# csmile-1006/ARP

Measured on NVIDIA B200. Metric: reward-labeled frames/sec, higher is better.
Workload: dtype fp16

## Files before the change

### arp_b200/build.py

```python
from __future__ import annotations

import hashlib
import os
import shutil
import subprocess
import sys
from pathlib import Path

PKG = Path(__file__).resolve().parent
CSRC = PKG / "csrc"
LIBDIR = PKG / "_lib"
LIB = LIBDIR / "libarp_b200.so"
STAMP = LIBDIR / "libarp_b200.stamp"

NVCC_FLAGS = [
    "-gencode", "arch=compute_100a,code=sm_100a",
    "-O3", "-std=c++17", "-lineinfo",
    "-shared", "-Xcompiler", "-fPIC",
    "-Xcompiler", "-fvisibility=hidden",
    "--expt-relaxed-constexpr",
    "-cudart", "static", "-Xcompiler", "-pthread",
]


if os.environ.get("ARP_OP_BF16", "0") not in ("", "0"):
    NVCC_FLAGS.append("-DARP_OP_FP16=0")


def _nvcc() -> str:
    for cand in (os.environ.get("NVCC"), shutil.which("nvcc"), "/usr/local/cuda/bin/nvcc"):
        if cand and Path(cand).exists():
            return cand
    raise RuntimeError("nvcc not found; arp_b200 has no prebuilt or CPU fallback")


def _sources_digest() -> str:
    h = hashlib.sha256()
    for p in sorted(list(CSRC.glob("*.cu")) + list(CSRC.glob("*.cuh")) + [PKG.parent / "include" / "arp_b200.h"]):
        h.update(p.name.encode())
        h.update(p.read_bytes())
    h.update(" ".join(NVCC_FLAGS).encode())
    return h.hexdigest()


def _file_digest(path: Path) -> str:
    return hashlib.sha256(path.read_bytes()).hexdigest()


def build_variant(out: Path, defines: list[str]) -> Path:
    out = Path(out)
    out.parent.mkdir(parents=True, exist_ok=True)
    flags = [f for f in NVCC_FLAGS if not f.startswith("-DARP_OP_")]
    res = subprocess.run([_nvcc(), *flags, *[f"-D{d}" for d in defines], "-o", str(out), str(CSRC / "capi.cu")],
                         capture_output=True, text=True)
    if res.returncode != 0:
        raise RuntimeError(f"nvcc failed:\n{res.stdout}\n{res.stderr}")
    return out


def build(force: bool = False, verbose: bool = False) -> Path:
    LIBDIR.mkdir(exist_ok=True)
    digest = _sources_digest()
    if not force and LIB.exists() and STAMP.exists() and STAMP.read_text().split() == [digest, _file_digest(LIB)]:
        return LIB
    cmd = [_nvcc(), *NVCC_FLAGS, "-o", str(LIB), str(CSRC / "capi.cu")]
    if verbose:
        cmd.insert(1, "-Xptxas")
        cmd.insert(2, "-v")
        print(" ".join(cmd), file=sys.stderr)
    res = subprocess.run(cmd, capture_output=True, text=True)
    if res.returncode != 0:
        raise RuntimeError(f"nvcc failed:\n{res.stdout}\n{res.stderr}")
    if verbose:
        print(res.stderr, file=sys.stderr)
    STAMP.write_text(f"{digest} {_file_digest(LIB)}")
    return LIB


JITTER_LIB = LIBDIR / "libarp_b200_jitter.so"


def build_jitter() -> Path:
    LIBDIR.mkdir(exist_ok=True)
    stamp = LIBDIR / "libarp_b200_jitter.stamp"
    digest = _sources_digest()
    if JITTER_LIB.exists() and stamp.exists() and stamp.read_text().split() == [digest, _file_digest(JITTER_LIB)]:
        return JITTER_LIB
    build_variant(JITTER_LIB, ["ARP_ATTN_JITTER"])
    stamp.write_text(f"{digest} {_file_digest(JITTER_LIB)}")
    return JITTER_LIB


if __name__ == "__main__":
    print(build(force="--force" in sys.argv, verbose="-v" in sys.argv))
```

### arp_b200/capi.py

```python
from __future__ import annotations

import ctypes as C
import os
from pathlib import Path

import numpy as np
import torch

_PKG = Path(__file__).resolve().parent
_LIB_PATH = Path(os.environ.get("ARP_B200_LIB") or _PKG / "_lib" / "libarp_b200.so")

ARP_OK = 0
ARP_ERR_INVALID, ARP_ERR_CUDA, ARP_ERR_STATE, ARP_ERR_NO_DEVICE, ARP_ERR_UNKNOWN_KEY = -1, -2, -3, -4, -5
PRE_PIL_BICUBIC, PRE_BILINEAR = 0, 1
HEAD_CLIP, HEAD_ADAPTER, HEAD_ADAPTER_ENSEMBLE, HEAD_CLIP_GOAL, HEAD_ADAPTER_GOAL = 0, 1, 2, 3, 4
REDUCE_FIRST, REDUCE_MEAN = 0, 1
DT_F32, DT_BF16, DT_F16 = 0, 1, 2
ACT_NONE, ACT_QUICKGELU, ACT_RELU = 0, 1, 2
PREC_BF16, PREC_F32, PREC_F32RESID = 0, 1, 2
PREC_16BIT = PREC_BF16
PRECISIONS = {"16bit": PREC_16BIT, "bf16": PREC_16BIT, "fp16": PREC_16BIT, "fp32resid": PREC_F32RESID, "fp32": PREC_F32}
(ARP_INFLATE_OK, ARP_INFLATE_TRUNCATED, ARP_INFLATE_BAD_HEADER, ARP_INFLATE_BAD_BLOCK, ARP_INFLATE_BAD_CODE,
 ARP_INFLATE_DISTANCE_TOO_FAR, ARP_INFLATE_TOO_LONG, ARP_INFLATE_TOO_SHORT, ARP_INFLATE_BAD_ADLER) = range(9)
MAX_TEXT = 16
MAX_TEXT_GROUPS = 16
MAX_TEXT_TOTAL = 64

EXPORTS = (
    "arp_create", "arp_destroy", "arp_last_error", "arp_abi_version", "arp_set_weight", "arp_missing_weights",
    "arp_set_text", "arp_label", "arp_label_host", "arp_compute_reward", "arp_encode_image", "arp_decode_only",
    "arp_scan_only", "arp_gemm_bf16", "arp_layernorm_bf16", "arp_attention", "arp_launch_count",
    "arp_profile_begin", "arp_profile_end", "arp_online_reward", "arp_preprocess_rtgs",
    "arp_quantile_f32", "arp_encode_taps_chw", "arp_operand_dtype", "arp_ln_gemm", "arp_resid_gemm_stats", "arp_label_file", "arp_wants_weight",
    "arp_set_text_groups", "arp_text_groups", "arp_embedding_dim", "arp_embed_host", "arp_embed_file",
    "arp_label_embeddings", "arp_tower_dim", "arp_embed_tower_host", "arp_embed_tower_file", "arp_label_tower",
    "arp_label_zfile", "arp_embed_zfile", "arp_embed_tower_zfile", "arp_inflate_rows",
)
PROFILE_CLASSES = ("gemm", "attention", "layernorm", "decode", "head", "scan", "other")


class ArpProfileStats(C.Structure):
    _fields_ = [("launches", C.c_int64), ("total_ms", C.c_double), ("flops", C.c_double), ("bytes", C.c_double)]


class ArpConfig(C.Structure):
    _fields_ = [(n, C.c_int32) for n in (
        "struct_size", "device", "patch", "width", "layers", "heads", "embed_dim", "in_h", "in_w", "use_crop",
        "preprocess", "head", "reduce", "max_batch", "precision")]


class ArpError(RuntimeError):
    def __init__(self, code: int, msg: str):
        super().__init__(f"arp_b200 error {code}: {msg}")
        self.code = code


_lib = None


def precision_enum(name: str) -> int:
    if name not in PRECISIONS:
        raise ValueError(f"precision must be one of {sorted(PRECISIONS)}, got {name!r}")
    return PRECISIONS[name]


def lib_path() -> Path:
    return _LIB_PATH


def load_library() -> C.CDLL:
    global _lib
    if _lib is not None:
        return _lib
    if not _LIB_PATH.exists():
        raise FileNotFoundError(
            f"{_LIB_PATH} not built — run `python -m arp_b200.build` (or __graft_entry__.build()). "
            "arp_b200 has no CPU or PyTorch fallback.")
    lib = C.CDLL(os.fspath(_LIB_PATH))
    vp, i32, i64, f32 = C.c_void_p, C.c_int32, C.c_int64, C.c_float
    lib.arp_create.argtypes = [C.POINTER(ArpConfig), C.POINTER(vp)]
    lib.arp_destroy.argtypes = [vp]
    lib.arp_destroy.restype = None
    lib.arp_last_error.argtypes = [vp]
    lib.arp_last_error.restype = C.c_char_p
    lib.arp_abi_version.argtypes = []
    lib.arp_operand_dtype.argtypes = []
    lib.arp_set_weight.argtypes = [vp, C.c_char_p, vp, i32, C.POINTER(i64), i32, vp]
    lib.arp_missing_weights.argtypes = [vp, C.c_char_p, i64]
    lib.arp_set_text.argtypes = [vp, vp, i32, i32, f32, vp]
    lib.arp_set_text_groups.argtypes = [vp, vp, i32, i32, vp, i32, f32, vp]
    lib.arp_text_groups.argtypes = [vp]
    lib.arp_label.argtypes = [vp, vp, i64, i64, vp, i32, i32, vp, vp, vp, vp, vp]
    lib.arp_label_host.argtypes = [vp, vp, i64, i64, vp, i32, i32, vp, vp, vp, vp]
    lib.arp_label_file.argtypes = [vp, i32, i64, i64, i64, vp, i32, i32, vp, vp, vp, vp]
    lib.arp_wants_weight.argtypes = [vp, C.c_char_p]
    lib.arp_embedding_dim.argtypes = [vp]
    lib.arp_embed_host.argtypes = [vp, vp, i64, i64, vp]
    lib.arp_embed_file.argtypes = [vp, i32, i64, i64, i64, vp]
    lib.arp_label_embeddings.argtypes = [vp, vp, i64, vp, i32, i32, vp, vp, vp, vp, vp]
    lib.arp_tower_dim.argtypes = [vp]
    lib.arp_embed_tower_host.argtypes = [vp, vp, i64, i64, vp]
    lib.arp_embed_tower_file.argtypes = [vp, i32, i64, i64, i64, vp]
    lib.arp_label_tower.argtypes = [vp, vp, i64, vp, i32, i32, vp, vp, vp, vp, vp]
    lib.arp_label_zfile.argtypes = [vp, i32, vp, vp, i64, i64, vp, i32, i32, vp, vp, vp, vp]
    lib.arp_embed_zfile.argtypes = [vp, i32, vp, vp, i64, i64, vp]
    lib.arp_embed_tower_zfile.argtypes = [vp, i32, vp, vp, i64, i64, vp]
    lib.arp_inflate_rows.argtypes = [vp, vp, vp, vp, i64, i64, vp, vp, vp]
    lib.arp_compute_reward.argtypes = [vp, vp, i64, i64, vp, vp, vp]
    lib.arp_online_reward.argtypes = [vp, vp, i32, vp, vp, vp]
    lib.arp_preprocess_rtgs.argtypes = [vp, vp, i64, vp, i32, i32, i32, vp, vp, vp, vp, vp]
    lib.arp_quantile_f32.argtypes = [vp, vp, i64, i64, i64, vp, vp]
    lib.arp_encode_taps_chw.argtypes = [vp, vp, i64, vp, vp, vp]
    lib.arp_encode_image.argtypes = [vp, vp, i64, i64, vp, vp]
    lib.arp_decode_only.argtypes = [vp, vp, i64, i64, vp, vp]
    lib.arp_scan_only.argtypes = [vp, vp, i64, vp, i32, i32, f32, vp, vp, vp, vp]
    lib.arp_gemm_bf16.argtypes = [vp, vp, vp, vp, i32, i64, i32, i32, vp, vp, i32, vp]
    lib.arp_ln_gemm.argtypes = [vp, vp, vp, vp, vp, vp, vp, i64, i32, i32, vp]
    lib.arp_resid_gemm_stats.argtypes = [vp, vp, vp, vp, vp, vp, i64, i32, i32, vp]
    lib.arp_layernorm_bf16.argtypes = [vp, vp, vp, vp, vp, i64, vp]
    lib.arp_attention.argtypes = [vp, vp, vp, i32, i32, vp]
    lib.arp_launch_count.argtypes = [vp]
    lib.arp_launch_count.restype = i64
    lib.arp_profile_begin.argtypes = [vp]
    lib.arp_profile_end.argtypes = [vp, C.POINTER(ArpProfileStats), i32]
    for name in EXPORTS:
        if name not in ("arp_destroy", "arp_last_error", "arp_launch_count"):
            getattr(lib, name).restype = C.c_int
    _lib = lib
    return lib


_TORCH_DT = {torch.float32: DT_F32, torch.bfloat16: DT_BF16, torch.float16: DT_F16}


def operand_dtype() -> torch.dtype:
    return {DT_BF16: torch.bfloat16, DT_F16: torch.float16}[load_library().arp_operand_dtype()]


def _ptr(t: "torch.Tensor | None"):
    return None if t is None else C.c_void_p(t.data_ptr())


def _stream_ptr(device) -> C.c_void_p:
    return C.c_void_p(torch.cuda.current_stream(device).cuda_stream)


class Engine:

    def __init__(self, *, device: int = 0, patch: int = 16, in_h: int = 64, in_w: int = 64, use_crop: bool = False,
                 preprocess: int = PRE_PIL_BICUBIC, head: int = HEAD_CLIP, reduce: int = REDUCE_FIRST,
                 max_batch: int = 256, layers: int = 12, width: int = 768, heads: int = 12, embed_dim: int = 512,
                 precision: int = PREC_BF16):
        self._lib = load_library()
        self._h = C.c_void_p()
        self.cfg = ArpConfig(C.sizeof(ArpConfig), device, patch, width, layers, heads, embed_dim, in_h, in_w,
                             int(bool(use_crop)), preprocess, head, reduce, max_batch, precision)
        rc = self._lib.arp_create(C.byref(self.cfg), C.byref(self._h))
        if rc != ARP_OK:
            raise ArpError(rc, (self._lib.arp_last_error(None) or b"").decode())
        self.device = torch.device("cuda", device)
        self.tokens = (224 // patch) ** 2 + 1
        self.adapter = head in (HEAD_ADAPTER, HEAD_ADAPTER_ENSEMBLE, HEAD_ADAPTER_GOAL)
        self.goal = head in (HEAD_CLIP_GOAL, HEAD_ADAPTER_GOAL)
        self.feat_dim = (layers + 1) * embed_dim if self.adapter else embed_dim
        self.n_text = 0
        self._grouped = False

    def close(self):
        if getattr(self, "_h", None) and self._h.value:
            self._lib.arp_destroy(self._h)
            self._h = C.c_void_p()

    def __del__(self):
        try:
            self.close()
        except Exception:
            pass

    def _check(self, rc: int):
        if rc != ARP_OK:
            raise ArpError(rc, (self._lib.arp_last_error(self._h) or b"").decode())

    @property
    def launch_count(self) -> int:
        return int(self._lib.arp_launch_count(self._h))

    def profile_begin(self):
        self._check(self._lib.arp_profile_begin(self._h))

    def profile_end(self) -> dict:
        arr = (ArpProfileStats * len(PROFILE_CLASSES))()
        self._check(self._lib.arp_profile_end(self._h, arr, len(PROFILE_CLASSES)))
        return {n: {"launches": int(a.launches), "total_ms": a.total_ms, "flops": a.flops, "bytes": a.bytes}
                for n, a in zip(PROFILE_CLASSES, arr)}

    def set_weight(self, name: str, tensor: torch.Tensor, strict: bool = True) -> bool:
        t = tensor.detach()
        if t.dtype not in _TORCH_DT:
            t = t.float()
        t = t.to(self.device).contiguous()
        shape = (C.c_int64 * max(t.dim(), 1))(*t.shape)
        rc = self._lib.arp_set_weight(self._h, name.encode(), _ptr(t), _TORCH_DT[t.dtype], shape, t.dim(),
                                      _stream_ptr(self.device))
        if rc == ARP_ERR_UNKNOWN_KEY and not strict:
            return False
        self._check(rc)
        torch.cuda.current_stream(self.device).synchronize()
        return True

    def load_state_dict(self, state_dict, strict: bool = False) -> list[str]:
        seen = getattr(self, "_uploaded", None)
        if seen is None:
            seen = self._uploaded = {}
        for k, v in state_dict.items():
            if not torch.is_tensor(v):
                continue
            if not strict and not self._lib.arp_wants_weight(self._h, k.encode()):
                continue
            mark = (v.data_ptr(), tuple(v.shape), v.dtype, v._version, v.device)
            if k in seen and seen[k][0] == mark and seen[k][1] is v:
                continue
            if self.set_weight(k, v, strict=strict):
                seen[k] = (mark, v)
        return self.missing_weights()

    def missing_weights(self) -> list[str]:
        buf = C.create_string_buffer(1 << 16)
        n = self._lib.arp_missing_weights(self._h, buf, len(buf))
        return [s for s in buf.value.decode().split("\n") if s] if n else []

    def set_text(self, text_emb: torch.Tensor, logit_scale_exp: float):
        t = text_emb.detach().to(self.device, torch.float32).contiguous()
        assert t.dim() == 2
        self._check(self._lib.arp_set_text(self._h, _ptr(t), t.shape[0], t.shape[1], float(logit_scale_exp),
                                           _stream_ptr(self.device)))
        torch.cuda.current_stream(self.device).synchronize()
        self.n_text = t.shape[0]
        self._grouped = False

    def set_text_groups(self, embs: "list[torch.Tensor]", logit_scale_exp: float):
        rows = [e.detach().to(self.device, torch.float32) for e in embs]
        assert rows and all(r.dim() == 2 for r in rows)
        t = torch.cat(rows).contiguous()
        off = np.concatenate([[0], np.cumsum([r.shape[0] for r in rows])]).astype(np.int32)
        self._check(self._lib.arp_set_text_groups(self._h, _ptr(t), t.shape[0], t.shape[1], C.c_void_p(off.ctypes.data),
                                                  len(rows), float(logit_scale_exp), _stream_ptr(self.device)))
        torch.cuda.current_stream(self.device).synchronize()
        self.n_text = t.shape[0]
        self._grouped = True

    @property
    def n_groups(self) -> int:
        return int(self._lib.arp_text_groups(self._h))

    def _lead(self) -> tuple:
        return (self.n_groups,) if self._grouped else ()

    def _host_outputs(self, T: int, num_frames: int):
        lead = self._lead()
        return (np.empty(lead + (T,), np.float32), np.empty(lead + (T,), np.float32),
                np.empty(lead + (T, num_frames), np.float32), np.empty(lead + (T, num_frames), np.float32))

    @staticmethod
    def _frames_view(ob: torch.Tensor):
        assert ob.dtype == torch.uint8 and ob.is_contiguous() and ob.dim() in (4, 5)
        T = ob.shape[0]
        frame = int(np.prod(ob.shape[-3:]))
        if ob.dim() == 5:
            F = ob.shape[1]
            return T, ob.data_ptr() + (F - 1) * frame, F * frame
        return T, ob.data_ptr(), frame
# ... 130 lines not shown
    @staticmethod
    def _chunk_table(chunk_offsets, chunk_bytes):
        off = np.ascontiguousarray(chunk_offsets, dtype=np.int64)
        nb = np.ascontiguousarray(chunk_bytes, dtype=np.int64)
        assert off.ndim == 1 and off.shape == nb.shape, (off.shape, nb.shape)
        return off, nb, C.c_void_p(off.ctypes.data), C.c_void_p(nb.ctypes.data)

    def label_zfile(self, fd: int, chunk_offsets: np.ndarray, chunk_bytes: np.ndarray, row_bytes: int,
                    ep_offsets: np.ndarray, num_frames: int, out=None):
        off, nb, p_off, p_nb = self._chunk_table(chunk_offsets, chunk_bytes)
        ep = np.ascontiguousarray(ep_offsets, dtype=np.int64)
        T = off.size
        if out is None:
            out = self._host_outputs(T, num_frames)
        hp = lambda a: C.c_void_p(a.ctypes.data)
        self._check(self._lib.arp_label_zfile(self._h, int(fd), p_off, p_nb, T, int(row_bytes), hp(ep), ep.size - 1,
                                              num_frames, hp(out[0]), hp(out[1]), hp(out[2]), hp(out[3])))
        return out

    def embed_zfile(self, fd: int, chunk_offsets: np.ndarray, chunk_bytes: np.ndarray, row_bytes: int,
                    out: "np.ndarray | None" = None) -> np.ndarray:
        off, nb, p_off, p_nb = self._chunk_table(chunk_offsets, chunk_bytes)
        out = self._emb_out(off.size, out)
        self._check(self._lib.arp_embed_zfile(self._h, int(fd), p_off, p_nb, off.size, int(row_bytes),
                                              C.c_void_p(out.ctypes.data)))
        return out

    def embed_tower_zfile(self, fd: int, chunk_offsets: np.ndarray, chunk_bytes: np.ndarray, row_bytes: int,
                          out: "np.ndarray | None" = None) -> np.ndarray:
        off, nb, p_off, p_nb = self._chunk_table(chunk_offsets, chunk_bytes)
        out = self._emb_out(off.size, out, self.tower_dim)
        self._check(self._lib.arp_embed_tower_zfile(self._h, int(fd), p_off, p_nb, off.size, int(row_bytes),
                                                    C.c_void_p(out.ctypes.data)))
        return out

    def inflate_rows(self, src: torch.Tensor, src_offsets: torch.Tensor, src_bytes: torch.Tensor, row_bytes: int):
        assert src.dtype == torch.uint8 and src.is_cuda and src.is_contiguous()
        so = src_offsets.to(self.device, torch.int64).contiguous()
        sb = src_bytes.to(self.device, torch.int64).contiguous()
        n = so.numel()
        assert sb.numel() == n
        out = torch.zeros((n, int(row_bytes)), device=self.device, dtype=torch.uint8)
        status = torch.full((n,), -1, device=self.device, dtype=torch.int32)
        self._check(self._lib.arp_inflate_rows(self._h, _ptr(src), _ptr(so), _ptr(sb), n, int(row_bytes), _ptr(out),
                                               _ptr(status), _stream_ptr(self.device)))
        return out, status

    def compute_reward(self, ob: torch.Tensor, want_logits: bool = False):
        T, p, stride = self._frames_view(ob)
        r = torch.empty(self._lead() + (T,), device=self.device, dtype=torch.float32)
        lg = torch.empty(T, max(self.n_text, 1), device=self.device, dtype=torch.float32) if want_logits else None
        self._check(self._lib.arp_compute_reward(self._h, C.c_void_p(p), T, stride, _ptr(r), _ptr(lg),
                                                 _stream_ptr(self.device)))
        return (r, lg) if want_logits else r

    def online_reward(self, frames: np.ndarray, want_logits: bool = False, want_features: bool = False):
        f = np.ascontiguousarray(frames, dtype=np.uint8)
        if f.ndim == 3:
            f = f[None]
        assert f.ndim == 4 and f.shape[1:] == (self.cfg.in_h, self.cfg.in_w, 3), f.shape
        n = f.shape[0]
        out = {}
        r = lg = ft = None
        if not self.goal:
            r = out["reward"] = np.empty(n, np.float32)
            if want_logits:
                lg = out["logits"] = np.empty((n, self.n_text), np.float32)
        if want_features or self.goal:
            ft = out["features"] = np.empty((n, self.feat_dim), np.float32)
        p = lambda a: None if a is None else C.c_void_p(a.ctypes.data)
        self._check(self._lib.arp_online_reward(self._h, p(f), n, p(r), p(lg), p(ft)))
        return out

    def preprocess_rtgs(self, reward: torch.Tensor, ep_offsets: torch.Tensor, num_frames: int, use_normalize: bool):
        r = reward.to(self.device, torch.float32).contiguous()
        off = ep_offsets.to(self.device, torch.int64).contiguous()
        T = r.numel()
        g = torch.zeros(T, device=self.device, dtype=torch.float32)
        gs = torch.zeros(T, num_frames, device=self.device, dtype=torch.float32)
        shifted = torch.empty(T, device=self.device, dtype=torch.float32) if use_normalize else None
        stats = np.zeros(4, np.float32)
        self._check(self._lib.arp_preprocess_rtgs(self._h, _ptr(r), T, _ptr(off), off.numel() - 1, num_frames,
                                                  int(bool(use_normalize)), _ptr(shifted), _ptr(g), _ptr(gs),
                                                  C.c_void_p(stats.ctypes.data), _stream_ptr(self.device)))
        return gs, g, stats

    def order_statistics(self, x: torch.Tensor, k_lo: int, k_hi: int) -> np.ndarray:
        x = x.to(self.device, torch.float32).contiguous().view(-1)
        out = np.zeros(2, np.float32)
        self._check(self._lib.arp_quantile_f32(self._h, _ptr(x), x.numel(), int(k_lo), int(k_hi),
                                               C.c_void_p(out.ctypes.data), _stream_ptr(self.device)))
        return out

    def encode_taps(self, chw: torch.Tensor):
        x = chw.to(self.device, torch.float32).contiguous()
        assert x.dim() == 4 and tuple(x.shape[1:]) == (3, 224, 224), x.shape
        T = x.shape[0]
        taps = torch.empty(T, self.cfg.layers * self.cfg.width, device=self.device, dtype=torch.float32)
        feat = torch.empty(T, self.cfg.embed_dim, device=self.device, dtype=torch.float32)
        self._check(self._lib.arp_encode_taps_chw(self._h, _ptr(x), T, _ptr(taps), _ptr(feat), _stream_ptr(self.device)))
        return taps, feat

    def encode_image(self, ob: torch.Tensor) -> torch.Tensor:
        T, p, stride = self._frames_view(ob)
        f = torch.empty(T, self.feat_dim, device=self.device, dtype=torch.float32)
        self._check(self._lib.arp_encode_image(self._h, C.c_void_p(p), T, stride, _ptr(f), _stream_ptr(self.device)))
        return f

    def decode_only(self, ob: torch.Tensor) -> torch.Tensor:
        T, p, stride = self._frames_view(ob)
        out = torch.empty(T, 3, 224, 224, device=self.device, dtype=torch.float32)
        self._check(self._lib.arp_decode_only(self._h, C.c_void_p(p), T, stride, _ptr(out), _stream_ptr(self.device)))
        return out

    def scan_only(self, reward: torch.Tensor, ep_offsets: torch.Tensor, num_frames: int, gamma: float = 1.0):
        r = reward.to(self.device, torch.float32).contiguous()
        off = ep_offsets.to(self.device, torch.int64).contiguous()
        T = r.numel()
        g = torch.empty(T, device=self.device, dtype=torch.float32)
        rs = torch.empty(T, num_frames, device=self.device, dtype=torch.float32)
        gs = torch.empty(T, num_frames, device=self.device, dtype=torch.float32)
        self._check(self._lib.arp_scan_only(self._h, _ptr(r), T, _ptr(off), off.numel() - 1, num_frames, gamma,
                                            _ptr(g), _ptr(rs), _ptr(gs), _stream_ptr(self.device)))
        return g, rs, gs

    def gemm(self, a: torch.Tensor, w: torch.Tensor, bias=None, resid=None, act: int = ACT_NONE,
             out_dtype=None) -> torch.Tensor:
        op = operand_dtype()
        assert a.dtype in (torch.bfloat16, torch.float16) and w.dtype in (torch.bfloat16, torch.float16)
        a, w = a.to(op).contiguous(), w.to(op).contiguous()
        M, K = a.shape
        N = w.shape[0]
        out_dtype = op if out_dtype in (None, torch.bfloat16, torch.float16) else out_dtype
        out = torch.empty(M, N, device=self.device, dtype=out_dtype)
        if resid is not None:
            resid = resid.to(out_dtype).contiguous()
        self._check(self._lib.arp_gemm_bf16(self._h, _ptr(a), _ptr(w), _ptr(out),
                                            DT_F32 if out_dtype == torch.float32 else _TORCH_DT[op], M, N, K, _ptr(bias),
                                            _ptr(resid), act, _stream_ptr(self.device)))
        return out

    def resid_gemm_stats(self, a: torch.Tensor, w: torch.Tensor, bias: torch.Tensor, x: torch.Tensor):
        op = operand_dtype()
        assert x.dtype == op and x.is_contiguous() and x.device == self.device
        a, w = a.to(op).contiguous(), w.to(op).contiguous()
        bias = bias.to(self.device, torch.float32).contiguous()
        M, K = a.shape
        N = w.shape[0]
        stats = torch.empty(M, 2, device=self.device, dtype=torch.float32)
        self._check(self._lib.arp_resid_gemm_stats(self._h, _ptr(a), _ptr(w), _ptr(bias), _ptr(x), _ptr(stats), M, N, K,
                                                   _stream_ptr(self.device)))
        return stats

    def ln_gemm(self, x: torch.Tensor, gamma, beta, w: torch.Tensor, bias: torch.Tensor, act: int = ACT_NONE) -> torch.Tensor:
        op = operand_dtype()
        x = x.to(op).contiguous()
        f = lambda t: t.to(self.device, torch.float32).contiguous()
        gamma, beta, w, bias = f(gamma), f(beta), f(w), f(bias)
        M, N = x.shape[0], w.shape[0]
        out = torch.empty(M, N, device=self.device, dtype=op)
        self._check(self._lib.arp_ln_gemm(self._h, _ptr(x), _ptr(gamma), _ptr(beta), _ptr(w), _ptr(bias), _ptr(out),
                                          M, N, act, _stream_ptr(self.device)))
        return out

    def layernorm(self, x: torch.Tensor, gamma: torch.Tensor, beta: torch.Tensor) -> torch.Tensor:
        assert x.dtype == torch.float32 and x.is_contiguous() and x.shape[-1] == 768
        y = torch.empty(x.shape, device=self.device, dtype=operand_dtype())
        self._check(self._lib.arp_layernorm_bf16(self._h, _ptr(x), _ptr(gamma), _ptr(beta), _ptr(y),
                                                 x.numel() // 768, _stream_ptr(self.device)))
        return y

    def attention(self, qkv: torch.Tensor, B: int, tokens: int) -> torch.Tensor:
        assert qkv.dtype in (torch.bfloat16, torch.float16)
        qkv = qkv.to(operand_dtype()).contiguous()
        out = torch.empty(B * tokens, qkv.shape[-1] // 3, device=self.device, dtype=qkv.dtype)
        self._check(self._lib.arp_attention(self._h, _ptr(qkv), _ptr(out), B, tokens, _stream_ptr(self.device)))
        return out
```

### arp_b200/csrc/attention_tc.cuh

```cuda
#pragma once

#include "common.cuh"

namespace arp {

constexpr int ATC_THREADS = 448;
constexpr int ATC_DH = 64;

template <int L>
struct AtcCfg {
  static constexpr int NK = (L + 15) / 16 * 16;
  static constexpr int QT = (L + 127) / 128;
  static constexpr int Q_BYTES = 128 * ATC_DH * 2;
  static constexpr int KV_BYTES = NK * ATC_DH * 2;
  static constexpr int KV_PAD = (KV_BYTES + 1023) / 1024 * 1024;
  static constexpr int BUF_BYTES = QT * Q_BYTES + 2 * KV_PAD;
  static constexpr int ONES_BYTES = 16 * 128;
  static constexpr int STAGE_BYTES = QT * 128 * ATC_DH * 2;
  static constexpr int SMEM_BYTES = 2 * BUF_BYTES + ONES_BYTES + STAGE_BYTES + 1024 + 256;
  static constexpr int O_COL = QT * NK;
  static constexpr int O_N = ATC_DH + 16;
  static constexpr bool SPREAD = QT == 2;
  static constexpr int Q1_LOADS = 5;
  static constexpr int QK_TX_BYTES = SPREAD ? Q_BYTES + Q1_LOADS * 16 * 128 + KV_BYTES : QT * Q_BYTES + KV_BYTES;
  static_assert(!SPREAD || (L - 176 > 16 && L - 176 <= 24 && NK % 64 == 16), "tile-1 spread is laid out for 193..200 tokens");
  static_assert(O_COL + O_N <= 512, "TMEM columns");
  static_assert(KV_PAD >= (NK / 16 - 1) * 2048, "the ones tile must sit past every step's V rows (positive LBO)");
};

__device__ __forceinline__ void umma_bf16_ts(uint32_t d_tmem, uint32_t a_tmem, uint64_t b_desc, uint32_t idesc,
                                             uint32_t accumulate) {
  asm volatile(
      "{\n\t"
      ".reg .pred p;\n\t"
      "setp.ne.b32 p, %4, 0;\n\t"
      "tcgen05.mma.cta_group::1.kind::f16 [%0], [%1], %2, %3, p;\n\t"
      "}\n" ::"r"(d_tmem),
      "r"(a_tmem), "l"(b_desc), "r"(idesc), "r"(accumulate)
      : "memory");
}

__device__ __forceinline__ void tmem_ld_32x16(uint32_t taddr, uint32_t (&r)[16]) {
  asm volatile(
      "tcgen05.ld.sync.aligned.32x32b.x16.b32 "
      "{%0, %1, %2, %3, %4, %5, %6, %7, %8, %9, %10, %11, %12, %13, %14, %15}, [%16];"
      : "=r"(r[0]), "=r"(r[1]), "=r"(r[2]), "=r"(r[3]), "=r"(r[4]), "=r"(r[5]), "=r"(r[6]), "=r"(r[7]),
        "=r"(r[8]), "=r"(r[9]), "=r"(r[10]), "=r"(r[11]), "=r"(r[12]), "=r"(r[13]), "=r"(r[14]), "=r"(r[15])
      : "r"(taddr)
      : "memory");
}
__device__ __forceinline__ void tmem_st_32x8(uint32_t taddr, const uint32_t (&r)[8]) {
  asm volatile("tcgen05.st.sync.aligned.32x32b.x8.b32 [%0], {%1, %2, %3, %4, %5, %6, %7, %8};" ::"r"(taddr),
               "r"(r[0]), "r"(r[1]), "r"(r[2]), "r"(r[3]), "r"(r[4]), "r"(r[5]), "r"(r[6]), "r"(r[7])
               : "memory");
}
__device__ __forceinline__ void tmem_st_wait() { asm volatile("tcgen05.wait::st.sync.aligned;" ::: "memory"); }

__device__ __forceinline__ uint64_t umma_desc_mnmajor_sw128(uint32_t smem_addr, uint32_t lbo_bytes = 16) {
  uint64_t d = 0;
  d |= static_cast<uint64_t>((smem_addr & 0x3FFFF) >> 4);
  d |= static_cast<uint64_t>((lbo_bytes >> 4) & 0x3FFF) << 16;
  d |= static_cast<uint64_t>(1024 >> 4) << 32;
  d |= static_cast<uint64_t>(1) << 46;
  d |= static_cast<uint64_t>(2) << 61;
  return d;
}

__device__ __forceinline__ uint32_t pack_bf16_int(float lo, float hi) {
  const uint32_t a = __float_as_uint(lo) + 0x8000u, b = __float_as_uint(hi) + 0x8000u;
  return (a >> 16) | (b & 0xffff0000u);
}

constexpr float kPExpOffset = ARP_OP_FP16 ? 97.0f : 0.0f;
__device__ __forceinline__ uint32_t pack_bf16_trunc(float lo, float hi) {
#if ARP_OP_FP16
  return (__float_as_uint(lo) >> 13) | ((__float_as_uint(hi) << 3) & 0xffff0000u);
#else
  return (__float_as_uint(lo) >> 16) | (__float_as_uint(hi) & 0xffff0000u);
#endif
}
constexpr uint32_t kOnes2 = ARP_OP_FP16 ? 0x3c003c00u : 0x3f803f80u;

__device__ __forceinline__ float ex2_approx(float x) {
  float y;
  asm("ex2.approx.ftz.f32 %0, %1;" : "=f"(y) : "f"(x));
  return y;
}

__device__ __forceinline__ void tmem_st_32x16(uint32_t taddr, const uint32_t (&r)[16]) {
  asm volatile(
      "tcgen05.st.sync.aligned.32x32b.x16.b32 [%0], {%1, %2, %3, %4, %5, %6, %7, %8, %9, %10, %11, %12, %13, %14, "
      "%15, %16};" ::"r"(taddr),
      "r"(r[0]), "r"(r[1]), "r"(r[2]), "r"(r[3]), "r"(r[4]), "r"(r[5]), "r"(r[6]), "r"(r[7]), "r"(r[8]), "r"(r[9]),
      "r"(r[10]), "r"(r[11]), "r"(r[12]), "r"(r[13]), "r"(r[14]), "r"(r[15])
      : "memory");
}

__device__ __forceinline__ void tmem_ld_16x256_x8(uint32_t taddr, uint32_t (&r)[32]) {
  asm volatile(
      "tcgen05.ld.sync.aligned.16x256b.x8.b32 "
      "{%0, %1, %2, %3, %4, %5, %6, %7, %8, %9, %10, %11, %12, %13, %14, %15, "
      "%16, %17, %18, %19, %20, %21, %22, %23, %24, %25, %26, %27, %28, %29, %30, %31}, [%32];"
      : "=r"(r[0]), "=r"(r[1]), "=r"(r[2]), "=r"(r[3]), "=r"(r[4]), "=r"(r[5]), "=r"(r[6]), "=r"(r[7]),
        "=r"(r[8]), "=r"(r[9]), "=r"(r[10]), "=r"(r[11]), "=r"(r[12]), "=r"(r[13]), "=r"(r[14]), "=r"(r[15]),
        "=r"(r[16]), "=r"(r[17]), "=r"(r[18]), "=r"(r[19]), "=r"(r[20]), "=r"(r[21]), "=r"(r[22]), "=r"(r[23]),
        "=r"(r[24]), "=r"(r[25]), "=r"(r[26]), "=r"(r[27]), "=r"(r[28]), "=r"(r[29]), "=r"(r[30]), "=r"(r[31])
      : "r"(taddr)
      : "memory");
}
__device__ __forceinline__ void tmem_ld_16x256_x2(uint32_t taddr, uint32_t (&r)[8]) {
  asm volatile("tcgen05.ld.sync.aligned.16x256b.x2.b32 {%0, %1, %2, %3, %4, %5, %6, %7}, [%8];"
               : "=r"(r[0]), "=r"(r[1]), "=r"(r[2]), "=r"(r[3]), "=r"(r[4]), "=r"(r[5]), "=r"(r[6]), "=r"(r[7])
               : "r"(taddr)
               : "memory");
}
__device__ __forceinline__ void tmem_st_16x128_x8(uint32_t taddr, const uint32_t (&r)[16]) {
  asm volatile(
      "tcgen05.st.sync.aligned.16x128b.x8.b32 [%0], {%1, %2, %3, %4, %5, %6, %7, %8, %9, %10, %11, %12, %13, %14, "
      "%15, %16};" ::"r"(taddr),
      "r"(r[0]), "r"(r[1]), "r"(r[2]), "r"(r[3]), "r"(r[4]), "r"(r[5]), "r"(r[6]), "r"(r[7]), "r"(r[8]), "r"(r[9]),
      "r"(r[10]), "r"(r[11]), "r"(r[12]), "r"(r[13]), "r"(r[14]), "r"(r[15])
      : "memory");
}
__device__ __forceinline__ void tmem_st_16x128_x2(uint32_t taddr, const uint32_t (&r)[4]) {
  asm volatile("tcgen05.st.sync.aligned.16x128b.x2.b32 [%0], {%1, %2, %3, %4};" ::"r"(taddr), "r"(r[0]), "r"(r[1]),
               "r"(r[2]), "r"(r[3])
               : "memory");
}
__device__ __forceinline__ void tmem_ld_32x1(uint32_t taddr, uint32_t& r) {
  asm volatile("tcgen05.ld.sync.aligned.32x32b.x1.b32 {%0}, [%1];" : "=r"(r) : "r"(taddr) : "memory");
}
__device__ __forceinline__ float rcp_approx(float x) {
  float y;
  asm("rcp.approx.ftz.f32 %0, %1;" : "=f"(y) : "f"(x));
  return y;
}

#ifdef ARP_ATTN_JITTER
__device__ __forceinline__ void atc_jitter(uint32_t salt) {
  uint32_t h = (static_cast<uint32_t>(clock64()) ^ (salt * 2654435761u) ^ (threadIdx.x >> 5) * 40503u ^ blockIdx.x * 9176u);
  h ^= h >> 13; h *= 0x5bd1e995u; h ^= h >> 15;
  if (h & 1) __nanosleep((h >> 1) & 8191);
}
#define ATC_JITTER(salt) atc_jitter(salt)
#else
#define ATC_JITTER(salt)
#endif

#ifdef ARP_ATTN_TRACE
constexpr int ATC_TR_ITEMS = 10, ATC_TR_EVENTS = 36;
__device__ long long g_attn_trace[2 * ATC_TR_ITEMS * ATC_TR_EVENTS];
#define ATC_TRACE(ev, slot, item)                                                                              \
  do {                                                                                                         \
    if (blockIdx.x == 0 && (threadIdx.x & 31) == 0 && (item) < ATC_TR_ITEMS)                                   \
      atc_tr[((slot) * ATC_TR_ITEMS + (item)) * ATC_TR_EVENTS + (ev)] = clock64();                             \
  } while (0)
#define ATC_TRACE_T(ev, slot, item)                                                                            \
  do {                                                                                                         \
    if (blockIdx.x == 0 && (item) < ATC_TR_ITEMS)                                                              \
      atc_tr[((slot) * ATC_TR_ITEMS + (item)) * ATC_TR_EVENTS + (ev)] = clock64();                             \
  } while (0)
#else
#define ATC_TRACE(ev, slot, item)
#define ATC_TRACE_T(ev, slot, item)
#endif

template <int L>
__global__ void __launch_bounds__(ATC_THREADS, 1)
attention_tc_kernel(const __grid_constant__ CUtensorMap tmap_q, const __grid_constant__ CUtensorMap tmap_kv,
                    const __grid_constant__ CUtensorMap tmap_o, const __grid_constant__ CUtensorMap tmap_q16,
                    const __grid_constant__ CUtensorMap tmap_o16, int n_frames, int heads, int width, float scale_log2e,
                    int reverse) {
  using C = AtcCfg<L>;
  extern __shared__ uint8_t smem_raw[];
  uint8_t* smem = reinterpret_cast<uint8_t*>((reinterpret_cast<uintptr_t>(smem_raw) + 1023) & ~uintptr_t(1023));
  uint8_t* ones = smem + 2 * C::BUF_BYTES;
  uint8_t* stage = ones + C::ONES_BYTES;
  uint64_t* bars = reinterpret_cast<uint64_t*>(stage + C::STAGE_BYTES);
  uint64_t* qk_full = bars;
  uint64_t* qk_empty = bars + 2;
  uint64_t* v_full = bars + 4;
  uint64_t* v_empty = bars + 6;
  uint64_t* s_full = bars + 8;
  uint64_t* o_full = bars + 10;
  uint64_t* o_drained = bars + 12;
  uint64_t* xu_turn = bars + 14;
  uint64_t* p_done = bars + 18;
  uint64_t* rem_go = bars + 20;
  uint32_t* tmem_slot = reinterpret_cast<uint32_t*>(bars + 22);

  const int warp = __shfl_sync(0xffffffffu, static_cast<int>(threadIdx.x >> 5), 0), lane = threadIdx.x & 31;
  const int n_items = n_frames * heads;
#ifdef ARP_ATTN_TRACE
  __shared__ long long atc_tr[2 * ATC_TR_ITEMS * ATC_TR_EVENTS];
  for (int i = threadIdx.x; i < 2 * ATC_TR_ITEMS * ATC_TR_EVENTS; i += ATC_THREADS) atc_tr[i] = 0;
#endif
  constexpr int SM_WARPS = 4 * C::QT;

  if (warp == 0 && lane == 0) {
    tma_prefetch_desc(&tmap_q);
    tma_prefetch_desc(&tmap_kv);
    tma_prefetch_desc(&tmap_o);
    tma_prefetch_desc(&tmap_q16);
    tma_prefetch_desc(&tmap_o16);
  }
  if (warp == 1 && lane == 0) {
    for (int i = 0; i < 2; ++i) {
      mbar_init(&qk_full[i], 1);
      mbar_init(&qk_empty[i], C::QT);
      mbar_init(&v_full[i], 1);
      mbar_init(&v_empty[i], C::QT);
      mbar_init(&s_full[i], 1);
      mbar_init(&o_full[i], 1);
    }
    for (int i = 0; i < 4; ++i) mbar_init(&xu_turn[i], 1);
    mbar_init(&p_done[0], 4);
    mbar_init(&p_done[1], C::SPREAD ? 5 : 4);
    mbar_init(&rem_go[0], 1);
    mbar_init(&rem_go[1], 1);
    mbar_init(&o_drained[0], 4);
    mbar_init(&o_drained[1], 4);
    fence_mbar_init();
  }
  for (int i = threadIdx.x; i < C::ONES_BYTES / 16; i += ATC_THREADS)
    reinterpret_cast<uint4*>(ones)[i] = make_uint4(kOnes2, kOnes2, kOnes2, kOnes2);
  if (C::SPREAD) {
    for (int i = threadIdx.x; i < 2 * 3 * 2048 / 16; i += ATC_THREADS) {
      const int b = i / (3 * 128), q = (i / 128) % 3, w = i % 128;
      reinterpret_cast<uint4*>(smem + b * C::BUF_BYTES + C::Q_BYTES + q * 4096 + 2048)[w] = make_uint4(0u, 0u, 0u, 0u);
    }
  }
  fence_proxy_async_smem();
  if (warp == 1) tmem_alloc<512>(tmem_slot);
  tc_fence_before();
  __syncthreads();
  tc_fence_after();
  const uint32_t tmem_base = __shfl_sync(0xffffffffu, *tmem_slot, 0);

  constexpr uint32_t idesc_s = umma_idesc_bf16(128, C::NK);
  constexpr uint32_t idesc_o = umma_idesc_bf16(128, C::O_N, 0, 1);
  auto issue_s = [&](uint32_t sbuf, int t, [[maybe_unused]] int tr_item) {
    const uint64_t dk = umma_desc_kmajor_sw128(sbuf + C::QT * C::Q_BYTES);
    const uint64_t dq = umma_desc_kmajor_sw128(sbuf + t * C::Q_BYTES);
    ATC_TRACE_T(24, t, tr_item);
#pragma unroll
    for (int k = 0; k < ATC_DH / 16; ++k) umma_bf16_ss(tmem_base + t * C::NK, dq + 2 * k, dk + 2 * k, idesc_s, k != 0);
    umma_commit(&s_full[t]);
    umma_commit(&qk_empty[(sbuf - smem_u32(smem)) / C::BUF_BYTES]);
    ATC_TRACE_T(27, t, tr_item);
  };
  auto issue_pv = [&](uint32_t sbuf, int t, [[maybe_unused]] int tr_item) {
    const uint32_t v_addr = sbuf + C::QT * C::Q_BYTES + C::KV_PAD;
    const uint64_t dv = umma_desc_mnmajor_sw128(v_addr, smem_u32(ones) - v_addr);
    constexpr uint64_t kStep = (2048ull >> 4) - ((2048ull >> 4) << 16);
    ATC_TRACE_T(28, t, tr_item);
#pragma unroll
    for (int k = 0; k < C::NK / 16; ++k)
      umma_bf16_ts(tmem_base + C::O_COL, tmem_base + t * C::NK + k * 8, dv + k * kStep, idesc_o, k != 0);
    umma_commit(&o_full[t]);
    ATC_TRACE_T(30, t, tr_item);
  };

  const bool sp_c0 = 192 + 2 * (lane & 3) < L, sp_c1 = 193 + 2 * (lane & 3) < L;
  auto spread_rowmax = [&](uint32_t tg, float& row_a, float& row_b) {
    auto max16 = [](const uint32_t (&r)[32], float& ma, float& mb) {
#pragma unroll
      for (int i = 0; i < 8; ++i) {
        ma = fmaxf(ma, fmaxf(__uint_as_float(r[4 * i]), __uint_as_float(r[4 * i + 1])));
        mb = fmaxf(mb, fmaxf(__uint_as_float(r[4 * i + 2]), __uint_as_float(r[4 * i + 3])));
      }
    };
    uint32_t a[32], bq[32], tl[8];
    float a0 = -INFINITY, a1 = -INFINITY, b0m = -INFINITY, b1m = -INFINITY;
    tmem_ld_16x256_x8(tg, a);
    tmem_ld_16x256_x8(tg + 64, bq);
    tmem_ld_wait();
    max16(a, a0, b0m);
    max16(bq, a1, b1m);
    tmem_ld_16x256_x8(tg + 128, a);
    tmem_ld_16x256_x2(tg + 192, tl);
    tmem_ld_wait();
    max16(a, a0, b0m);
    if (sp_c0) { a1 = fmaxf(a1, __uint_as_float(tl[0])); b1m = fmaxf(b1m, __uint_as_float(tl[2])); }
    if (sp_c1) { a1 = fmaxf(a1, __uint_as_float(tl[1])); b1m = fmaxf(b1m, __uint_as_float(tl[3])); }
    float ma = fmaxf(a0, a1), mb = fmaxf(b0m, b1m);
    ma = fmaxf(ma, __shfl_xor_sync(0xffffffffu, ma, 1));
    mb = fmaxf(mb, __shfl_xor_sync(0xffffffffu, mb, 1));
    ma = fmaxf(ma, __shfl_xor_sync(0xffffffffu, ma, 2));
    mb = fmaxf(mb, __shfl_xor_sync(0xffffffffu, mb, 2));
    row_a = ma;
    row_b = mb;
  };
  auto spread_exp = [&](uint32_t tg, float max_a, float max_b, bool both) {
    const float mo_a = max_a * scale_log2e + kPExpOffset, mo_b = max_b * scale_log2e + kPExpOffset;
    const uint64_t sc2 = f32x2_pack(scale_log2e, scale_log2e), na2 = f32x2_pack(-mo_a, -mo_a), nb2 = f32x2_pack(-mo_b, -mo_b);
    auto chunk16 = [&](const uint32_t (&src)[32], int blk) {
      uint32_t pk[16];
// ... 349 lines not shown
```

### arp_b200/csrc/capi.cu

```cuda
#include <cuda.h>
#include <cuda_runtime.h>

#include <atomic>
#include <chrono>
#include <cmath>
#include <condition_variable>
#include <cstdarg>
#include <cstdio>
#include <cstring>
#include <algorithm>
#include <map>
#include <mutex>
#include <string>
#include <thread>
#include <tuple>
#include <vector>

#include <cerrno>
#include <unistd.h>

#include "../../include/arp_b200.h"
#include "attention_tc.cuh"
#include "decode.cuh"
#include "fp32_path.cuh"
#include "gemm_tcgen05.cuh"
#include "head.cuh"
#include "inflate.cuh"
#include "layernorm.cuh"
#include "rtgstats.cuh"
#include "scan.cuh"
#include "tower.cuh"

using namespace arp;
static_assert(ARP_MAX_TEXT == HEAD_MAX_TEXT && ARP_MAX_TEXT_GROUPS == HEAD_MAX_GROUPS &&
              ARP_MAX_TEXT_TOTAL == HEAD_MAX_TEXT_TOTAL, "text limits of include/arp_b200.h and head.cuh disagree");
typedef arp::op_t bf16;
#define ARP_OP_DTYPE (ARP_OP_FP16 ? ARP_F16 : ARP_BF16)

static thread_local std::string g_create_error;

struct ArpHandle;
static int fail(ArpHandle* h, int code, const char* fmt, ...);

#define ARP_CUDA(h, expr)                                                                      \
  do {                                                                                         \
    cudaError_t _e = (expr);                                                                   \
    if (_e != cudaSuccess)                                                                     \
      return fail(h, ARP_ERR_CUDA, "%s failed: %s (%s:%d)", #expr, cudaGetErrorString(_e), __FILE__, __LINE__); \
  } while (0)

#define ARP_TRY(expr)            \
  do {                           \
    int _r = (expr);             \
    if (_r != ARP_OK) return _r; \
  } while (0)

typedef CUresult (*PFN_encodeTiled)(CUtensorMap*, CUtensorMapDataType, cuuint32_t, void*, const cuuint64_t*,
                                    const cuuint64_t*, const cuuint32_t*, const cuuint32_t*, CUtensorMapInterleave,
                                    CUtensorMapSwizzle, CUtensorMapL2promotion, CUtensorMapFloatOOBfill);

static PFN_encodeTiled get_encode_tiled() {
  static PFN_encodeTiled fn = nullptr;
  if (fn) return fn;
  void* p = nullptr;
  cudaDriverEntryPointQueryResult q;
  if (cudaGetDriverEntryPoint("cuTensorMapEncodeTiled", &p, cudaEnableDefault, &q) != cudaSuccess ||
      q != cudaDriverEntryPointSuccess)
    return nullptr;
  fn = reinterpret_cast<PFN_encodeTiled>(p);
  return fn;
}

struct LayerW {
  float *ln1_g = nullptr, *ln1_b = nullptr, *ln2_g = nullptr, *ln2_b = nullptr;
  bf16 *w_qkv = nullptr, *w_out = nullptr, *w_fc = nullptr, *w_proj = nullptr;
  float *b_qkv = nullptr, *b_out = nullptr, *b_fc = nullptr, *b_proj = nullptr;
  float *w_qkv_f32 = nullptr, *w_fc_f32 = nullptr;
  bf16 *w_qkv_fold = nullptr, *w_fc_fold = nullptr;
  float *s_qkv = nullptr, *c_qkv = nullptr, *s_fc = nullptr, *c_fc = nullptr;
};

struct WeightSlot {
  void** dst_f32 = nullptr;
  void** dst;
  int64_t numel;
  bool as_bf16;
  bool required;
  bool set;
};

struct TmapKey {
  const void* ptr; uint64_t rows, cols, ld; uint32_t box_rows, box_cols, elem;
  bool operator<(const TmapKey& o) const {
    return std::tie(ptr, rows, cols, ld, box_rows, box_cols, elem) <
           std::tie(o.ptr, o.rows, o.cols, o.ld, o.box_rows, o.box_cols, o.elem);
  }
};

struct ArpHandle {
  ArpConfig cfg;
  std::string err;
  int64_t launches = 0;
  bool resid16 = true;
  int dir = 0;
  bool f32 = false;
  int tokens = 0, grid = 0, kp = 0;
  bool adapter = false, goal = false;
  int n_scales = 0, feat_dim = 0;

  bf16* conv1 = nullptr;
  float *class_emb = nullptr, *pos_emb = nullptr, *rowtab = nullptr;
  float *ln_pre_g = nullptr, *ln_pre_b = nullptr, *ln_post_g = nullptr, *ln_post_b = nullptr;
  float* proj = nullptr;
  std::vector<LayerW> layers;
  bf16 *inter_w = nullptr, *fc1_w = nullptr, *fc2_w = nullptr;
  float *fc1_b = nullptr, *fc2_b = nullptr, *res_w = nullptr;
  float res_sigmoid = 0.f;
  bool finalized = false;
  bool adapter_ready = false;
  std::map<std::string, WeightSlot> slots;

  float* text = nullptr;
  int* group_off = nullptr;
  int group_off_host[HEAD_MAX_GROUPS + 1] = {};
  int n_text = 0, text_dim = 0, n_groups = 1;
  float logit_scale = 0.f;

  int *h_min = nullptr, *h_cnt = nullptr, *h_k = nullptr, *v_min = nullptr, *v_cnt = nullptr, *v_k = nullptr;
  int h_ksize = 0, v_ksize = 0, max_rows = 0;
  float* lut = nullptr;
  int crop_top = 0, crop_left = 0, src_h = 0, src_w = 0;

  struct Work {
    bf16* x16 = nullptr;
    float2* stats = nullptr;
    float* x = nullptr;
    bf16 *xn = nullptr, *qkv = nullptr, *attn = nullptr, *hid = nullptr;
    bf16 *taps = nullptr, *featb = nullptr, *hid2 = nullptr;
    float *featf = nullptr, *mlp = nullptr;
    float* xcls = nullptr;
    bf16 *xncls = nullptr, *qcls = nullptr, *acls = nullptr, *hcls = nullptr;
    float *chw32 = nullptr, *xn32 = nullptr, *qkv32 = nullptr, *attn32 = nullptr, *hid32 = nullptr;
    float *taps32 = nullptr, *hid2_32 = nullptr;
  } ws;

  void* scratch[2] = {nullptr, nullptr};
  size_t scratch_bytes[2] = {0, 0};
  uint8_t* stage_dev[2] = {nullptr, nullptr};
  size_t stage_bytes = 0;
  uint8_t* zsrc_dev[2] = {nullptr, nullptr};
  size_t zsrc_bytes = 0;
  uint8_t* zrows_dev = nullptr;
  size_t zrows_bytes = 0;
  void* ztab_dev = nullptr;
  size_t ztab_bytes = 0;
  uint8_t* pin_ring = nullptr;
  size_t pin_bytes = 0;
  cudaEvent_t ev_slot[8] = {nullptr, nullptr, nullptr, nullptr, nullptr, nullptr, nullptr, nullptr};
  cudaStream_t copy_stream = nullptr, own_stream = nullptr;
  cudaEvent_t ev_copied[2] = {nullptr, nullptr}, ev_consumed[2] = {nullptr, nullptr};

  std::map<TmapKey, CUtensorMap> tmaps;
  std::vector<void*> allocs;

  struct OnlineGraph { cudaGraphExec_t exec = nullptr; int64_t launches = 0; uint64_t epoch = 0; };
  std::map<int, OnlineGraph> online_graphs;
  uint64_t online_epoch = 1;
  float* online_out = nullptr;
  void* stats_dev = nullptr;

  bool profiling = false;
  struct ProfRec { int cls; double flops; double bytes; cudaEvent_t e0, e1; };
  std::vector<ProfRec> prof;
  std::vector<cudaEvent_t> event_pool;
};

enum ProfClass { PC_GEMM = 0, PC_ATTENTION = 1, PC_LAYERNORM = 2, PC_DECODE = 3, PC_HEAD = 4, PC_SCAN = 5, PC_OTHER = 6, PC_COUNT = 7 };

static cudaEvent_t prof_event(ArpHandle* h) {
  if (!h->event_pool.empty()) { cudaEvent_t e = h->event_pool.back(); h->event_pool.pop_back(); return e; }
  cudaEvent_t e = nullptr;
  cudaEventCreate(&e);
  return e;
}

struct ProfScope {
  ArpHandle* h; cudaStream_t st; size_t idx; bool on;
  ProfScope(ArpHandle* h_, int cls, double flops, double bytes, cudaStream_t st_) : h(h_), st(st_), idx(0), on(h_->profiling) {
    if (!on) return;
    ArpHandle::ProfRec r{cls, flops, bytes, prof_event(h), prof_event(h)};
    cudaEventRecord(r.e0, st);
    idx = h->prof.size();
    h->prof.push_back(r);
  }
  ~ProfScope() { if (on) cudaEventRecord(h->prof[idx].e1, st); }
};

static int fail(ArpHandle* h, int code, const char* fmt, ...) {
  char buf[1024];
  va_list ap;
  va_start(ap, fmt);
  vsnprintf(buf, sizeof(buf), fmt, ap);
  va_end(ap);
  if (h) h->err = buf; else g_create_error = buf;
  return code;
}

template <typename T>
static int dev_alloc(ArpHandle* h, T** p, size_t count) {
  void* q = nullptr;
  ARP_CUDA(h, cudaMalloc(&q, count * sizeof(T) + 256));
  h->allocs.push_back(q);
  ARP_CUDA(h, cudaMemset(q, 0, count * sizeof(T) + 256));
  *p = reinterpret_cast<T*>(q);
  return ARP_OK;
}

static double bicubic_filter(double x) {
  const double a = -0.5;
  if (x < 0.0) x = -x;
  if (x < 1.0) return ((a + 2.0) * x - (a + 3.0)) * x * x + 1;
  if (x < 2.0) return (((x - 5) * x + 8) * x - 4) * a;
  return 0.0;
}

static void pil_bicubic_tables(int in_size, int out_size, std::vector<int>& xmin_v, std::vector<int>& cnt_v,
                               std::vector<int>& kk, int& ksize) {
  double scale = static_cast<double>(in_size) / out_size;
  double filterscale = scale < 1.0 ? 1.0 : scale;
  const double support = 2.0 * filterscale;
  ksize = static_cast<int>(std::ceil(support)) * 2 + 1;
  xmin_v.assign(out_size, 0);
  cnt_v.assign(out_size, 0);
  kk.assign(static_cast<size_t>(out_size) * ksize, 0);
  std::vector<double> k(ksize);
  for (int xx = 0; xx < out_size; ++xx) {
    const double center = 0.0 + (xx + 0.5) * scale;
    double ww = 0.0;
    const double ss = 1.0 / filterscale;
    int xmin = static_cast<int>(center - support + 0.5);
    if (xmin < 0) xmin = 0;
    int xmax = static_cast<int>(center + support + 0.5);
    if (xmax > in_size) xmax = in_size;
    xmax -= xmin;
    for (int x = 0; x < xmax; ++x) {
      const double w = bicubic_filter((x + xmin - center + 0.5) * ss);
      k[x] = w;
      ww += w;
    }
    for (int x = 0; x < xmax; ++x)
      if (ww != 0.0) k[x] /= ww;
    for (int x = 0; x < xmax; ++x) {
      const double v = k[x] * (1 << 22);
      kk[static_cast<size_t>(xx) * ksize + x] = v < 0 ? static_cast<int>(-0.5 + v) : static_cast<int>(0.5 + v);
    }
    xmin_v[xx] = xmin;
    cnt_v[xx] = xmax;
  }
}

static const float kClipMean[3] = {0.48145466f, 0.4578275f, 0.40821073f};
static const float kClipStd[3] = {0.26862954f, 0.26130258f, 0.27577711f};

template <typename T>
static int upload(ArpHandle* h, T** dst, const std::vector<T>& v) {
  ARP_TRY(dev_alloc(h, dst, v.size()));
  ARP_CUDA(h, cudaMemcpy(*dst, v.data(), v.size() * sizeof(T), cudaMemcpyHostToDevice));
  return ARP_OK;
}

static int build_decode_tables(ArpHandle* h) {
  const ArpConfig& c = h->cfg;
  h->src_h = c.in_h;
  h->src_w = c.in_w;
  h->crop_top = h->crop_left = 0;
  if (c.use_crop) {
    if (c.preprocess == ARP_PRE_PIL_BICUBIC) {
      const int cs = c.in_w / 2;
      h->src_h = h->src_w = cs;
      h->crop_top = static_cast<int>(std::nearbyint((c.in_h - cs) / 2.0));
      h->crop_left = static_cast<int>(std::nearbyint((c.in_w - cs) / 2.0));
    } else {
      const int cs = c.in_w / 2;
      h->src_h = h->src_w = cs;
      h->crop_top = (c.in_h - cs) / 2;
      h->crop_left = (c.in_w - cs) / 2;
    }
  }
  if (h->src_h <= 0 || h->src_w <= 0 || h->crop_top < 0 || h->crop_top + h->src_h > c.in_h || h->crop_left < 0 ||
      h->crop_left + h->src_w > c.in_w)
    return fail(h, ARP_ERR_INVALID, "bad crop geometry for %dx%d (a crop larger than the frame would be zero-padded by "
                "torchvision; not supported)", c.in_h, c.in_w);
  if (c.preprocess == ARP_PRE_PIL_BICUBIC) {
    int out_w = DEC_OUT, out_h = DEC_OUT;
    if (h->src_w > h->src_h) out_w = static_cast<int>(static_cast<long long>(DEC_OUT) * h->src_w / h->src_h);
    else if (h->src_h > h->src_w) out_h = static_cast<int>(static_cast<long long>(DEC_OUT) * h->src_h / h->src_w);
    const int win_left = static_cast<int>(std::nearbyint((out_w - DEC_OUT) / 2.0));
    const int win_top = static_cast<int>(std::nearbyint((out_h - DEC_OUT) / 2.0));
    std::vector<int> xm, xc, xk, ym, yc, yk;
    {
      std::vector<int> fm, fc, fk;
      pil_bicubic_tables(h->src_w, out_w, fm, fc, fk, h->h_ksize);
      xm.assign(fm.begin() + win_left, fm.begin() + win_left + DEC_OUT);
      xc.assign(fc.begin() + win_left, fc.begin() + win_left + DEC_OUT);
      xk.assign(fk.begin() + (size_t)win_left * h->h_ksize, fk.begin() + (size_t)(win_left + DEC_OUT) * h->h_ksize);
      pil_bicubic_tables(h->src_h, out_h, fm, fc, fk, h->v_ksize);
      ym.assign(fm.begin() + win_top, fm.begin() + win_top + DEC_OUT);
      yc.assign(fc.begin() + win_top, fc.begin() + win_top + DEC_OUT);
      yk.assign(fk.begin() + (size_t)win_top * h->v_ksize, fk.begin() + (size_t)(win_top + DEC_OUT) * h->v_ksize);
    }
    if (h->h_ksize > 64 || h->v_ksize > 64) return fail(h, ARP_ERR_INVALID, "downscale factor too large");
    {
// ... 16 lines not shown
    ARP_TRY(upload(h, &h->h_min, xm)); ARP_TRY(upload(h, &h->h_cnt, xc)); ARP_TRY(upload(h, &h->h_k, xk));
    ARP_TRY(upload(h, &h->v_min, ym)); ARP_TRY(upload(h, &h->v_cnt, yc)); ARP_TRY(upload(h, &h->v_k, yk));
    std::vector<float> lut(3 * 256);
    for (int ch = 0; ch < 3; ++ch)
      for (int u = 0; u < 256; ++u) {
        volatile float v = static_cast<float>(u) / 255.0f;
        volatile float w = v - kClipMean[ch];
        lut[ch * 256 + u] = w / kClipStd[ch];
      }
    ARP_TRY(upload(h, &h->lut, lut));
  } else {
    const float sc = static_cast<float>(h->src_h) / DEC_OUT;
    h->max_rows = static_cast<int>(sc * DEC_BAND) + 4;
    if (h->max_rows > h->src_h) h->max_rows = h->src_h;
    h->h_ksize = h->v_ksize = 0;
  }
  return ARP_OK;
}

static void add_slot(ArpHandle* h, const std::string& name, void** dst, int64_t numel, bool as_bf16, bool required) {
  WeightSlot s;
  s.dst = dst; s.numel = numel; s.as_bf16 = as_bf16; s.required = required; s.set = false;
  h->slots[name] = s;
}

static void register_slots(ArpHandle* h) {
  const ArpConfig& c = h->cfg;
  const int W = c.width, P = c.patch;
  add_slot(h, "visual.conv1.weight", (void**)&h->conv1, (int64_t)W * 3 * P * P, true, true);
  add_slot(h, "visual.class_embedding", (void**)&h->class_emb, W, false, true);
  add_slot(h, "visual.positional_embedding", (void**)&h->pos_emb, (int64_t)h->tokens * W, false, true);
  add_slot(h, "visual.ln_pre.weight", (void**)&h->ln_pre_g, W, false, true);
  add_slot(h, "visual.ln_pre.bias", (void**)&h->ln_pre_b, W, false, true);
  add_slot(h, "visual.ln_post.weight", (void**)&h->ln_post_g, W, false, true);
  add_slot(h, "visual.ln_post.bias", (void**)&h->ln_post_b, W, false, true);
  add_slot(h, "visual.proj", (void**)&h->proj, (int64_t)W * c.embed_dim, false, true);
  h->layers.resize(c.layers);
  for (int l = 0; l < c.layers; ++l) {
    LayerW& L = h->layers[l];
    const std::string p = "visual.transformer.resblocks." + std::to_string(l) + ".";
    add_slot(h, p + "ln_1.weight", (void**)&L.ln1_g, W, false, true);
    add_slot(h, p + "ln_1.bias", (void**)&L.ln1_b, W, false, true);
    add_slot(h, p + "ln_2.weight", (void**)&L.ln2_g, W, false, true);
    add_slot(h, p + "ln_2.bias", (void**)&L.ln2_b, W, false, true);
    add_slot(h, p + "attn.in_proj_weight", (void**)&L.w_qkv, (int64_t)3 * W * W, true, true);
    add_slot(h, p + "attn.in_proj_bias", (void**)&L.b_qkv, 3 * W, false, true);
    add_slot(h, p + "attn.out_proj.weight", (void**)&L.w_out, (int64_t)W * W, true, true);
    add_slot(h, p + "attn.out_proj.bias", (void**)&L.b_out, W, false, true);
    add_slot(h, p + "mlp.c_fc.weight", (void**)&L.w_fc, (int64_t)4 * W * W, true, true);
    add_slot(h, p + "mlp.c_fc.bias", (void**)&L.b_fc, 4 * W, false, true);
    add_slot(h, p + "mlp.c_proj.weight", (void**)&L.w_proj, (int64_t)4 * W * W, true, true);
    add_slot(h, p + "mlp.c_proj.bias", (void**)&L.b_proj, W, false, true);
    h->slots[p + "attn.in_proj_weight"].dst_f32 = (void**)&L.w_qkv_f32;
    h->slots[p + "mlp.c_fc.weight"].dst_f32 = (void**)&L.w_fc_f32;
  }
  if (h->adapter) {
    const int64_t D = h->feat_dim;
    const int64_t Din = (int64_t)c.layers * W;
    const int64_t Dmid = (int64_t)c.layers * c.embed_dim;
    add_slot(h, "image_intermediate_linear.weight", (void**)&h->inter_w, Dmid * Din, true, true);
    add_slot(h, "image_adapter.layers.0.weight", (void**)&h->fc1_w, 2 * D * D, true, true);
    add_slot(h, "image_adapter.layers.0.bias", (void**)&h->fc1_b, 2 * D, false, true);
    add_slot(h, "image_adapter.layers.3.weight", (void**)&h->fc2_w, 2 * D * D, true, true);
    add_slot(h, "image_adapter.layers.3.bias", (void**)&h->fc2_b, D, false, true);
    add_slot(h, "image_residual_weight", (void**)&h->res_w, 1, false, true);
  }
}

template <typename S, typename D>
__global__ void convert_kernel(const S* __restrict__ src, D* __restrict__ dst, size_t n) {
  for (size_t i = static_cast<size_t>(blockIdx.x) * blockDim.x + threadIdx.x; i < n;
       i += static_cast<size_t>(gridDim.x) * blockDim.x)
    dst[i] = static_cast<D>(static_cast<float>(src[i]));
}

template <typename S, typename D>
static void launch_convert(ArpHandle* h, const void* src, void* dst, size_t n, cudaStream_t st) {
  const int blocks = static_cast<int>(std::min<size_t>((n + 255) / 256, 148 * 16));
  convert_kernel<S, D><<<blocks, 256, 0, st>>>(static_cast<const S*>(src), static_cast<D*>(dst), n);
  h->launches++;
}

__global__ void build_rowtab_kernel(const float* __restrict__ pos, const float* __restrict__ cls,
                                    float* __restrict__ tab, int tokens, int W) {
  const int i = blockIdx.x * blockDim.x + threadIdx.x;
  if (i >= tokens * W) return;
  tab[i] = pos[i] + (i < W ? cls[i] : 0.f);
}

extern "C" int arp_abi_version(void) { return ARP_B200_ABI_VERSION; }
extern "C" int arp_operand_dtype(void) { return ARP_OP_DTYPE; }

extern "C" const char* arp_last_error(const ArpHandle* h) { return h ? h->err.c_str() : g_create_error.c_str(); }

extern "C" int64_t arp_launch_count(const ArpHandle* h) { return h ? h->launches : 0; }

extern "C" int arp_profile_begin(ArpHandle* h) {
  if (!h) return ARP_ERR_INVALID;
  for (auto& r : h->prof) { h->event_pool.push_back(r.e0); h->event_pool.push_back(r.e1); }
  h->prof.clear();
  h->profiling = true;
  return ARP_OK;
}

extern "C" int arp_profile_end(ArpHandle* h, ArpProfileStats* out, int32_t n_classes) {
  if (!h || !out || n_classes < 1) return fail(h, ARP_ERR_INVALID, "null argument");
  h->profiling = false;
  ARP_CUDA(h, cudaSetDevice(h->cfg.device));
  ARP_CUDA(h, cudaDeviceSynchronize());
  for (int i = 0; i < n_classes; ++i) out[i] = ArpProfileStats{0, 0.0, 0.0, 0.0};
  for (auto& r : h->prof) {
    float ms = 0.f;
    cudaEventElapsedTime(&ms, r.e0, r.e1);
    if (r.cls < n_classes) {
      out[r.cls].launches += 1;
      out[r.cls].total_ms += ms;
      out[r.cls].flops += r.flops;
      out[r.cls].bytes += r.bytes;
    }
    h->event_pool.push_back(r.e0);
    h->event_pool.push_back(r.e1);
  }
  h->prof.clear();
  return ARP_OK;
}

template <typename K>
static int set_smem(ArpHandle* h, K kernel, int bytes) {
  ARP_CUDA(h, cudaFuncSetAttribute(kernel, cudaFuncAttributeMaxDynamicSharedMemorySize, bytes));
  return ARP_OK;
}

extern "C" void arp_destroy(ArpHandle* h) {
  if (!h) return;
  cudaSetDevice(h->cfg.device);
  cudaDeviceSynchronize();
  for (void* p : h->allocs) cudaFree(p);
  for (int i = 0; i < 2; ++i) if (h->scratch[i]) cudaFree(h->scratch[i]);
  for (int i = 0; i < 2; ++i) {
    if (h->stage_dev[i]) cudaFree(h->stage_dev[i]);
    if (h->zsrc_dev[i]) cudaFree(h->zsrc_dev[i]);
    if (h->ev_copied[i]) cudaEventDestroy(h->ev_copied[i]);
    if (h->ev_consumed[i]) cudaEventDestroy(h->ev_consumed[i]);
  }
  if (h->zrows_dev) cudaFree(h->zrows_dev);
  if (h->ztab_dev) cudaFree(h->ztab_dev);
  if (h->pin_ring) cudaFreeHost(h->pin_ring);
  for (cudaEvent_t e : h->ev_slot) if (e) cudaEventDestroy(e);
  for (auto& kv : h->online_graphs) if (kv.second.exec) cudaGraphExecDestroy(kv.second.exec);
  for (auto& r : h->prof) { cudaEventDestroy(r.e0); cudaEventDestroy(r.e1); }
  for (cudaEvent_t e : h->event_pool) cudaEventDestroy(e);
  if (h->copy_stream) cudaStreamDestroy(h->copy_stream);
  if (h->own_stream) cudaStreamDestroy(h->own_stream);
  delete h;
}

extern "C" int arp_create(const ArpConfig* cfg, ArpHandle** out) {
  if (!cfg || !out) return fail(nullptr, ARP_ERR_INVALID, "null argument");
  if (cfg->struct_size != (int32_t)sizeof(ArpConfig))
    return fail(nullptr, ARP_ERR_INVALID, "ArpConfig.struct_size %d != %zu", cfg->struct_size, sizeof(ArpConfig));
  *out = nullptr;
  int ndev = 0;
  if (cudaGetDeviceCount(&ndev) != cudaSuccess || ndev == 0 || cfg->device < 0 || cfg->device >= ndev)
    return fail(nullptr, ARP_ERR_NO_DEVICE, "no CUDA device %d (count %d); this library has no CPU path", cfg->device, ndev);
  cudaDeviceProp prop;
  if (cudaGetDeviceProperties(&prop, cfg->device) != cudaSuccess || prop.major != 10)
    return fail(nullptr, ARP_ERR_NO_DEVICE, "device %d is sm_%d%d; arp_b200 is built for sm_100a only", cfg->device,
                prop.major, prop.minor);
  if (cfg->width != 768 || cfg->embed_dim != 512 || cfg->heads * 64 != cfg->width)
    return fail(nullptr, ARP_ERR_INVALID, "only ViT-B geometry is built (width 768, 64-wide heads, embed 512)");
  if (cfg->patch != 16 && cfg->patch != 32) return fail(nullptr, ARP_ERR_INVALID, "patch must be 16 or 32");
  if (cfg->layers < 1 || cfg->layers > 48 || cfg->max_batch < 1 || cfg->in_h < 8 || cfg->in_w < 8)
    return fail(nullptr, ARP_ERR_INVALID, "bad layers / max_batch / frame size");
  if (cfg->head < 0 || cfg->head > ARP_HEAD_ADAPTER_GOAL || cfg->preprocess < 0 || cfg->preprocess > 1)
    return fail(nullptr, ARP_ERR_INVALID, "bad head / preprocess enum");
  if (cfg->precision != ARP_PREC_BF16 && cfg->precision != ARP_PREC_F32 && cfg->precision != ARP_PREC_F32RESID)
    return fail(nullptr, ARP_ERR_INVALID, "bad precision enum");
  if (!get_encode_tiled()) return fail(nullptr, ARP_ERR_CUDA, "cuTensorMapEncodeTiled not available from the driver");

  ArpHandle* h = new ArpHandle();
  h->cfg = *cfg;
  auto bail = [&](int code) { g_create_error = h->err; arp_destroy(h); return code; };
  if (cudaSetDevice(cfg->device) != cudaSuccess) { h->err = "cudaSetDevice failed"; return bail(ARP_ERR_CUDA); }
  h->f32 = cfg->precision == ARP_PREC_F32;
  h->resid16 = cfg->precision == ARP_PREC_BF16;
  h->grid = DEC_OUT / cfg->patch;
  h->tokens = h->grid * h->grid + 1;
  h->kp = 3 * cfg->patch * cfg->patch;
  h->adapter = cfg->head == ARP_HEAD_ADAPTER || cfg->head == ARP_HEAD_ADAPTER_ENSEMBLE || cfg->head == ARP_HEAD_ADAPTER_GOAL;
  h->goal = cfg->head == ARP_HEAD_CLIP_GOAL || cfg->head == ARP_HEAD_ADAPTER_GOAL;
  h->n_scales = cfg->layers + 1;
  h->feat_dim = h->adapter ? h->n_scales * cfg->embed_dim : cfg->embed_dim;
  if (h->adapter && h->n_scales != 13) { h->err = "adapter heads are built for 12-layer CLIP (13 scales)"; return bail(ARP_ERR_INVALID); }

  int r = build_decode_tables(h);
  if (r != ARP_OK) return bail(r);
  register_slots(h);

  const size_t B = cfg->max_batch, M = B * h->tokens, W = cfg->width;
#define CREATE_TRY(e) do { int _r = (e); if (_r != ARP_OK) return bail(_r); } while (0)
  CREATE_TRY(dev_alloc(h, &h->rowtab, (size_t)h->tokens * W));
  {
    ArpHandle::Work& w = h->ws;
    if (h->f32) {
      CREATE_TRY(dev_alloc(h, &w.x, M * W));
      CREATE_TRY(dev_alloc(h, &w.chw32, B * 3 * DEC_OUT * DEC_OUT));
      CREATE_TRY(dev_alloc(h, &w.xn32, M * W));
      CREATE_TRY(dev_alloc(h, &w.qkv32, M * 3 * W));
      CREATE_TRY(dev_alloc(h, &w.attn32, M * W));
      CREATE_TRY(dev_alloc(h, &w.hid32, M * std::max<size_t>(4 * W, h->kp)));
      if (h->adapter) {
        const size_t D = h->feat_dim;
        CREATE_TRY(dev_alloc(h, &w.taps32, B * cfg->layers * W));
        CREATE_TRY(dev_alloc(h, &w.featf, B * D));
        CREATE_TRY(dev_alloc(h, &w.hid2_32, B * 2 * D));
        CREATE_TRY(dev_alloc(h, &w.mlp, B * D));
      }
    } else {
      CREATE_TRY(dev_alloc(h, &w.qkv, M * 3 * W));
      if (cudaMemset(w.qkv, 0, M * 3 * W * sizeof(bf16)) != cudaSuccess) { h->err = "cudaMemset failed"; return bail(ARP_ERR_CUDA); }
      if (h->resid16) {
        CREATE_TRY(dev_alloc(h, &w.x16, M * W));
        CREATE_TRY(dev_alloc(h, &w.stats, M * (2 * W / 256)));
        w.x = reinterpret_cast<float*>(w.qkv);
      } else {
        CREATE_TRY(dev_alloc(h, &w.x, M * W));
        CREATE_TRY(dev_alloc(h, &w.xn, M * W));
      }
      CREATE_TRY(dev_alloc(h, &w.attn, M * W));
      CREATE_TRY(dev_alloc(h, &w.hid, M * std::max<size_t>(4 * W, h->kp)));
      CREATE_TRY(dev_alloc(h, &w.xcls, B * W));
      CREATE_TRY(dev_alloc(h, &w.xncls, B * W));
      CREATE_TRY(dev_alloc(h, &w.qcls, B * W));
      CREATE_TRY(dev_alloc(h, &w.acls, B * W));
      CREATE_TRY(dev_alloc(h, &w.hcls, B * 4 * W));
      if (h->adapter) {
        const size_t D = h->feat_dim;
        CREATE_TRY(dev_alloc(h, &w.taps, B * cfg->layers * W));
        CREATE_TRY(dev_alloc(h, &w.featf, B * D));
        CREATE_TRY(dev_alloc(h, &w.featb, B * D));
        CREATE_TRY(dev_alloc(h, &w.hid2, B * 2 * D));
        CREATE_TRY(dev_alloc(h, &w.mlp, B * D));
      }
    }
  }
  for (auto& kv : h->slots) {
    WeightSlot& s = kv.second;
    void* p = nullptr;
    if (h->f32) s.as_bf16 = false;
    if (cudaMalloc(&p, s.numel * (s.as_bf16 ? 2 : 4) + 256) != cudaSuccess) { h->err = "cudaMalloc(weights) failed"; return bail(ARP_ERR_CUDA); }
    h->allocs.push_back(p);
    *s.dst = p;
    if (s.dst_f32 && h->resid16 && !h->f32) {
      float* q = nullptr;
      if (dev_alloc(h, &q, (size_t)s.numel) != ARP_OK) return bail(ARP_ERR_CUDA);
      *s.dst_f32 = q;
    }
  }
  if (h->resid16 && !h->f32) {
    for (auto& L : h->layers) {
      if (dev_alloc(h, &L.w_qkv_fold, (size_t)3 * W * W) != ARP_OK || dev_alloc(h, &L.w_fc_fold, (size_t)4 * W * W) != ARP_OK ||
          dev_alloc(h, &L.s_qkv, (size_t)3 * W) != ARP_OK || dev_alloc(h, &L.c_qkv, (size_t)3 * W) != ARP_OK ||
          dev_alloc(h, &L.s_fc, (size_t)4 * W) != ARP_OK || dev_alloc(h, &L.c_fc, (size_t)4 * W) != ARP_OK)
        return bail(ARP_ERR_CUDA);
    }
  }
#define G2_ATTR(T, A, R) CREATE_TRY(set_smem(h, gemm_tcgen05_kernel<T, A, 2, R>, G2Cfg<2>::SMEM_BYTES));
  G2_ATTR(bf16, ACT_NONE, G2_STORE) G2_ATTR(bf16, ACT_QUICKGELU, G2_STORE) G2_ATTR(bf16, ACT_RELU, G2_STORE)
  G2_ATTR(float, ACT_NONE, G2_STORE) G2_ATTR(float, ACT_QUICKGELU, G2_STORE) G2_ATTR(float, ACT_RELU, G2_STORE)
  G2_ATTR(float, ACT_NONE, G2_REDUCE) G2_ATTR(bf16, ACT_NONE, G2_REDUCE)
  G2_ATTR(bf16, ACT_NONE, G2_LNFOLD) G2_ATTR(bf16, ACT_QUICKGELU, G2_LNFOLD) G2_ATTR(bf16, ACT_NONE, G2_RESID_STATS)
#undef G2_ATTR
  CREATE_TRY(set_smem(h, attention_tc_kernel<197>, AtcCfg<197>::SMEM_BYTES));
  CREATE_TRY(set_smem(h, attention_tc_kernel<50>, AtcCfg<50>::SMEM_BYTES));
  CREATE_TRY(set_smem(h, decode_kernel, 160 * 1024));
  CREATE_TRY(set_smem(h, clip_head_kernel<768, 512>, HEAD_SMEM_BYTES));
  CREATE_TRY(set_smem(h, attention_f32_kernel, attn_f32_smem_bytes(197)));
  if (cudaStreamCreateWithFlags(&h->copy_stream, cudaStreamNonBlocking) != cudaSuccess ||
      cudaStreamCreateWithFlags(&h->own_stream, cudaStreamNonBlocking) != cudaSuccess) {
    h->err = "cudaStreamCreate failed";
    return bail(ARP_ERR_CUDA);
  }
  for (int i = 0; i < 2; ++i) {
    cudaEventCreateWithFlags(&h->ev_copied[i], cudaEventDisableTiming);
    cudaEventCreateWithFlags(&h->ev_consumed[i], cudaEventDisableTiming);
  }
#undef CREATE_TRY
  *out = h;
  return ARP_OK;
}

static bool is_ignored_key(const std::string& n) {
  static const char* prefixes[] = {"transformer.", "token_embedding.", "positional_embedding", "ln_final.",
                                   "text_projection", "logit_scale", "text_intermediate_linear.", "text_adapter.",
                                   "text_residual_weight", "inverse_layer.", "lambda_id", "input_resolution",
                                   "context_length", "vocab_size", "image_intermediate_linear.", "image_adapter.",
                                   "image_residual_weight"};
  for (const char* p : prefixes)
    if (n.compare(0, strlen(p), p) == 0) return true;
  return false;
}

extern "C" int arp_set_weight(ArpHandle* h, const char* name, const void* data, int32_t dtype, const int64_t* shape,
                              int32_t ndim, void* stream) {
  if (!h || !name || !data || (ndim > 0 && !shape)) return fail(h, ARP_ERR_INVALID, "null argument");
  cudaStream_t st = static_cast<cudaStream_t>(stream);
  std::string key(name);
  if (key.compare(0, 11, "clip_model.") == 0) key = key.substr(11);
  auto it = h->slots.find(key);
  if (it == h->slots.end()) {
    if (is_ignored_key(key)) return ARP_OK;
    return fail(h, ARP_ERR_UNKNOWN_KEY, "unknown weight '%s'", name);
  }
  WeightSlot& s = it->second;
  int64_t numel = 1;
  for (int i = 0; i < ndim; ++i) numel *= shape[i];
  if (numel != s.numel) return fail(h, ARP_ERR_INVALID, "weight '%s': %lld elements, expected %lld", name, (long long)numel, (long long)s.numel);
  ARP_CUDA(h, cudaSetDevice(h->cfg.device));
  void* dst = *s.dst;
  const size_t n = static_cast<size_t>(numel);
  if (s.as_bf16) {
    if (dtype == ARP_F32) launch_convert<float, bf16>(h, data, dst, n, st);
    else if (dtype == ARP_OP_DTYPE) ARP_CUDA(h, cudaMemcpyAsync(dst, data, n * 2, cudaMemcpyDeviceToDevice, st));
    else if (dtype == ARP_F16) launch_convert<__half, bf16>(h, data, dst, n, st);
    else if (dtype == ARP_BF16) launch_convert<__nv_bfloat16, bf16>(h, data, dst, n, st);
    else return fail(h, ARP_ERR_INVALID, "bad dtype %d", dtype);
  } else {
    if (dtype == ARP_F32) ARP_CUDA(h, cudaMemcpyAsync(dst, data, n * 4, cudaMemcpyDeviceToDevice, st));
    else if (dtype == ARP_F16) launch_convert<__half, float>(h, data, dst, n, st);
    else if (dtype == ARP_BF16) launch_convert<__nv_bfloat16, float>(h, data, dst, n, st);
    else return fail(h, ARP_ERR_INVALID, "bad dtype %d", dtype);
  }
  if (s.dst_f32 && *s.dst_f32) {
    void* d32 = *s.dst_f32;
    if (dtype == ARP_F32) ARP_CUDA(h, cudaMemcpyAsync(d32, data, n * 4, cudaMemcpyDeviceToDevice, st));
    else if (dtype == ARP_F16) launch_convert<__half, float>(h, data, d32, n, st);
    else launch_convert<__nv_bfloat16, float>(h, data, d32, n, st);
  }
  ARP_CUDA(h, cudaGetLastError());
  s.set = true;
  h->finalized = false;
  h->adapter_ready = false;
  h->online_epoch++;
  return ARP_OK;
}

extern "C" int arp_missing_weights(const ArpHandle* h, char* names_out, int64_t names_cap) {
  if (!h) return -1;
  int missing = 0;
  std::string names;
  for (const auto& kv : h->slots)
    if (kv.second.required && !kv.second.set) {
      ++missing;
      names += kv.first;
      names += '\n';
    }
  if (names_out && names_cap > 0) {
    const size_t n = std::min<size_t>(names.size(), static_cast<size_t>(names_cap - 1));
    memcpy(names_out, names.data(), n);
    names_out[n] = 0;
  }
  return missing;
}

static int read_res_sigmoid(ArpHandle* h, cudaStream_t st) {
  float w = 0.f;
  ARP_CUDA(h, cudaMemcpyAsync(&w, h->res_w, 4, cudaMemcpyDeviceToHost, st));
  ARP_CUDA(h, cudaStreamSynchronize(st));
  h->res_sigmoid = 1.0f / (1.0f + expf(-w));
  return ARP_OK;
}

static int finalize_weights(ArpHandle* h, cudaStream_t st) {
  if (h->finalized) return ARP_OK;
  char buf[256];
  const int miss = arp_missing_weights(h, buf, sizeof(buf));
  if (miss) return fail(h, ARP_ERR_STATE, "%d weights not set, first: %.200s", miss, buf);
  const int n = h->tokens * h->cfg.width;
  build_rowtab_kernel<<<(n + 255) / 256, 256, 0, st>>>(h->pos_emb, h->class_emb, h->rowtab, h->tokens, h->cfg.width);
  h->launches++;
  if (h->resid16 && !h->f32) {
    const int W = h->cfg.width;
    for (auto& L : h->layers) {
      fold_ln_weights_kernel<<<(3 * W + 7) / 8, 256, 0, st>>>(L.w_qkv_f32, L.ln1_g, L.ln1_b, L.b_qkv, L.w_qkv_fold, L.s_qkv, L.c_qkv, 3 * W, W);
      fold_ln_weights_kernel<<<(4 * W + 7) / 8, 256, 0, st>>>(L.w_fc_f32, L.ln2_g, L.ln2_b, L.b_fc, L.w_fc_fold, L.s_fc, L.c_fc, 4 * W, W);
      h->launches += 2;
    }
  }
  if (h->adapter) ARP_TRY(read_res_sigmoid(h, st));
  ARP_CUDA(h, cudaGetLastError());
  h->finalized = true;
  return ARP_OK;
}

static int adapter_weights_ready(ArpHandle* h, cudaStream_t st) {
  if (h->adapter_ready || h->finalized) return ARP_OK;
  static const char* names[] = {"image_intermediate_linear.weight", "image_adapter.layers.0.weight",
                                "image_adapter.layers.0.bias", "image_adapter.layers.3.weight",
                                "image_adapter.layers.3.bias", "image_residual_weight"};
  for (const char* n : names)
    if (!h->slots.at(n).set) return fail(h, ARP_ERR_STATE, "adapter weight '%s' not set", n);
  ARP_TRY(read_res_sigmoid(h, st));
  h->adapter_ready = true;
  return ARP_OK;
}

static int set_text_rows(ArpHandle* h, const float* text_emb_dev, int32_t n_text_total, int32_t dim,
                         const int32_t* group_offsets_host, int32_t n_groups, float logit_scale_exp, cudaStream_t st) {
  if (!h || !text_emb_dev || !group_offsets_host) return fail(h, ARP_ERR_INVALID, "null argument");
  if (n_groups < 1 || n_groups > HEAD_MAX_GROUPS)
    return fail(h, ARP_ERR_INVALID, "n_groups must be in [1,%d], got %d", HEAD_MAX_GROUPS, n_groups);
  if (n_text_total < 1 || n_text_total > HEAD_MAX_TEXT_TOTAL)
    return fail(h, ARP_ERR_INVALID, "n_text_total must be in [1,%d], got %d", HEAD_MAX_TEXT_TOTAL, n_text_total);
  if (group_offsets_host[0] != 0 || group_offsets_host[n_groups] != n_text_total)
    return fail(h, ARP_ERR_INVALID, "group offsets must run from 0 to n_text_total=%d", n_text_total);
  for (int g = 0; g < n_groups; ++g) {
    const int n = group_offsets_host[g + 1] - group_offsets_host[g];
    if (n < 1 || n > HEAD_MAX_TEXT)
      return fail(h, ARP_ERR_INVALID, "group %d has %d texts, must be in [1,%d]", g, n, HEAD_MAX_TEXT);
  }
  if (dim != h->feat_dim) return fail(h, ARP_ERR_INVALID, "text dim %d, head expects %d", dim, h->feat_dim);
  ARP_CUDA(h, cudaSetDevice(h->cfg.device));
  if (!h->text) ARP_TRY(dev_alloc(h, &h->text, (size_t)HEAD_MAX_TEXT_TOTAL * h->feat_dim));
  if (!h->group_off) ARP_TRY(dev_alloc(h, &h->group_off, (size_t)HEAD_MAX_GROUPS + 1));
  std::copy(group_offsets_host, group_offsets_host + n_groups + 1, h->group_off_host);
  ARP_CUDA(h, cudaMemcpyAsync(h->text, text_emb_dev, (size_t)n_text_total * dim * 4, cudaMemcpyDeviceToDevice, st));
  ARP_CUDA(h, cudaMemcpyAsync(h->group_off, h->group_off_host, (size_t)(n_groups + 1) * 4, cudaMemcpyHostToDevice, st));
  h->n_text = n_text_total;
  h->n_groups = n_groups;
  h->text_dim = dim;
  h->logit_scale = logit_scale_exp;
  h->online_epoch++;
  return ARP_OK;
}

extern "C" int arp_set_text_groups(ArpHandle* h, const float* text_emb_dev, int32_t n_text_total, int32_t dim,
                                   const int32_t* group_offsets_host, int32_t n_groups, float logit_scale_exp,
                                   void* stream) {
  if (h && h->goal) return fail(h, ARP_ERR_INVALID, "goal-conditioned heads take no text");
  return set_text_rows(h, text_emb_dev, n_text_total, dim, group_offsets_host, n_groups, logit_scale_exp,
                       static_cast<cudaStream_t>(stream));
}

extern "C" int arp_set_text(ArpHandle* h, const float* text_emb_dev, int32_t n_text, int32_t dim, float logit_scale_exp,
                            void* stream) {
  if (h && (n_text < 1 || n_text > HEAD_MAX_TEXT))
    return fail(h, ARP_ERR_INVALID, "n_text must be in [1,%d]", HEAD_MAX_TEXT);
  const int32_t off[2] = {0, n_text};
  return set_text_rows(h, text_emb_dev, n_text, dim, off, 1, logit_scale_exp, static_cast<cudaStream_t>(stream));
}

extern "C" int arp_text_groups(const ArpHandle* h) { return h ? h->n_groups : 0; }

static int get_tmap(ArpHandle* h, const void* ptr, uint64_t rows, uint64_t cols, uint64_t ld, uint32_t box_rows,
                    const CUtensorMap** out, uint32_t box_cols = GEMM_BK, uint32_t elem = 2) {
  TmapKey key{ptr, rows, cols, ld, box_rows, box_cols, elem};
  auto it = h->tmaps.find(key);
  if (it == h->tmaps.end()) {
    if (h->tmaps.size() > 4096) h->tmaps.clear();
    CUtensorMap m;
    cuuint64_t gdim[2] = {cols, rows};
    cuuint64_t gstr[1] = {ld * elem};
    cuuint32_t box[2] = {box_cols, box_rows};
    cuuint32_t estr[2] = {1, 1};
    if ((reinterpret_cast<uintptr_t>(ptr) & 15) || (gstr[0] & 15))
      return fail(h, ARP_ERR_INVALID, "GEMM operand must be 16-byte aligned with a 16-byte multiple row pitch");
    CUresult r = get_encode_tiled()(&m, elem == 2 ? (ARP_OP_FP16 ? CU_TENSOR_MAP_DATA_TYPE_FLOAT16 : CU_TENSOR_MAP_DATA_TYPE_BFLOAT16) : CU_TENSOR_MAP_DATA_TYPE_FLOAT32,
                                    2, const_cast<void*>(ptr), gdim, gstr, box,
                                    estr, CU_TENSOR_MAP_INTERLEAVE_NONE, CU_TENSOR_MAP_SWIZZLE_128B,
                                    CU_TENSOR_MAP_L2_PROMOTION_L2_256B, CU_TENSOR_MAP_FLOAT_OOB_FILL_NONE);
    if (r != CUDA_SUCCESS) return fail(h, ARP_ERR_CUDA, "cuTensorMapEncodeTiled failed (%d) rows=%llu cols=%llu", (int)r, (unsigned long long)rows, (unsigned long long)cols);
    it = h->tmaps.emplace(key, m).first;
  }
  *out = &it->second;
  return ARP_OK;
}

static int get_tmap_attn_out(ArpHandle* h, const void* ptr, uint64_t frames, uint64_t tokens, uint64_t width,
                             const CUtensorMap** out, uint32_t box_rows = 32) {
  TmapKey key{ptr, frames, tokens, width, box_rows, 64, 0x30002u};
  auto it = h->tmaps.find(key);
  if (it == h->tmaps.end()) {
    if (h->tmaps.size() > 4096) h->tmaps.clear();
    CUtensorMap m;
    cuuint64_t gdim[3] = {width, tokens, frames};
    cuuint64_t gstr[2] = {width * 2, tokens * width * 2};
    cuuint32_t box[3] = {64, box_rows, 1};
    cuuint32_t estr[3] = {1, 1, 1};
    if ((reinterpret_cast<uintptr_t>(ptr) & 15) || (gstr[0] & 15))
      return fail(h, ARP_ERR_INVALID, "attention output must be 16-byte aligned with a 16-byte multiple row pitch");
    CUresult r = get_encode_tiled()(&m, ARP_OP_FP16 ? CU_TENSOR_MAP_DATA_TYPE_FLOAT16 : CU_TENSOR_MAP_DATA_TYPE_BFLOAT16, 3,
                                    const_cast<void*>(ptr), gdim, gstr, box, estr, CU_TENSOR_MAP_INTERLEAVE_NONE,
                                    CU_TENSOR_MAP_SWIZZLE_128B, CU_TENSOR_MAP_L2_PROMOTION_L2_256B,
                                    CU_TENSOR_MAP_FLOAT_OOB_FILL_NONE);
    if (r != CUDA_SUCCESS) return fail(h, ARP_ERR_CUDA, "cuTensorMapEncodeTiled (attention output) failed (%d)", (int)r);
    it = h->tmaps.emplace(key, m).first;
  }
  *out = &it->second;
  return ARP_OK;
}

template <typename K>
static cudaError_t launch_clustered(K kernel, int grid, int cg, int smem, cudaStream_t st, const CUtensorMap& ta,
                                    const CUtensorMap& tb, const CUtensorMap& to, const GemmArgs& g) {
  cudaLaunchConfig_t cfg{};
  cfg.gridDim = dim3(grid);
  cfg.blockDim = dim3(G2_THREADS);
  cfg.dynamicSmemBytes = smem;
  cfg.stream = st;
  cudaLaunchAttribute attr[1];
  attr[0].id = cudaLaunchAttributeClusterDimension;
  attr[0].val.clusterDim.x = cg;
  attr[0].val.clusterDim.y = 1;
  attr[0].val.clusterDim.z = 1;
  cfg.attrs = attr;
  cfg.numAttrs = 1;
  return cudaLaunchKernelEx(&cfg, kernel, ta, tb, to, g);
}

struct LnFoldArgs { const float2* stats; const float* svec; const float* cvec; int nparts = 1; };

static int launch_gemm(ArpHandle* h, const bf16* a, int64_t a_rows_alloc, const bf16* w, void* out, bool out_f32,
                       int act, int64_t M, int N, int K, int ldo, const float* bias, const void* resid, int ldr,
                       const float* rowtab, int period, cudaStream_t st, const LnFoldArgs* fold = nullptr,
                       float2* stats_out = nullptr) {
  if (M <= 0) return ARP_OK;
  if (N % GEMM_BN || K % GEMM_BK) return fail(h, ARP_ERR_INVALID, "GEMM needs N %% 256 == 0 and K %% 64 == 0 (N=%d K=%d)", N, K);
  if (M > 0x7fffffff / 2) return fail(h, ARP_ERR_INVALID, "GEMM M too large");
  constexpr int cg = 2;
  const size_t osz = out_f32 ? 4 : 2;
  GemmArgs g;
  memset(&g, 0, sizeof(g));
  g.M = (int)M; g.N = N; g.K = K; g.out = out; g.ldo = ldo; g.bias = bias;
  g.rowtab = rowtab; g.period = period > 0 ? period : 1;
  g.reverse = h->dir ^= 1;
  const bool reduce = resid != nullptr;
  if (fold) {
    if (out_f32 || act == ACT_RELU || reduce || rowtab || !fold->stats || !fold->svec || !fold->cvec)
      return fail(h, ARP_ERR_INVALID, "bad LayerNorm-folded GEMM");
    g.ln_stats = fold->stats; g.ln_nparts = fold->nparts; g.svec = fold->svec; g.cvec = fold->cvec; g.eps = 1e-5f;
    g.bias = nullptr;
  }
  const bool resid_stats = stats_out != nullptr;
  if (resid_stats) {
    if (!reduce || resid != out || out_f32 || ldr != ldo || rowtab || !bias) return fail(h, ARP_ERR_INVALID, "bad residual+statistics GEMM");
    g.resid = static_cast<const bf16*>(resid); g.ldr = ldr; g.stats_out = stats_out; g.eps = 1e-5f;
  }
  if (reduce) {
    if (act != ACT_NONE) return fail(h, ARP_ERR_INVALID, "the residual epilogue takes no activation");
    if (resid != out)
      ARP_CUDA(h, cudaMemcpy2DAsync(out, (size_t)ldo * osz, resid, (size_t)ldr * osz, (size_t)N * osz, (size_t)M,
                                    cudaMemcpyDeviceToDevice, st));
  }
  const CUtensorMap *ta, *tb, *to;
  ARP_TRY(get_tmap(h, a, (uint64_t)a_rows_alloc, (uint64_t)K, (uint64_t)K, GEMM_BM, &ta));
  ARP_TRY(get_tmap(h, w, (uint64_t)N, (uint64_t)K, (uint64_t)K, GEMM_BN / cg, &tb));
  ARP_TRY(get_tmap(h, out, (uint64_t)M, (uint64_t)N, (uint64_t)ldo, 32, &to, out_f32 ? 32 : 64, out_f32 ? 4 : 2));
  const int row_blocks = (int)((M + GEMM_BM * cg - 1) / (GEMM_BM * cg));
  const int tiles = row_blocks * (N / GEMM_BN);
  const int grid = std::min(tiles * cg, kNumSMs / cg * cg);
  const int smem = G2Cfg<cg>::SMEM_BYTES;
  ProfScope prof(h, PC_GEMM, 2.0 * (double)M * N * K,
                 (double)M * K * 2 + (double)N * K * 2 + (double)M * N * osz * (reduce ? 2 : 1), st);
  cudaError_t e;
#define G2_LAUNCH(T, A, R) e = launch_clustered(gemm_tcgen05_kernel<T, A, cg, R>, grid, cg, smem, st, *ta, *tb, *to, g)
  if (fold) {
    if (act == ACT_NONE) G2_LAUNCH(bf16, ACT_NONE, G2_LNFOLD);
    else G2_LAUNCH(bf16, ACT_QUICKGELU, G2_LNFOLD);
  } else if (resid_stats) {
    G2_LAUNCH(bf16, ACT_NONE, G2_RESID_STATS);
  } else if (reduce) {
    if (out_f32) G2_LAUNCH(float, ACT_NONE, G2_REDUCE);
    else G2_LAUNCH(bf16, ACT_NONE, G2_REDUCE);
  } else if (out_f32) {
    if (act == ACT_NONE) G2_LAUNCH(float, ACT_NONE, G2_STORE);
    else if (act == ACT_QUICKGELU) G2_LAUNCH(float, ACT_QUICKGELU, G2_STORE);
    else G2_LAUNCH(float, ACT_RELU, G2_STORE);
  } else {
    if (act == ACT_NONE) G2_LAUNCH(bf16, ACT_NONE, G2_STORE);
    else if (act == ACT_QUICKGELU) G2_LAUNCH(bf16, ACT_QUICKGELU, G2_STORE);
    else G2_LAUNCH(bf16, ACT_RELU, G2_STORE);
  }
#undef G2_LAUNCH
  h->launches++;
  if (e != cudaSuccess) return fail(h, ARP_ERR_CUDA, "GEMM launch failed: %s", cudaGetErrorString(e));
  return ARP_OK;
}

static int launch_decode(ArpHandle* h, const uint8_t* ob, int64_t n, int64_t stride, void* out, int out_kind,
                         cudaStream_t st) {
  if (n <= 0) return ARP_OK;
  DecodeArgs a;
  memset(&a, 0, sizeof(a));
  a.ob = ob; a.frame_stride = stride; a.in_w = h->cfg.in_w;
  a.crop_top = h->crop_top; a.crop_left = h->crop_left; a.src_h = h->src_h; a.src_w = h->src_w;
  a.T = (int)n; a.mode = h->cfg.preprocess; a.out_kind = out_kind;
  a.h_min = h->h_min; a.h_cnt = h->h_cnt; a.h_k = h->h_k; a.h_ksize = h->h_ksize;
  a.v_min = h->v_min; a.v_cnt = h->v_cnt; a.v_k = h->v_k; a.v_ksize = h->v_ksize;
  a.lut = h->lut;
  for (int c = 0; c < 3; ++c) { a.mean[c] = kClipMean[c]; a.stdv[c] = kClipStd[c]; }
  a.out = out; a.patch = h->cfg.patch; a.grid = h->grid; a.tokens = h->tokens; a.max_rows = h->max_rows;
  const int smem = dec_smem_bytes(h->src_w, h->max_rows, h->h_ksize, h->v_ksize, out_kind);
  if (smem > 160 * 1024) return fail(h, ARP_ERR_INVALID, "frame too large for the decode kernel (%d B smem)", smem);
  ProfScope prof(h, PC_DECODE, 0.0,
                 (double)n * ((double)h->src_h * h->src_w * 3 +
                              (out_kind == DEC_OUT_PATCH_BF16 ? (double)h->tokens * h->kp * 2 : 3.0 * DEC_OUT * DEC_OUT * 4)), st);
  for (int64_t f0 = 0; f0 < n; f0 += 32768) {
    const int cnt = (int)std::min<int64_t>(32768, n - f0);
    DecodeArgs b = a;
    b.ob = ob + f0 * stride;
    b.T = cnt;
    if (out_kind == DEC_OUT_PATCH_BF16) b.out = static_cast<bf16*>(out) + (size_t)f0 * h->tokens * h->kp;
    else b.out = static_cast<float*>(out) + (size_t)f0 * 3 * DEC_OUT * DEC_OUT;
    decode_kernel<<<dim3(DEC_OUT / DEC_BAND, cnt), DEC_THREADS, smem, st>>>(b);
    h->launches++;
  }
  ARP_CUDA(h, cudaGetLastError());
  return ARP_OK;
}

static int launch_ln_bf16(ArpHandle* h, const float* x, const float* g, const float* b, bf16* y, int64_t M,
                          cudaStream_t st) {
  if (M <= 0) return ARP_OK;
  ProfScope prof(h, PC_LAYERNORM, 0.0, (double)M * 768 * 6, st);
  layernorm_f32_bf16_kernel<768><<<(unsigned)((M + 7) / 8), 256, 0, st>>>(x, g, b, y, (int)M, 1e-5f, h->dir ^= 1);
  h->launches++;
  ARP_CUDA(h, cudaGetLastError());
  return ARP_OK;
}

static int launch_row_moments(ArpHandle* h, const bf16* x, float2* stats, int64_t M, cudaStream_t st) {
  if (M <= 0) return ARP_OK;
  ProfScope prof(h, PC_LAYERNORM, 0.0, (double)M * (768 * 2 + 8), st);
  row_moments_kernel<768><<<(unsigned)((M + 7) / 8), 256, 0, st>>>(x, stats, (int)M, 1e-5f, h->dir ^= 1);
  h->launches++;
  ARP_CUDA(h, cudaGetLastError());
  return ARP_OK;
}

static int launch_attention(ArpHandle* h, const bf16* qkv, bf16* out, int B, int tokens, cudaStream_t st,
                            int64_t rows_alloc = 0) {
  if (B <= 0) return ARP_OK;
  const float scale_log2e = 0.125f * 1.4426950408889634f;
  ProfScope prof(h, PC_ATTENTION, 4.0 * (double)B * h->cfg.heads * tokens * tokens * 64,
                 (double)B * tokens * h->cfg.width * 2 * 4, st);
  if (tokens != 197 && tokens != 50) return fail(h, ARP_ERR_INVALID, "attention is built for 197 or 50 tokens, got %d", tokens);
  const int W = h->cfg.width;
  const uint64_t rows = rows_alloc > 0 ? (uint64_t)rows_alloc : (uint64_t)B * tokens;
  const int nk = (tokens + 15) / 16 * 16;
  const CUtensorMap *tq, *tkv, *to, *tq16, *to16;
  ARP_TRY(get_tmap(h, qkv, rows, 3 * W, 3 * W, 128, &tq));
  ARP_TRY(get_tmap(h, qkv, rows, 3 * W, 3 * W, nk, &tkv));
  ARP_TRY(get_tmap_attn_out(h, out, (uint64_t)B, (uint64_t)tokens, (uint64_t)W, &to));
  ARP_TRY(get_tmap(h, qkv, rows, 3 * W, 3 * W, 16, &tq16));
  ARP_TRY(get_tmap_attn_out(h, out, (uint64_t)B, (uint64_t)tokens, (uint64_t)W, &to16, 16));
  const int grid = std::min(B * h->cfg.heads, kNumSMs);
  const int rev = h->dir ^= 1;
  if (tokens == 197)
    attention_tc_kernel<197><<<grid, ATC_THREADS, AtcCfg<197>::SMEM_BYTES, st>>>(*tq, *tkv, *to, *tq16, *to16, B, h->cfg.heads, W, scale_log2e, rev);
  else
    attention_tc_kernel<50><<<grid, ATC_THREADS, AtcCfg<50>::SMEM_BYTES, st>>>(*tq, *tkv, *to, *tq16, *to16, B, h->cfg.heads, W, scale_log2e, rev);
  h->launches++;
  ARP_CUDA(h, cudaGetLastError());
  return ARP_OK;
}

static int encode_chunk_f32(ArpHandle* h, const uint8_t* ob, int64_t n, int64_t stride, cudaStream_t st,
                            const float* chw, float* taps32);

template <typename XT>
static int last_block_cls(ArpHandle* h, const LayerW& L, const XT* x, int64_t n, cudaStream_t st, float* taps32) {
  const ArpConfig& c = h->cfg;
  ArpHandle::Work& ws = h->ws;
  const int W = c.width;
  const int64_t B = c.max_batch;
  gather_cls_rows_f32_kernel<768, XT><<<(unsigned)((n + 7) / 8), 256, 0, st>>>(x, ws.xcls, (int)n, h->tokens, W, 0);
  h->launches++;
  ARP_TRY(launch_ln_bf16(h, ws.xcls, L.ln1_g, L.ln1_b, ws.xncls, n, st));
  ARP_TRY(launch_gemm(h, ws.xncls, B, L.w_qkv, ws.qcls, false, ACT_NONE, n, W, W, W, L.b_qkv, nullptr, 0, nullptr, 0, st));
  {
    ProfScope prof(h, PC_ATTENTION, 4.0 * (double)n * c.heads * h->tokens * 64,
                   (double)n * h->tokens * W * 2 * 2 + (double)n * W * 2 * 2, st);
    const unsigned blocks = (unsigned)((n * c.heads + 7) / 8);
    if (h->tokens == 197)
      cls_attention_kernel<197><<<blocks, 256, 0, st>>>(ws.qcls, ws.qkv, ws.acls, (int)n, c.heads, W, 0.125f);
    else if (h->tokens == 50)
      cls_attention_kernel<50><<<blocks, 256, 0, st>>>(ws.qcls, ws.qkv, ws.acls, (int)n, c.heads, W, 0.125f);
    else
      return fail(h, ARP_ERR_INVALID, "attention is built for 197 or 50 tokens, got %d", h->tokens);
    h->launches++;
  }
  ARP_TRY(launch_gemm(h, ws.acls, B, L.w_out, ws.xcls, true, ACT_NONE, n, W, W, W, L.b_out, ws.xcls, W, nullptr, 0, st));
  ARP_TRY(launch_ln_bf16(h, ws.xcls, L.ln2_g, L.ln2_b, ws.xncls, n, st));
  ARP_TRY(launch_gemm(h, ws.xncls, B, L.w_fc, ws.hcls, false, ACT_QUICKGELU, n, 4 * W, W, 4 * W, L.b_fc, nullptr, 0,
                      nullptr, 0, st));
  ARP_TRY(launch_gemm(h, ws.hcls, B, L.w_proj, ws.xcls, true, ACT_NONE, n, W, 4 * W, W, L.b_proj, ws.xcls, W, nullptr,
                      0, st));
  const int l = c.layers - 1;
  if (h->adapter) {
    gather_cls_bf16_kernel<768, float><<<(unsigned)((n + 7) / 8), 256, 0, st>>>(ws.xcls, ws.taps, (int)n, 1, c.layers * W, l * W);
    h->launches++;
  }
  if (taps32) {
    gather_cls_rows_f32_kernel<768, float><<<(unsigned)((n + 7) / 8), 256, 0, st>>>(ws.xcls, taps32, (int)n, 1,
                                                                                 c.layers * W, l * W);
    h->launches++;
  }
  return ARP_OK;
}

template <typename XT>
static void gather_taps(ArpHandle* h, const XT* x, int64_t n, int l, cudaStream_t st, float* taps32) {
  const ArpConfig& c = h->cfg;
  if (h->adapter) {
    gather_cls_bf16_kernel<768, XT><<<(unsigned)((n + 7) / 8), 256, 0, st>>>(x, h->ws.taps, (int)n, h->tokens,
                                                                          c.layers * c.width, l * c.width);
    h->launches++;
  }
  if (taps32) {
    gather_cls_rows_f32_kernel<768, XT><<<(unsigned)((n + 7) / 8), 256, 0, st>>>(x, taps32, (int)n, h->tokens,
                                                                              c.layers * c.width, l * c.width);
    h->launches++;
  }
}

static int encode_blocks_r16(ArpHandle* h, int64_t n, cudaStream_t st, float* taps32) {
  const ArpConfig& c = h->cfg;
  ArpHandle::Work& ws = h->ws;
  const int W = c.width;
  const int64_t M = n * h->tokens, Mcap = (int64_t)c.max_batch * h->tokens;
  {
    ProfScope prof(h, PC_LAYERNORM, 0.0, (double)M * (768 * 6 + 8), st);
    layernorm_pre_r16_kernel<768><<<(unsigned)((M + 7) / 8), 256, 0, st>>>(ws.x, h->ln_pre_g, h->ln_pre_b, ws.x16,
                                                                          ws.stats, (int)M, 1e-5f);
    h->launches++;
  }
  int parts = 1;
  for (int l = 0; l < c.layers; ++l) {
    const LayerW& L = h->layers[l];
    if (l == c.layers - 1) {
      const LnFoldArgs f_kv{ws.stats, L.s_qkv + W, L.c_qkv + W, parts};
      ARP_TRY(launch_gemm(h, ws.x16, Mcap, L.w_qkv_fold + (size_t)W * W, ws.qkv + W, false, ACT_NONE, M, 2 * W, W, 3 * W,
                          nullptr, nullptr, 0, nullptr, 0, st, &f_kv));
      ARP_TRY(last_block_cls(h, L, ws.x16, n, st, taps32));
      break;
    }
    const LnFoldArgs f_qkv{ws.stats, L.s_qkv, L.c_qkv, parts};
    ARP_TRY(launch_gemm(h, ws.x16, Mcap, L.w_qkv_fold, ws.qkv, false, ACT_NONE, M, 3 * W, W, 3 * W, nullptr, nullptr, 0,
                        nullptr, 0, st, &f_qkv));
    parts = 2 * W / 256;
    const LnFoldArgs f_fc{ws.stats, L.s_fc, L.c_fc, parts};
    ARP_TRY(launch_attention(h, ws.qkv, ws.attn, (int)n, h->tokens, st, Mcap));
    ARP_TRY(launch_gemm(h, ws.attn, Mcap, L.w_out, ws.x16, false, ACT_NONE, M, W, W, W, L.b_out, ws.x16, W, nullptr, 0, st,
                        nullptr, ws.stats));
    ARP_TRY(launch_gemm(h, ws.x16, Mcap, L.w_fc_fold, ws.hid, false, ACT_QUICKGELU, M, 4 * W, W, 4 * W, nullptr, nullptr,
                        0, nullptr, 0, st, &f_fc));
    ARP_TRY(launch_gemm(h, ws.hid, Mcap, L.w_proj, ws.x16, false, ACT_NONE, M, W, 4 * W, W, L.b_proj, ws.x16, W, nullptr,
                        0, st, nullptr, ws.stats));
    gather_taps(h, ws.x16, n, l, st, taps32);
  }
  return ARP_OK;
}

static int encode_blocks_r32(ArpHandle* h, int64_t n, cudaStream_t st, float* taps32) {
  const ArpConfig& c = h->cfg;
  ArpHandle::Work& ws = h->ws;
  const int W = c.width;
  const int64_t M = n * h->tokens, Mcap = (int64_t)c.max_batch * h->tokens;
  {
    ProfScope prof(h, PC_LAYERNORM, 0.0, (double)M * 768 * 8, st);
    layernorm_f32_inplace_kernel<768><<<(unsigned)((M + 7) / 8), 256, 0, st>>>(ws.x, h->ln_pre_g, h->ln_pre_b, (int)M, 1e-5f);
    h->launches++;
  }
  for (int l = 0; l < c.layers; ++l) {
    const LayerW& L = h->layers[l];
    ARP_TRY(launch_ln_bf16(h, ws.x, L.ln1_g, L.ln1_b, ws.xn, M, st));
    if (l == c.layers - 1) {
      ARP_TRY(launch_gemm(h, ws.xn, Mcap, L.w_qkv + (size_t)W * W, ws.qkv + W, false, ACT_NONE, M, 2 * W, W, 3 * W,
                          L.b_qkv + W, nullptr, 0, nullptr, 0, st));
      ARP_TRY(last_block_cls(h, L, ws.x, n, st, taps32));
      break;
    }
    ARP_TRY(launch_gemm(h, ws.xn, Mcap, L.w_qkv, ws.qkv, false, ACT_NONE, M, 3 * W, W, 3 * W, L.b_qkv, nullptr, 0,
                        nullptr, 0, st));
    ARP_TRY(launch_attention(h, ws.qkv, ws.attn, (int)n, h->tokens, st, Mcap));
    ARP_TRY(launch_gemm(h, ws.attn, Mcap, L.w_out, ws.x, true, ACT_NONE, M, W, W, W, L.b_out, ws.x, W, nullptr, 0, st));
    ARP_TRY(launch_ln_bf16(h, ws.x, L.ln2_g, L.ln2_b, ws.xn, M, st));
    ARP_TRY(launch_gemm(h, ws.xn, Mcap, L.w_fc, ws.hid, false, ACT_QUICKGELU, M, 4 * W, W, 4 * W, L.b_fc, nullptr, 0,
                        nullptr, 0, st));
    ARP_TRY(launch_gemm(h, ws.hid, Mcap, L.w_proj, ws.x, true, ACT_NONE, M, W, 4 * W, W, L.b_proj, ws.x, W, nullptr, 0, st));
    gather_taps(h, ws.x, n, l, st, taps32);
  }
  return ARP_OK;
}

static int encode_chunk(ArpHandle* h, const uint8_t* ob, int64_t n, int64_t stride, cudaStream_t st,
                        const float* chw = nullptr, float* taps32 = nullptr) {
  if (h->f32) return encode_chunk_f32(h, ob, n, stride, st, chw, taps32);
  const ArpConfig& c = h->cfg;
  ArpHandle::Work& ws = h->ws;
  const int W = c.width;
  const int64_t M = n * h->tokens;
  const int64_t Mcap = (int64_t)c.max_batch * h->tokens;
  bf16* patches = ws.hid;
  if (chw) {
    ProfScope prof(h, PC_DECODE, 0.0, (double)n * (3.0 * DEC_OUT * DEC_OUT * 4 + (double)h->tokens * h->kp * 2), st);
    patchify_chw_bf16_kernel<<<kNumSMs * 8, 256, 0, st>>>(chw, patches, (int)n, c.patch, h->grid, h->tokens);
    h->launches++;
  } else {
    ARP_TRY(launch_decode(h, ob, n, stride, patches, DEC_OUT_PATCH_BF16, st));
  }
  ARP_TRY(launch_gemm(h, patches, Mcap, h->conv1, ws.x, true, ACT_NONE, M, W, h->kp, W, nullptr, nullptr, 0,
                      h->rowtab, h->tokens, st));
  ARP_TRY(h->resid16 ? encode_blocks_r16(h, n, st, taps32) : encode_blocks_r32(h, n, st, taps32));
  ARP_CUDA(h, cudaGetLastError());
  return ARP_OK;
}

static int launch_sgemm(ArpHandle* h, const float* a, int lda, const void* w, float* out, int ldo, int act, int64_t M,
                        int N, int K, const float* bias, const float* resid, int ldr, const float* rowtab, int period,
                        cudaStream_t st) {
  if (M <= 0) return ARP_OK;
  if (N % SG_BN || K % SG_BK) return fail(h, ARP_ERR_INVALID, "fp32 GEMM needs N %% 128 == 0 and K %% 16 == 0 (N=%d K=%d)", N, K);
  ProfScope prof(h, PC_GEMM, 2.0 * (double)M * N * K, ((double)M * K + (double)N * K + (double)M * N) * 4, st);
  dim3 grid(N / SG_BN, (unsigned)((M + SG_BM - 1) / SG_BM));
  sgemm_nt_f32_kernel<<<grid, SG_THREADS, 0, st>>>(a, static_cast<const float*>(w), out, (int)M, N, K, lda, ldo, bias,
                                                   resid, ldr, rowtab, period > 0 ? period : 1, act);
  h->launches++;
  ARP_CUDA(h, cudaGetLastError());
  return ARP_OK;
}

static int encode_chunk_f32(ArpHandle* h, const uint8_t* ob, int64_t n, int64_t stride, cudaStream_t st,
                            const float* chw, float* taps32) {
  const ArpConfig& c = h->cfg;
  ArpHandle::Work& ws = h->ws;
  const int W = c.width;
  const int64_t M = n * h->tokens;
  if (h->tokens != 197 && h->tokens != 50) return fail(h, ARP_ERR_INVALID, "unsupported token count %d", h->tokens);
  float* patches = ws.hid32;
  if (!chw) ARP_TRY(launch_decode(h, ob, n, stride, ws.chw32, DEC_OUT_CHW_F32, st));
  im2col_f32_kernel<<<kNumSMs * 8, 256, 0, st>>>(chw ? chw : ws.chw32, patches, (int)n, c.patch, h->grid, h->tokens);
  h->launches++;
  ARP_TRY(launch_sgemm(h, patches, h->kp, h->conv1, ws.x, W, F32_ACT_NONE, M, W, h->kp, nullptr, nullptr, 0, h->rowtab,
                       h->tokens, st));
  auto ln = [&](const float* x, const float* g, const float* b, float* y) {
    ProfScope prof(h, PC_LAYERNORM, 0.0, (double)M * W * 8, st);
    layernorm_f32_f32_kernel<768><<<(unsigned)((M + 7) / 8), 256, 0, st>>>(x, g, b, y, (int)M, 1e-5f);
    h->launches++;
  };
  ln(ws.x, h->ln_pre_g, h->ln_pre_b, ws.x);
  for (int l = 0; l < c.layers; ++l) {
    const LayerW& L = h->layers[l];
    ln(ws.x, L.ln1_g, L.ln1_b, ws.xn32);
    ARP_TRY(launch_sgemm(h, ws.xn32, W, L.w_qkv, ws.qkv32, 3 * W, F32_ACT_NONE, M, 3 * W, W, L.b_qkv, nullptr, 0, nullptr,
                         0, st));
    {
      ProfScope prof(h, PC_ATTENTION, 4.0 * (double)n * c.heads * h->tokens * h->tokens * 64, (double)M * W * 4 * 4, st);
      for (int64_t b0 = 0; b0 < n; b0 += 32768) {
        const int cnt = (int)std::min<int64_t>(32768, n - b0);
        attention_f32_kernel<<<dim3(c.heads, cnt), A32_THREADS, attn_f32_smem_bytes(h->tokens), st>>>(
            ws.qkv32 + (size_t)b0 * h->tokens * 3 * W, ws.attn32 + (size_t)b0 * h->tokens * W, h->tokens, W);
        h->launches++;
      }
    }
    ARP_TRY(launch_sgemm(h, ws.attn32, W, L.w_out, ws.x, W, F32_ACT_NONE, M, W, W, L.b_out, ws.x, W, nullptr, 0, st));
    ln(ws.x, L.ln2_g, L.ln2_b, ws.xn32);
    ARP_TRY(launch_sgemm(h, ws.xn32, W, L.w_fc, ws.hid32, 4 * W, F32_ACT_QUICKGELU, M, 4 * W, W, L.b_fc, nullptr, 0,
                         nullptr, 0, st));
    ARP_TRY(launch_sgemm(h, ws.hid32, 4 * W, L.w_proj, ws.x, W, F32_ACT_NONE, M, W, 4 * W, L.b_proj, ws.x, W, nullptr, 0,
                         st));
    if (h->adapter) {
      gather_cls_rows_f32_kernel<768, float><<<(unsigned)((n + 7) / 8), 256, 0, st>>>(ws.x, ws.taps32, (int)n, h->tokens,
                                                                        c.layers * W, l * W);
      h->launches++;
    }
    if (taps32) {
      gather_cls_rows_f32_kernel<768, float><<<(unsigned)((n + 7) / 8), 256, 0, st>>>(ws.x, taps32, (int)n, h->tokens,
                                                                        c.layers * W, l * W);
      h->launches++;
    }
  }
  ARP_CUDA(h, cudaGetLastError());
  return ARP_OK;
}

static void adapter_clip_feature(ArpHandle* h, int64_t n, cudaStream_t st) {
  const ArpConfig& c = h->cfg;
  ArpHandle::Work& ws = h->ws;
  const float* xsrc = h->f32 ? ws.x : ws.xcls;
  const int xtok = h->f32 ? h->tokens : 1;
  clip_head_kernel<768, 512><<<(unsigned)((n + HEAD_FR - 1) / HEAD_FR), 256, HEAD_SMEM_BYTES, st>>>(
      xsrc, xtok, h->ln_post_g, h->ln_post_b, 1e-5f, h->proj, nullptr, 0, nullptr, 0, 0.f, 0, ws.featf, h->feat_dim,
      c.layers * c.embed_dim, nullptr, nullptr, 0, (int)n);
  h->launches++;
}

static int adapter_tail(ArpHandle* h, int64_t n, float* reward_out, int64_t ld, float* logits_out, float* feat_out,
                        cudaStream_t st) {
  const ArpConfig& c = h->cfg;
  ArpHandle::Work& ws = h->ws;
  const bool need_text = reward_out || logits_out;
  const int D = h->feat_dim, Dmid = c.layers * c.embed_dim, Din = c.layers * c.width;
  const int64_t B = c.max_batch;
  if (h->f32) {
    ARP_TRY(launch_sgemm(h, ws.taps32, Din, h->inter_w, ws.featf, D, F32_ACT_NONE, n, Dmid, Din, nullptr, nullptr, 0,
                         nullptr, 0, st));
    ARP_TRY(launch_sgemm(h, ws.featf, D, h->fc1_w, ws.hid2_32, 2 * D, F32_ACT_RELU, n, 2 * D, D, h->fc1_b, nullptr, 0,
                         nullptr, 0, st));
    ARP_TRY(launch_sgemm(h, ws.hid2_32, 2 * D, h->fc2_w, ws.mlp, D, F32_ACT_NONE, n, D, 2 * D, h->fc2_b, nullptr, 0,
                         nullptr, 0, st));
// ... 787 lines not shown
  const int blocks = (int)std::min<int64_t>((n + 255) / 256, kNumSMs * 8);
  radix_select_init_kernel<<<1, 256, 0, st>>>(&sd->sel, k0, k1);
  h->launches++;
  for (int pass = 0; pass < 4; ++pass) {
    radix_select_hist_kernel<<<blocks, 256, 0, st>>>(x, n, &sd->sel, pass);
    radix_select_pick_kernel<<<1, 256, 0, st>>>(&sd->sel, pass, res2);
    h->launches += 2;
  }
  ARP_CUDA(h, cudaGetLastError());
  return ARP_OK;
}

extern "C" int arp_quantile_f32(ArpHandle* h, const float* x_dev, int64_t n, int64_t k_lo, int64_t k_hi,
                                float* lo_hi_host, void* stream) {
  if (!h || !x_dev || !lo_hi_host) return fail(h, ARP_ERR_INVALID, "null argument");
  if (n < 1 || k_lo < 0 || k_hi < 0 || k_lo >= n || k_hi >= n) return fail(h, ARP_ERR_INVALID, "ranks must be in [0, n)");
  cudaStream_t st = static_cast<cudaStream_t>(stream);
  ARP_CUDA(h, cudaSetDevice(h->cfg.device));
  ARP_TRY(ensure_stats(h));
  StatsDev* sd = static_cast<StatsDev*>(h->stats_dev);
  ProfScope prof(h, PC_SCAN, 0.0, (double)n * 4 * 4, st);
  ARP_TRY(launch_select(h, x_dev, n, (uint64_t)k_lo, (uint64_t)k_hi, sd->res + 4, st));
  ARP_CUDA(h, cudaMemcpyAsync(lo_hi_host, sd->res + 4, 8, cudaMemcpyDeviceToHost, st));
  ARP_CUDA(h, cudaStreamSynchronize(st));
  return ARP_OK;
}

extern "C" int arp_preprocess_rtgs(ArpHandle* h, const float* reward_dev, int64_t T, const int64_t* ep_offsets_dev,
                                   int32_t n_eps, int32_t num_frames, int32_t use_normalize, float* shifted_dev,
                                   float* rtg_dev, float* rtg_stacked_dev, float* stats_host, void* stream) {
  if (!h || !reward_dev || !ep_offsets_dev || !rtg_dev || !rtg_stacked_dev || !stats_host)
    return fail(h, ARP_ERR_INVALID, "null argument");
  if (T < 1 || n_eps < 1) return fail(h, ARP_ERR_INVALID, "empty dataset");
  if (use_normalize && !shifted_dev) return fail(h, ARP_ERR_INVALID, "use_normalize needs a [T] scratch buffer");
  cudaStream_t st = static_cast<cudaStream_t>(stream);
  ARP_CUDA(h, cudaSetDevice(h->cfg.device));
  ARP_TRY(ensure_stats(h));
  StatsDev* sd = static_cast<StatsDev*>(h->stats_dev);
  ARP_TRY(launch_minmax(h, reward_dev, T, sd->res, st));
  const float* r = reward_dev;
  if (use_normalize) {
    sub_scalar_f32_kernel<<<(int)std::min<int64_t>((T + 255) / 256, kNumSMs * 8), 256, 0, st>>>(reward_dev, sd->res,
                                                                                              shifted_dev, T);
    h->launches++;
    r = shifted_dev;
  }
  ARP_TRY(scan_launch(h, r, T, ep_offsets_dev, n_eps, num_frames, 1.0f, rtg_dev, nullptr, rtg_stacked_dev, st));
  int64_t off_last = 0;
  ARP_CUDA(h, cudaMemcpyAsync(&off_last, ep_offsets_dev + n_eps, 8, cudaMemcpyDeviceToHost, st));
  ARP_CUDA(h, cudaStreamSynchronize(st));
  const int64_t rows = std::min<int64_t>(off_last, T);
  if (rows < 1) return fail(h, ARP_ERR_INVALID, "no labeled rows");
  ARP_TRY(launch_minmax(h, rtg_dev, rows, sd->res + 2, st));
  ARP_CUDA(h, cudaMemcpyAsync(stats_host, sd->res, 16, cudaMemcpyDeviceToHost, st));
  ARP_CUDA(h, cudaStreamSynchronize(st));
  return ARP_OK;
}

extern "C" int arp_online_reward(ArpHandle* h, const uint8_t* ob_host, int32_t n, float* reward_host,
                                 float* logits_host, float* feat_host) {
  if (!h) return ARP_ERR_INVALID;
  cudaStream_t st = h->own_stream;
  const ArpConfig& c = h->cfg;
  const size_t frame_bytes = (size_t)c.in_h * c.in_w * 3;
  if (n < 1 || n > c.max_batch) return fail(h, ARP_ERR_INVALID, "n must be in [1, max_batch=%d]", c.max_batch);
  ARP_TRY(check_ready(h, ob_host, n, (int64_t)frame_bytes, st));
  const bool text_head = !h->goal;
  if (text_head && !h->text) return fail(h, ARP_ERR_STATE, "arp_set_text has not been called");
  if (h->n_groups > 1)
    return fail(h, ARP_ERR_INVALID, "the online reward scores one instruction set: call arp_set_text (%d groups are set)",
                h->n_groups);
  if (!text_head && (reward_host || logits_host))
    return fail(h, ARP_ERR_INVALID, "goal-conditioned heads produce features only (reward = -||f - f_goal||, vl_reward.py:26-41)");
  ARP_TRY(ensure_stage(h));
  const size_t per = 1 + HEAD_MAX_TEXT + (size_t)h->feat_dim;
  if (!h->online_out) ARP_TRY(dev_alloc(h, &h->online_out, per * c.max_batch));
  float* d_r = h->online_out;
  float* d_lg = d_r + c.max_batch;
  float* d_f = d_lg + (size_t)c.max_batch * HEAD_MAX_TEXT;
  auto run = [&]() -> int {
    ARP_TRY(encode_chunk(h, h->stage_dev[0], n, (int64_t)frame_bytes, st));
    ARP_TRY(head_chunk(h, n, text_head ? d_r : nullptr, n, text_head ? d_lg : nullptr, d_f, st));
    if (h->adapter) {
      l2_normalize_rows_kernel<<<(unsigned)((n + 7) / 8), 256, 0, st>>>(d_f, h->feat_dim, n);
      h->launches++;
    }
    return ARP_OK;
  };
  ARP_CUDA(h, cudaMemcpyAsync(h->stage_dev[0], ob_host, frame_bytes * n, cudaMemcpyHostToDevice, st));
  if (h->profiling) {
    ARP_TRY(run());
  } else {
    ArpHandle::OnlineGraph& g = h->online_graphs[n];
    if (!g.exec || g.epoch != h->online_epoch) {
      if (g.exec) { cudaGraphExecDestroy(g.exec); g.exec = nullptr; }
      const int64_t l0 = h->launches;
      cudaGraph_t graph = nullptr;
      ARP_CUDA(h, cudaStreamBeginCapture(st, cudaStreamCaptureModeThreadLocal));
      const int rc = run();
      const cudaError_t e = cudaStreamEndCapture(st, &graph);
      if (rc != ARP_OK) { if (graph) cudaGraphDestroy(graph); return rc; }
      if (e != cudaSuccess) return fail(h, ARP_ERR_CUDA, "graph capture failed: %s", cudaGetErrorString(e));
      const cudaError_t ei = cudaGraphInstantiate(&g.exec, graph, 0);
      cudaGraphDestroy(graph);
      if (ei != cudaSuccess) { g.exec = nullptr; return fail(h, ARP_ERR_CUDA, "cudaGraphInstantiate failed: %s", cudaGetErrorString(ei)); }
      g.launches = h->launches - l0;
      g.epoch = h->online_epoch;
      h->launches = l0;
    }
    ARP_CUDA(h, cudaGraphLaunch(g.exec, st));
    h->launches += g.launches;
  }
  if (reward_host) ARP_CUDA(h, cudaMemcpyAsync(reward_host, d_r, (size_t)n * 4, cudaMemcpyDeviceToHost, st));
  if (logits_host) ARP_CUDA(h, cudaMemcpyAsync(logits_host, d_lg, (size_t)n * h->n_text * 4, cudaMemcpyDeviceToHost, st));
  if (feat_host) ARP_CUDA(h, cudaMemcpyAsync(feat_host, d_f, (size_t)n * h->feat_dim * 4, cudaMemcpyDeviceToHost, st));
  ARP_CUDA(h, cudaStreamSynchronize(st));
  return ARP_OK;
}

extern "C" int arp_decode_only(ArpHandle* h, const uint8_t* ob_dev, int64_t T, int64_t row_stride_bytes,
                               float* chw_dev, void* stream) {
  if (!h || !chw_dev || (T > 0 && !ob_dev)) return fail(h, ARP_ERR_INVALID, "null argument");
  ARP_CUDA(h, cudaSetDevice(h->cfg.device));
  return launch_decode(h, ob_dev, T, row_stride_bytes, chw_dev, DEC_OUT_CHW_F32, static_cast<cudaStream_t>(stream));
}

extern "C" int arp_gemm_bf16(ArpHandle* h, const void* a_dev, const void* w_dev, void* out_dev, int32_t out_dtype,
                             int64_t M, int32_t N, int32_t K, const float* bias_dev, const void* resid_dev,
                             int32_t act, void* stream) {
  if (!h || !a_dev || !w_dev || !out_dev) return fail(h, ARP_ERR_INVALID, "null argument");
  if (act < 0 || act > 2 || (out_dtype != ARP_F32 && out_dtype != ARP_OP_DTYPE)) return fail(h, ARP_ERR_INVALID, "bad act / out_dtype");
  ARP_CUDA(h, cudaSetDevice(h->cfg.device));
  return launch_gemm(h, static_cast<const bf16*>(a_dev), M, static_cast<const bf16*>(w_dev), out_dev,
                     out_dtype == ARP_F32, act, M, N, K, N, bias_dev, resid_dev, N, nullptr, 0,
                     static_cast<cudaStream_t>(stream));
}

extern "C" int arp_resid_gemm_stats(ArpHandle* h, const void* a_dev, const void* w_dev, const float* bias_dev, void* x_dev,
                                    float* stats_dev, int64_t M, int32_t N, int32_t K, void* stream) {
  if (!h || !a_dev || !w_dev || !bias_dev || !x_dev || !stats_dev) return fail(h, ARP_ERR_INVALID, "null argument");
  ARP_CUDA(h, cudaSetDevice(h->cfg.device));
  cudaStream_t st = static_cast<cudaStream_t>(stream);
  const int nparts = 2 * N / 256;
  ARP_TRY(ensure_scratch(h, 0, (size_t)M * nparts * sizeof(float2) + 256));
  float2* parts = reinterpret_cast<float2*>(h->scratch[0]);
  ARP_TRY(launch_gemm(h, static_cast<const bf16*>(a_dev), M, static_cast<const bf16*>(w_dev), x_dev, false, ACT_NONE, M, N, K,
                      N, bias_dev, x_dev, N, nullptr, 0, st, nullptr, parts));
  merge_row_stats_kernel<<<(unsigned)((M + 255) / 256), 256, 0, st>>>(parts, nparts, reinterpret_cast<float2*>(stats_dev), (int)M, 1e-5f);
  h->launches++;
  ARP_CUDA(h, cudaGetLastError());
  return ARP_OK;
}

extern "C" int arp_ln_gemm(ArpHandle* h, const void* x_dev, const float* gamma_dev, const float* beta_dev,
                           const float* w_f32_dev, const float* bias_dev, void* out_dev, int64_t M, int32_t N,
                           int32_t act, void* stream) {
  if (!h || !x_dev || !gamma_dev || !beta_dev || !w_f32_dev || !bias_dev || !out_dev) return fail(h, ARP_ERR_INVALID, "null argument");
  if (act != ACT_NONE && act != ACT_QUICKGELU) return fail(h, ARP_ERR_INVALID, "bad act");
  if (M < 1 || N < 256 || N % 256) return fail(h, ARP_ERR_INVALID, "bad M / N");
  ARP_CUDA(h, cudaSetDevice(h->cfg.device));
  cudaStream_t st = static_cast<cudaStream_t>(stream);
  const int K = 768;
  uint8_t* tmp = nullptr;
  const size_t b_w = (size_t)N * K * sizeof(bf16), b_v = (size_t)N * 4, b_s = (size_t)M * sizeof(float2);
  auto al = [](size_t b) { return (b + 255) & ~static_cast<size_t>(255); };
  ARP_CUDA(h, cudaMalloc((void**)&tmp, al(b_w) + 2 * al(b_v) + al(b_s)));
  bf16* wf = reinterpret_cast<bf16*>(tmp);
  float* svec = reinterpret_cast<float*>(tmp + al(b_w));
  float* cvec = reinterpret_cast<float*>(tmp + al(b_w) + al(b_v));
  float2* stats = reinterpret_cast<float2*>(tmp + al(b_w) + 2 * al(b_v));
  fold_ln_weights_kernel<<<(N + 7) / 8, 256, 0, st>>>(w_f32_dev, gamma_dev, beta_dev, bias_dev, wf, svec, cvec, N, K);
  h->launches++;
  int rc = launch_row_moments(h, static_cast<const bf16*>(x_dev), stats, M, st);
  const LnFoldArgs f{stats, svec, cvec};
  if (rc == ARP_OK)
    rc = launch_gemm(h, static_cast<const bf16*>(x_dev), M, wf, out_dev, false, act, M, N, K, N, nullptr, nullptr, 0,
                     nullptr, 0, st, &f);
  cudaStreamSynchronize(st);
  h->tmaps.clear();
  cudaFree(tmp);
  return rc;
}

extern "C" int arp_layernorm_bf16(ArpHandle* h, const float* x_dev, const float* gamma_dev, const float* beta_dev,
                                  void* y_dev, int64_t M, void* stream) {
  if (!h || !x_dev || !gamma_dev || !beta_dev || !y_dev) return fail(h, ARP_ERR_INVALID, "null argument");
  ARP_CUDA(h, cudaSetDevice(h->cfg.device));
  return launch_ln_bf16(h, x_dev, gamma_dev, beta_dev, static_cast<bf16*>(y_dev), M, static_cast<cudaStream_t>(stream));
}

extern "C" int arp_attention(ArpHandle* h, const void* qkv_dev, void* out_dev, int32_t B, int32_t tokens,
                             void* stream) {
  if (!h || !qkv_dev || !out_dev) return fail(h, ARP_ERR_INVALID, "null argument");
  ARP_CUDA(h, cudaSetDevice(h->cfg.device));
  return launch_attention(h, static_cast<const bf16*>(qkv_dev), static_cast<bf16*>(out_dev), B, tokens,
                          static_cast<cudaStream_t>(stream));
}

#ifdef ARP_ATTN_TRACE
extern "C" __attribute__((visibility("default"))) int arp_debug_attn_trace(long long* out, int cap) {
  const int n = 2 * ATC_TR_ITEMS * ATC_TR_EVENTS;
  cudaDeviceSynchronize();
  if (cap < n) return -1;
  cudaMemcpyFromSymbol(out, g_attn_trace, (size_t)n * sizeof(long long));
  return n;
}
#endif
```

### arp_b200/csrc/common.cuh

```cuda
#pragma once

#include <cuda.h>
#include <cuda_bf16.h>
#include <cuda_fp16.h>
#include <cuda_runtime.h>
#include <stdint.h>

#ifndef ARP_WATCHDOG_CYCLES
#define ARP_WATCHDOG_CYCLES (5ll * 1000 * 1000 * 1000)
#endif

namespace arp {

constexpr int kNumSMs = 148;

__device__ __forceinline__ uint32_t smem_u32(const void* p) {
  return static_cast<uint32_t>(__cvta_generic_to_shared(p));
}

__device__ __forceinline__ uint32_t lane_id() { return threadIdx.x & 31; }

__device__ __forceinline__ bool elect_one() {
  uint32_t pred = 0;
  asm volatile(
      "{\n\t"
      ".reg .pred p;\n\t"
      "elect.sync _|p, 0xffffffff;\n\t"
      "selp.u32 %0, 1, 0, p;\n\t"
      "}\n"
      : "=r"(pred));
  return pred != 0;
}

__device__ __forceinline__ float warp_sum(float v) {
#pragma unroll
  for (int o = 16; o > 0; o >>= 1) v += __shfl_xor_sync(0xffffffffu, v, o);
  return v;
}

__device__ __forceinline__ float warp_max(float v) {
#pragma unroll
  for (int o = 16; o > 0; o >>= 1) v = fmaxf(v, __shfl_xor_sync(0xffffffffu, v, o));
  return v;
}

#ifndef ARP_OP_FP16
#define ARP_OP_FP16 1
#endif
#if ARP_OP_FP16
using op_t = __half;
using op2_t = __half2;
constexpr uint32_t kOpFormat = 0;
__device__ __forceinline__ op2_t floats_to_op2(float lo, float hi) { return __floats2half2_rn(lo, hi); }
__device__ __forceinline__ op_t float_to_op(float v) { return __float2half_rn(v); }
__device__ __forceinline__ float op_to_float(op_t v) { return __half2float(v); }
#else
using op_t = __nv_bfloat16;
using op2_t = __nv_bfloat162;
constexpr uint32_t kOpFormat = 1;
__device__ __forceinline__ op2_t floats_to_op2(float lo, float hi) { return __floats2bfloat162_rn(lo, hi); }
__device__ __forceinline__ op_t float_to_op(float v) { return __float2bfloat16_rn(v); }
__device__ __forceinline__ float op_to_float(op_t v) { return __bfloat162float(v); }
#endif

__device__ __forceinline__ uint32_t pack_op(float lo, float hi) {
  op2_t v = floats_to_op2(lo, hi);
  return *reinterpret_cast<uint32_t*>(&v);
}

__device__ __forceinline__ uint64_t f32x2_pack(float lo, float hi) {
  uint64_t r;
  asm("mov.b64 %0, {%1, %2};" : "=l"(r) : "f"(lo), "f"(hi));
  return r;
}
__device__ __forceinline__ void f32x2_unpack(uint64_t v, float& lo, float& hi) {
  asm("mov.b64 {%0, %1}, %2;" : "=f"(lo), "=f"(hi) : "l"(v));
}
__device__ __forceinline__ uint64_t f32x2_fma(uint64_t a, uint64_t b, uint64_t c) {
  uint64_t d;
  asm("fma.rn.f32x2 %0, %1, %2, %3;" : "=l"(d) : "l"(a), "l"(b), "l"(c));
  return d;
}
__device__ __forceinline__ uint64_t f32x2_mul(uint64_t a, uint64_t b) {
  uint64_t d;
  asm("mul.rn.f32x2 %0, %1, %2;" : "=l"(d) : "l"(a), "l"(b));
  return d;
}
__device__ __forceinline__ uint64_t f32x2_add(uint64_t a, uint64_t b) {
  uint64_t d;
  asm("add.rn.f32x2 %0, %1, %2;" : "=l"(d) : "l"(a), "l"(b));
  return d;
}

__device__ __forceinline__ void mbar_init(uint64_t* bar, uint32_t count) {
  asm volatile("mbarrier.init.shared::cta.b64 [%0], %1;" ::"r"(smem_u32(bar)), "r"(count) : "memory");
}

__device__ __forceinline__ void fence_mbar_init() {
  asm volatile("fence.mbarrier_init.release.cluster;" ::: "memory");
}

__device__ __forceinline__ void mbar_arrive(uint64_t* bar) {
  asm volatile("mbarrier.arrive.shared::cta.b64 _, [%0];" ::"r"(smem_u32(bar)) : "memory");
}

__device__ __forceinline__ void mbar_arrive_expect_tx(uint64_t* bar, uint32_t bytes) {
  asm volatile("mbarrier.arrive.expect_tx.shared::cta.b64 _, [%0], %1;" ::"r"(smem_u32(bar)), "r"(bytes)
               : "memory");
}

__device__ __forceinline__ bool mbar_try_wait(uint64_t* bar, uint32_t parity) {
  uint32_t ok;
  asm volatile(
      "{\n\t"
      ".reg .pred p;\n\t"
      "mbarrier.try_wait.parity.shared::cta.b64 p, [%1], %2;\n\t"
      "selp.u32 %0, 1, 0, p;\n\t"
      "}\n"
      : "=r"(ok)
      : "r"(smem_u32(bar)), "r"(parity)
      : "memory");
  return ok != 0;
}

__device__ __forceinline__ bool mbar_test_wait(uint64_t* bar, uint32_t parity) {
  uint32_t ok;
  asm volatile(
      "{\n\t"
      ".reg .pred p;\n\t"
      "mbarrier.test_wait.parity.shared::cta.b64 p, [%1], %2;\n\t"
      "selp.u32 %0, 1, 0, p;\n\t"
      "}\n"
      : "=r"(ok)
      : "r"(smem_u32(bar)), "r"(parity)
      : "memory");
  return ok != 0;
}

__device__ __forceinline__ void mbar_wait(uint64_t* bar, uint32_t parity) {
  if (mbar_try_wait(bar, parity)) return;
  const long long t0 = clock64();
  while (!mbar_try_wait(bar, parity)) {
    if (clock64() - t0 > ARP_WATCHDOG_CYCLES) {
      printf("arp_b200: mbarrier watchdog (block %d thread %d bar %u parity %u)\n", blockIdx.x, threadIdx.x,
             smem_u32(bar), parity);
      __trap();
    }
  }
}

__device__ __forceinline__ int lds_volatile(const volatile int* p) {
  int v;
  asm volatile("ld.volatile.shared.s32 %0, [%1];" : "=r"(v) : "r"(smem_u32(const_cast<const int*>(p))) : "memory");
  return v;
}
__device__ __forceinline__ void sts_volatile(volatile int* p, int v) {
  asm volatile("st.volatile.shared.s32 [%0], %1;" ::"r"(smem_u32(const_cast<int*>(p))), "r"(v) : "memory");
}
__device__ __forceinline__ int atoms_add(int* p, int v) {
  int old;
  asm volatile("atom.shared.add.s32 %0, [%1], %2;" : "=r"(old) : "r"(smem_u32(p)), "r"(v) : "memory");
  return old;
}

__device__ __forceinline__ void tma_prefetch_desc(const CUtensorMap* m) {
  asm volatile("prefetch.tensormap [%0];" ::"l"(reinterpret_cast<uint64_t>(m)) : "memory");
}

__device__ __forceinline__ void tma_load_2d(void* dst, const CUtensorMap* m, uint64_t* bar, int c0, int c1) {
  asm volatile(
      "cp.async.bulk.tensor.2d.shared::cluster.global.mbarrier::complete_tx::bytes [%0], [%1, {%3, %4}], [%2];"
      ::"r"(smem_u32(dst)),
      "l"(reinterpret_cast<uint64_t>(m)), "r"(smem_u32(bar)), "r"(c0), "r"(c1)
      : "memory");
}

__device__ __forceinline__ void tma_store_2d(const CUtensorMap* m, const void* src, int c0, int c1) {
  asm volatile("cp.async.bulk.tensor.2d.global.shared::cta.bulk_group [%0, {%2, %3}], [%1];" ::"l"(
                   reinterpret_cast<uint64_t>(m)),
               "r"(smem_u32(src)), "r"(c0), "r"(c1)
               : "memory");
}
__device__ __forceinline__ void tma_store_3d(const CUtensorMap* m, const void* src, int c0, int c1, int c2) {
  asm volatile("cp.async.bulk.tensor.3d.global.shared::cta.bulk_group [%0, {%2, %3, %4}], [%1];" ::"l"(
                   reinterpret_cast<uint64_t>(m)),
               "r"(smem_u32(src)), "r"(c0), "r"(c1), "r"(c2)
               : "memory");
}
__device__ __forceinline__ void tma_prefetch_l2_2d(const CUtensorMap* m, int c0, int c1) {
  asm volatile("cp.async.bulk.prefetch.tensor.2d.L2.global.tile [%0, {%1, %2}];" ::"l"(reinterpret_cast<uint64_t>(m)), "r"(c0),
               "r"(c1)
               : "memory");
}
__device__ __forceinline__ void tma_store_commit() { asm volatile("cp.async.bulk.commit_group;" ::: "memory"); }
template <int N>
__device__ __forceinline__ void tma_store_wait_read() {
  asm volatile("cp.async.bulk.wait_group.read %0;" ::"n"(N) : "memory");
}
template <int N>
__device__ __forceinline__ void tma_store_wait_all() {
  asm volatile("cp.async.bulk.wait_group %0;" ::"n"(N) : "memory");
}
__device__ __forceinline__ void fence_proxy_async_all() { asm volatile("fence.proxy.async;" ::: "memory"); }
__device__ __forceinline__ void named_bar_sync(int id, int count) {
  asm volatile("bar.sync %0, %1;" ::"r"(id), "r"(count) : "memory");
}
__device__ __forceinline__ void fence_proxy_async_smem() {
  asm volatile("fence.proxy.async.shared::cta;" ::: "memory");
}

template <int kCols>
__device__ __forceinline__ void tmem_alloc(uint32_t* dst_smem) {
  asm volatile("tcgen05.alloc.cta_group::1.sync.aligned.shared::cta.b32 [%0], %1;" ::"r"(smem_u32(dst_smem)),
               "n"(kCols)
               : "memory");
  asm volatile("tcgen05.relinquish_alloc_permit.cta_group::1.sync.aligned;" ::: "memory");
}
template <int kCols>
__device__ __forceinline__ void tmem_dealloc(uint32_t addr) {
  asm volatile("tcgen05.dealloc.cta_group::1.sync.aligned.b32 %0, %1;" ::"r"(addr), "n"(kCols) : "memory");
}
__device__ __forceinline__ void tc_fence_before() { asm volatile("tcgen05.fence::before_thread_sync;" ::: "memory"); }
__device__ __forceinline__ void tc_fence_after() { asm volatile("tcgen05.fence::after_thread_sync;" ::: "memory"); }

__device__ __forceinline__ void umma_bf16_ss(uint32_t d_tmem, uint64_t a_desc, uint64_t b_desc, uint32_t idesc,
                                             uint32_t accumulate) {
  asm volatile(
      "{\n\t"
      ".reg .pred p;\n\t"
      "setp.ne.b32 p, %4, 0;\n\t"
      "tcgen05.mma.cta_group::1.kind::f16 [%0], %1, %2, %3, p;\n\t"
      "}\n" ::"r"(d_tmem),
      "l"(a_desc), "l"(b_desc), "r"(idesc), "r"(accumulate)
      : "memory");
}

__device__ __forceinline__ void umma_commit(uint64_t* bar) {
  asm volatile("tcgen05.commit.cta_group::1.mbarrier::arrive::one.shared::cluster.b64 [%0];" ::"r"(smem_u32(bar))
               : "memory");
}

__device__ __forceinline__ void tmem_ld_32x32(uint32_t taddr, uint32_t (&r)[32]) {
  asm volatile(
      "tcgen05.ld.sync.aligned.32x32b.x32.b32 "
      "{%0, %1, %2, %3, %4, %5, %6, %7, %8, %9, %10, %11, %12, %13, %14, %15, "
      "%16, %17, %18, %19, %20, %21, %22, %23, %24, %25, %26, %27, %28, %29, %30, %31}, [%32];"
// ... 94 lines not shown
```

### arp_b200/csrc/gemm_tcgen05.cuh

```cuda
#pragma once

#include "common.cuh"

namespace arp {

enum GemmAct : int { ACT_NONE = 0, ACT_QUICKGELU = 1, ACT_RELU = 2 };
enum G2Mode : int { G2_STORE = 0, G2_REDUCE = 1, G2_LNFOLD = 2, G2_RESID_STATS = 3 };

struct GemmArgs {
  int M, N, K;
  void* out;
  int ldo;
  const float* bias;
  const float* rowtab;
  int period;
  int reverse;
  const float2* ln_stats;
  int ln_nparts;
  const float* svec;
  const float* cvec;
  const op_t* resid;
  int ldr;
  float2* stats_out;
  float eps;
};

constexpr int GEMM_BM = 128;
constexpr int GEMM_BN = 256;
constexpr int GEMM_BK = 64;
constexpr int GEMM_A_BYTES = GEMM_BM * GEMM_BK * 2;

__device__ __forceinline__ float quick_gelu(float x) {
  float t;
  asm("tanh.approx.f32 %0, %1;" : "=f"(t) : "f"(0.851f * x));
  const float h = 0.5f * x;
  return fmaf(h, t, h);
}

constexpr int G2_THREADS = 320;
constexpr int G2_EPI_WARPS = 8;
constexpr int G2_STAGE_UNIT = 32 * 128;
constexpr int G2_STAGING_BYTES = G2_EPI_WARPS * G2_STAGE_UNIT;

template <int CG>
struct G2Cfg {
  static constexpr int B_ROWS = GEMM_BN / CG;
  static constexpr int STAGE_BYTES = GEMM_A_BYTES + B_ROWS * GEMM_BK * 2;
  static constexpr int STAGES = CG == 1 ? 3 : 6;
  static constexpr int SMEM_BYTES = STAGES * STAGE_BYTES + G2_STAGING_BYTES + 1024 + 256;
};

template <typename OutT, int ACT, int CG, int MODE>
__global__ void __launch_bounds__(G2_THREADS, 1)
gemm_tcgen05_kernel(const __grid_constant__ CUtensorMap tmap_a, const __grid_constant__ CUtensorMap tmap_b,
                    const __grid_constant__ CUtensorMap tmap_out, const GemmArgs args) {
  using Cfg = G2Cfg<CG>;
  constexpr int STAGES = Cfg::STAGES;
  extern __shared__ uint8_t smem_raw[];
  uint8_t* smem = reinterpret_cast<uint8_t*>((reinterpret_cast<uintptr_t>(smem_raw) + 1023) & ~uintptr_t(1023));
  uint8_t* staging = smem + STAGES * Cfg::STAGE_BYTES;
  uint64_t* bars = reinterpret_cast<uint64_t*>(staging + G2_STAGING_BYTES);
  uint64_t* full_bar = bars;
  uint64_t* empty_bar = bars + STAGES;
  uint64_t* tfull_bar = bars + 2 * STAGES;
  uint64_t* tempty_bar = tfull_bar + 2;
  uint32_t* tmem_slot = reinterpret_cast<uint32_t*>(tempty_bar + 2);
  static_assert(MODE != G2_RESID_STATS || sizeof(OutT) == 2, "G2_RESID_STATS updates the 16-bit residual stream");

  const int warp = __shfl_sync(0xffffffffu, static_cast<int>(threadIdx.x >> 5), 0);
  const int lane = threadIdx.x & 31;
  const uint32_t rank = CG == 2 ? cluster_ctarank() : 0;
  const int cluster_id = blockIdx.x / CG;
  const int num_clusters = gridDim.x / CG;

  const int num_m = (args.M + GEMM_BM * CG - 1) / (GEMM_BM * CG);
  const int num_n = args.N / GEMM_BN;
  const int num_tiles = num_m * num_n;
  const int num_kb = args.K / GEMM_BK;
  const int my_tiles = cluster_id < num_tiles ? (num_tiles - cluster_id + num_clusters - 1) / num_clusters : 0;
  auto tile_coords = [&](int it, int& m_blk, int& n_blk) {
    const int tile = cluster_id + it * num_clusters;
    const int tile_o = args.reverse ? num_tiles - 1 - tile : tile;
    m_blk = tile_o / num_n;
    n_blk = tile_o % num_n;
  };

  if (warp == 0 && lane == 0) {
    tma_prefetch_desc(&tmap_a);
    tma_prefetch_desc(&tmap_b);
    tma_prefetch_desc(&tmap_out);
  }
  if (warp == 1 && lane == 0) {
    for (int i = 0; i < STAGES; ++i) {
      mbar_init(&full_bar[i], 1);
      mbar_init(&empty_bar[i], 1);
    }
    for (int i = 0; i < 2; ++i) {
      mbar_init(&tfull_bar[i], 1);
      mbar_init(&tempty_bar[i], G2_EPI_WARPS * CG);
    }
    fence_mbar_init();
  }
  if (warp == 1) {
    if (CG == 1) tmem_alloc<512>(tmem_slot); else tmem_alloc_cg2<512>(tmem_slot);
  }
  tc_fence_before();
  if (CG == 2) cluster_sync_all(); else __syncthreads();
  tc_fence_after();
  const uint32_t tmem_base = __shfl_sync(0xffffffffu, *tmem_slot, 0);

  if (warp == 0) {
    if (elect_one()) {
      int stage = 0;
      uint32_t phase = 0;
      for (int it = 0; it < my_tiles; ++it) {
        int m_blk, n_blk;
        tile_coords(it, m_blk, n_blk);
        const int a_row = (m_blk * CG + rank) * GEMM_BM;
        const int b_row = n_blk * GEMM_BN + rank * Cfg::B_ROWS;
        for (int kb = 0; kb < num_kb; ++kb) {
          mbar_wait(&empty_bar[stage], phase ^ 1);
          uint8_t* sa = smem + stage * Cfg::STAGE_BYTES;
          uint8_t* sb = sa + GEMM_A_BYTES;
          if (CG == 1) {
            mbar_arrive_expect_tx(&full_bar[stage], Cfg::STAGE_BYTES);
            tma_load_2d(sa, &tmap_a, &full_bar[stage], kb * GEMM_BK, a_row);
            tma_load_2d(sb, &tmap_b, &full_bar[stage], kb * GEMM_BK, b_row);
          } else {
            if (rank == 0) mbar_arrive_expect_tx(&full_bar[stage], 2 * Cfg::STAGE_BYTES);
            const uint32_t leader_bar = mapa_u32(smem_u32(&full_bar[stage]), 0);
            tma_load_2d_cg2(sa, &tmap_a, leader_bar, kb * GEMM_BK, a_row);
            tma_load_2d_cg2(sb, &tmap_b, leader_bar, kb * GEMM_BK, b_row);
          }
          if (++stage == STAGES) { stage = 0; phase ^= 1; }
        }
      }
    }
  } else if (warp == 1) {
    if (rank == 0 && elect_one()) {
      constexpr uint32_t idesc = umma_idesc_bf16(GEMM_BM * CG, GEMM_BN);
      int stage = 0;
      uint32_t phase = 0;
      int acc = 0;
      uint32_t acc_phase = 0;
      for (int it = 0; it < my_tiles; ++it) {
        mbar_wait(&tempty_bar[acc], acc_phase ^ 1);
        tc_fence_after();
        const uint32_t d_tmem = tmem_base + acc * GEMM_BN;
        for (int kb = 0; kb < num_kb; ++kb) {
          mbar_wait(&full_bar[stage], phase);
          tc_fence_after();
          const uint32_t sa = smem_u32(smem + stage * Cfg::STAGE_BYTES);
          const uint64_t da = umma_desc_kmajor_sw128(sa);
          const uint64_t db = umma_desc_kmajor_sw128(sa + GEMM_A_BYTES);
#pragma unroll
          for (int k = 0; k < GEMM_BK / 16; ++k) {
            if (CG == 1) umma_bf16_ss(d_tmem, da + 2 * k, db + 2 * k, idesc, (kb | k) != 0);
            else umma_bf16_ss_cg2(d_tmem, da + 2 * k, db + 2 * k, idesc, (kb | k) != 0);
          }
          if (CG == 1) {
            umma_commit(&empty_bar[stage]);
            if (kb == num_kb - 1) umma_commit(&tfull_bar[acc]);
          } else {
            umma_commit_cg2(&empty_bar[stage], 0b11);
            if (kb == num_kb - 1) umma_commit_cg2(&tfull_bar[acc], 0b11);
          }
          if (++stage == STAGES) { stage = 0; phase ^= 1; }
        }
        if (++acc == 2) { acc = 0; acc_phase ^= 1; }
      }
    }
  } else {
    const int ew = warp - 2;
    const int quarter = warp & 3;
    const int half = ew >> 2;
    uint8_t* sbuf = staging + ew * G2_STAGE_UNIT;
    constexpr int UNIT_COLS = sizeof(OutT) == 4 ? 32 : 64;
    constexpr int UNITS = 128 / UNIT_COLS;
    const uint32_t tempty_leader0 = CG == 2 ? mapa_u32(smem_u32(&tempty_bar[0]), 0) : 0;
    const uint32_t tempty_leader1 = CG == 2 ? mapa_u32(smem_u32(&tempty_bar[1]), 0) : 0;
    int acc = 0;
    uint32_t acc_phase = 0;
    const int sw = lane & 7;
    for (int it = 0; it < my_tiles; ++it) {
      int m_blk, n_blk;
      tile_coords(it, m_blk, n_blk);
      const int row0 = (m_blk * CG + rank) * GEMM_BM + quarter * 32;
      const int row = row0 + lane;
      uint4 xo[MODE == G2_RESID_STATS ? 16 : 1];
      float st_n = 0.f, st_mean = 0.f, st_m2 = 0.f;
      if (MODE == G2_RESID_STATS) {
#pragma unroll
        for (int c = 0; c < 16; ++c) {
          const int r = row0 + 4 * (c & 7) + (lane >> 3);
          const op_t* xp = args.resid + static_cast<size_t>(r) * args.ldr + n_blk * GEMM_BN + half * 128 + (c >> 3) * 64 + (lane & 7) * 8;
          xo[c] = r < args.M ? *reinterpret_cast<const uint4*>(xp) : make_uint4(0u, 0u, 0u, 0u);
        }
        if (lane == 0 && it + 1 < my_tiles) {
          int m2, n2;
          tile_coords(it + 1, m2, n2);
          const int r2 = (m2 * CG + rank) * GEMM_BM + quarter * 32, c2 = n2 * GEMM_BN + half * 128;
          tma_prefetch_l2_2d(&tmap_out, c2, r2);
          tma_prefetch_l2_2d(&tmap_out, c2 + 64, r2);
        }
      }
      float ln_rstd = 1.f, ln_rm = 0.f;
      if (MODE == G2_LNFOLD && row < args.M) {
        if (args.ln_nparts == 1) {
          const float2 p = __ldg(args.ln_stats + row);
          ln_rstd = p.x;
          ln_rm = p.y;
        } else {
          const float2* pp = args.ln_stats + static_cast<size_t>(row) * args.ln_nparts;
          float mean = 0.f, m2 = 0.f;
          if (args.ln_nparts == 6) {
            const float4 a = __ldg(reinterpret_cast<const float4*>(pp));
            const float4 b = __ldg(reinterpret_cast<const float4*>(pp) + 1);
            const float4 c = __ldg(reinterpret_cast<const float4*>(pp) + 2);
            mean = ((a.x + a.z) + (b.x + b.z) + (c.x + c.z)) * (1.0f / 6.0f);
            const float d0 = a.x - mean, d1 = a.z - mean, d2 = b.x - mean, d3 = b.z - mean, d4 = c.x - mean, d5 = c.z - mean;
            m2 = ((a.y + a.w) + (b.y + b.w) + (c.y + c.w)) +
                 128.0f * ((d0 * d0 + d1 * d1) + (d2 * d2 + d3 * d3) + (d4 * d4 + d5 * d5));
          } else {
            for (int i = 0; i < args.ln_nparts; ++i) mean += __ldg(pp + i).x;
            mean *= 1.0f / static_cast<float>(args.ln_nparts);
            for (int i = 0; i < args.ln_nparts; ++i) {
              const float2 p = __ldg(pp + i);
              const float d = p.x - mean;
              m2 += fmaf(128.0f * d, d, p.y);
            }
          }
          ln_rstd = rsqrtf(m2 / (128.0f * static_cast<float>(args.ln_nparts)) + args.eps);
          ln_rm = -mean * ln_rstd;
        }
      }
      mbar_wait(&tfull_bar[acc], acc_phase);
      tc_fence_after();
      const uint32_t taddr = tmem_base + acc * GEMM_BN + half * 128 + (static_cast<uint32_t>(quarter * 32) << 16);
      const float* tab_row =
          args.rowtab ? args.rowtab + static_cast<size_t>(row % args.period) * args.N : nullptr;
#pragma unroll(MODE == G2_RESID_STATS ? UNITS : 1)
      for (int u = 0; u < UNITS; ++u) {
        const int n0 = n_blk * GEMM_BN + half * 128 + u * UNIT_COLS;
        if (MODE == G2_RESID_STATS) {
          if (lane == 0) tma_store_wait_read<0>();
          __syncwarp();
#pragma unroll
          for (int i = 0; i < 8; ++i) {
            const int r = 4 * i + (lane >> 3);
            *reinterpret_cast<uint4*>(sbuf + r * 128 + (((lane & 7) ^ (r & 7)) << 4)) = xo[u * 8 + i];
          }
          __syncwarp();
          uint4* srow = reinterpret_cast<uint4*>(sbuf + lane * 128);
#pragma unroll
          for (int hh = 0; hh < 2; ++hh) {
            uint32_t r[32];
            tmem_ld_32x32(taddr + u * 64 + hh * 32, r);
            tmem_ld_wait();
            if (u == UNITS - 1 && hh == 1) {
              tc_fence_before();
              __syncwarp();
              if (lane == 0) {
                if (CG == 1) mbar_arrive_relaxed(&tempty_bar[acc]);
                else mbar_arrive_cluster_relaxed(acc ? tempty_leader1 : tempty_leader0);
              }
            }
            float y[32];
            float s1 = 0.f;
#pragma unroll
            for (int c = 0; c < 4; ++c) {
              const uint4 q = srow[(hh * 4 + c) ^ sw];
              const uint32_t w4[4] = {q.x, q.y, q.z, q.w};
              const float4 b0 = __ldg(reinterpret_cast<const float4*>(args.bias + n0 + hh * 32 + 8 * c));
              const float4 b1 = __ldg(reinterpret_cast<const float4*>(args.bias + n0 + hh * 32 + 8 * c + 4));
              const float bb[8] = {b0.x, b0.y, b0.z, b0.w, b1.x, b1.y, b1.z, b1.w};
              uint32_t pk[4];
#pragma unroll
              for (int e = 0; e < 4; ++e) {
                const op2_t xh = *reinterpret_cast<const op2_t*>(&w4[e]);
                const op2_t yh = floats_to_op2(__uint_as_float(r[8 * c + 2 * e]) + bb[2 * e] + op_to_float(xh.x),
                                               __uint_as_float(r[8 * c + 2 * e + 1]) + bb[2 * e + 1] + op_to_float(xh.y));
                pk[e] = *reinterpret_cast<const uint32_t*>(&yh);
                y[8 * c + 2 * e] = op_to_float(yh.x);
                y[8 * c + 2 * e + 1] = op_to_float(yh.y);
                s1 += y[8 * c + 2 * e] + y[8 * c + 2 * e + 1];
              }
              srow[(hh * 4 + c) ^ sw] = make_uint4(pk[0], pk[1], pk[2], pk[3]);
            }
            const float mu = s1 * (1.0f / 32.0f);
            float m2 = 0.f;
#pragma unroll
            for (int j = 0; j < 32; ++j) {
              const float d = y[j] - mu;
              m2 = fmaf(d, d, m2);
            }
            const float nt = st_n + 32.0f;
            const float d = mu - st_mean, f = __fdividef(32.0f, nt);
            st_mean = fmaf(d, f, st_mean);
            st_m2 += fmaf(d * d, st_n * f, m2);
            st_n = nt;
          }
          fence_proxy_async_smem();
          __syncwarp();
          if (lane == 0) {
            tma_store_2d(&tmap_out, sbuf, n0, row0);
            tma_store_commit();
          }
          continue;
        }
        float v[UNIT_COLS];
        {
          uint32_t r[32];
          tmem_ld_32x32(taddr + u * UNIT_COLS, r);
          if (UNIT_COLS == 64) {
            uint32_t r2[32];
            tmem_ld_32x32(taddr + u * UNIT_COLS + 32, r2);
            tmem_ld_wait();
#pragma unroll
            for (int j = 0; j < 32; ++j) v[(UNIT_COLS == 64 ? 32 : 0) + j] = __uint_as_float(r2[j]);
          } else {
            tmem_ld_wait();
          }
#pragma unroll
          for (int j = 0; j < 32; ++j) v[j] = __uint_as_float(r[j]);
        }
        if (u == UNITS - 1) {
          tc_fence_before();
          __syncwarp();
          if (lane == 0) {
            if (CG == 1) mbar_arrive_relaxed(&tempty_bar[acc]);
            else mbar_arrive_cluster_relaxed(acc ? tempty_leader1 : tempty_leader0);
          }
        }
        if (MODE == G2_LNFOLD) {
#pragma unroll
          for (int j = 0; j < UNIT_COLS; j += 4) {
            const float4 sv = __ldg(reinterpret_cast<const float4*>(args.svec + n0 + j));
            const float4 cv = __ldg(reinterpret_cast<const float4*>(args.cvec + n0 + j));
            v[j] = fmaf(ln_rstd, v[j], fmaf(ln_rm, sv.x, cv.x));
            v[j + 1] = fmaf(ln_rstd, v[j + 1], fmaf(ln_rm, sv.y, cv.y));
            v[j + 2] = fmaf(ln_rstd, v[j + 2], fmaf(ln_rm, sv.z, cv.z));
            v[j + 3] = fmaf(ln_rstd, v[j + 3], fmaf(ln_rm, sv.w, cv.w));
          }
        } else if (args.bias) {
#pragma unroll
          for (int j = 0; j < UNIT_COLS; j += 4) {
            const float4 b = __ldg(reinterpret_cast<const float4*>(args.bias + n0 + j));
            v[j] += b.x; v[j + 1] += b.y; v[j + 2] += b.z; v[j + 3] += b.w;
          }
        }
        if (tab_row) {
#pragma unroll
          for (int j = 0; j < UNIT_COLS; j += 4) {
            const float4 b = __ldg(reinterpret_cast<const float4*>(tab_row + n0 + j));
            v[j] += b.x; v[j + 1] += b.y; v[j + 2] += b.z; v[j + 3] += b.w;
          }
        }
        if (ACT == ACT_QUICKGELU) {
#pragma unroll
          for (int j = 0; j < UNIT_COLS; ++j) v[j] = quick_gelu(v[j]);
        } else if (ACT == ACT_RELU) {
#pragma unroll
          for (int j = 0; j < UNIT_COLS; ++j) v[j] = fmaxf(v[j], 0.0f);
        }
        if (lane == 0) tma_store_wait_read<0>();
        __syncwarp();
        uint4* srow = reinterpret_cast<uint4*>(sbuf + lane * 128);
#pragma unroll
        for (int c = 0; c < 8; ++c) {
          uint4 q;
          if (sizeof(OutT) == 4) {
            q = make_uint4(__float_as_uint(v[4 * c]), __float_as_uint(v[4 * c + 1]), __float_as_uint(v[4 * c + 2]),
                           __float_as_uint(v[4 * c + 3]));
          } else {
            q = make_uint4(pack_op(v[8 * c], v[8 * c + 1]), pack_op(v[8 * c + 2], v[8 * c + 3]),
                           pack_op(v[8 * c + 4], v[8 * c + 5]), pack_op(v[8 * c + 6], v[8 * c + 7]));
          }
          srow[c ^ sw] = q;
        }
        fence_proxy_async_smem();
        __syncwarp();
        if (lane == 0) {
          if (MODE == G2_REDUCE) tma_reduce_add_2d(&tmap_out, sbuf, n0, row0);
          else tma_store_2d(&tmap_out, sbuf, n0, row0);
          tma_store_commit();
        }
      }
      if (MODE == G2_RESID_STATS && row < args.M)
        args.stats_out[static_cast<size_t>(row) * (2 * num_n) + n_blk * 2 + half] = make_float2(st_mean, st_m2);
      if (++acc == 2) { acc = 0; acc_phase ^= 1; }
    }
    if (lane == 0) tma_store_wait_all<0>();
  }

  tc_fence_before();
  if (CG == 2) cluster_sync_all(); else __syncthreads();
  if (warp == 1) {
    tc_fence_after();
    if (CG == 1) tmem_dealloc<512>(tmem_base); else tmem_dealloc_cg2<512>(tmem_base);
  }
}

}
```

### include/arp_b200.h

```cpp
#ifndef ARP_B200_H_
#define ARP_B200_H_

#include <stdint.h>

#ifdef __cplusplus
extern "C" {
#endif

#define ARP_B200_ABI_VERSION 9

#define ARP_MAX_TEXT 16
#define ARP_MAX_TEXT_GROUPS 16
#define ARP_MAX_TEXT_TOTAL 64

#if defined(__GNUC__)
#define ARP_API __attribute__((visibility("default")))
#else
#define ARP_API
#endif

typedef enum ArpStatus {
  ARP_OK = 0,
  ARP_ERR_INVALID = -1,
  ARP_ERR_CUDA = -2,
  ARP_ERR_STATE = -3,
  ARP_ERR_NO_DEVICE = -4,
  ARP_ERR_UNKNOWN_KEY = -5
} ArpStatus;

typedef enum ArpInflateStatus {
  ARP_INFLATE_OK = 0,
  ARP_INFLATE_TRUNCATED = 1,
  ARP_INFLATE_BAD_HEADER = 2,
  ARP_INFLATE_BAD_BLOCK = 3,
  ARP_INFLATE_BAD_CODE = 4,
  ARP_INFLATE_DISTANCE_TOO_FAR = 5,
  ARP_INFLATE_TOO_LONG = 6,
  ARP_INFLATE_TOO_SHORT = 7,
  ARP_INFLATE_BAD_ADLER = 8
} ArpInflateStatus;

typedef enum ArpPreprocess { ARP_PRE_PIL_BICUBIC = 0, ARP_PRE_BILINEAR = 1 } ArpPreprocess;
typedef enum ArpHead {
  ARP_HEAD_CLIP = 0,
  ARP_HEAD_ADAPTER = 1,
  ARP_HEAD_ADAPTER_ENSEMBLE = 2,
  ARP_HEAD_CLIP_GOAL = 3,
  ARP_HEAD_ADAPTER_GOAL = 4
} ArpHead;
typedef enum ArpReduce { ARP_REDUCE_FIRST = 0, ARP_REDUCE_MEAN = 1 } ArpReduce;

typedef enum ArpDType { ARP_F32 = 0, ARP_BF16 = 1, ARP_F16 = 2 } ArpDType;
typedef enum ArpPrecision { ARP_PREC_BF16 = 0, ARP_PREC_F32 = 1, ARP_PREC_F32RESID = 2 } ArpPrecision;

typedef struct ArpHandle ArpHandle;

typedef struct ArpConfig {
  int32_t struct_size;
  int32_t device;
  int32_t patch;
  int32_t width;
  int32_t layers;
  int32_t heads;
  int32_t embed_dim;
  int32_t in_h, in_w;
  int32_t use_crop;
  int32_t preprocess;
  int32_t head;
  int32_t reduce;
  int32_t max_batch;
  int32_t precision;
} ArpConfig;

ARP_API int arp_create(const ArpConfig* cfg, ArpHandle** out);
ARP_API void arp_destroy(ArpHandle* h);
ARP_API const char* arp_last_error(const ArpHandle* h);
ARP_API int arp_abi_version(void);
ARP_API int arp_operand_dtype(void);

ARP_API int arp_set_weight(ArpHandle* h, const char* name, const void* data, int32_t dtype, const int64_t* shape,
                   int32_t ndim, void* stream);
ARP_API int arp_wants_weight(const ArpHandle* h, const char* name);
ARP_API int arp_missing_weights(const ArpHandle* h, char* names_out, int64_t names_cap);

ARP_API int arp_set_text(ArpHandle* h, const float* text_emb_dev, int32_t n_text, int32_t dim, float logit_scale_exp,
                 void* stream);
ARP_API int arp_set_text_groups(ArpHandle* h, const float* text_emb_dev, int32_t n_text_total, int32_t dim,
                        const int32_t* group_offsets_host, int32_t n_groups, float logit_scale_exp, void* stream);
ARP_API int arp_text_groups(const ArpHandle* h);

ARP_API int arp_label(ArpHandle* h, const uint8_t* ob_dev, int64_t T, int64_t row_stride_bytes,
              const int64_t* ep_offsets_dev, int32_t n_eps, int32_t num_frames, float* reward_dev, float* rtg_dev,
              float* reward_stacked_dev, float* rtg_stacked_dev, void* stream);

ARP_API int arp_label_host(ArpHandle* h, const uint8_t* ob_host, int64_t T, int64_t row_stride_bytes,
                   const int64_t* ep_offsets_host, int32_t n_eps, int32_t num_frames, float* reward_host,
                   float* rtg_host, float* reward_stacked_host, float* rtg_stacked_host);

ARP_API int arp_label_file(ArpHandle* h, int32_t fd, int64_t file_offset, int64_t T, int64_t row_stride_bytes,
                   const int64_t* ep_offsets_host, int32_t n_eps, int32_t num_frames, float* reward_host,
                   float* rtg_host, float* reward_stacked_host, float* rtg_stacked_host);

ARP_API int arp_embedding_dim(const ArpHandle* h);
ARP_API int arp_embed_host(ArpHandle* h, const uint8_t* ob_host, int64_t T, int64_t row_stride_bytes, float* emb_host);
ARP_API int arp_embed_file(ArpHandle* h, int32_t fd, int64_t file_offset, int64_t T, int64_t row_stride_bytes,
                           float* emb_host);
ARP_API int arp_label_embeddings(ArpHandle* h, const float* emb_dev, int64_t T, const int64_t* ep_offsets_dev,
                                 int32_t n_eps, int32_t num_frames, float* reward_dev, float* rtg_dev,
                                 float* reward_stacked_dev, float* rtg_stacked_dev, void* stream);

ARP_API int arp_tower_dim(const ArpHandle* h);
ARP_API int arp_embed_tower_host(ArpHandle* h, const uint8_t* ob_host, int64_t T, int64_t row_stride_bytes,
                                 float* rec_host);
ARP_API int arp_embed_tower_file(ArpHandle* h, int32_t fd, int64_t file_offset, int64_t T, int64_t row_stride_bytes,
                                 float* rec_host);

ARP_API int arp_label_zfile(ArpHandle* h, int32_t fd, const int64_t* chunk_offset_host, const int64_t* chunk_bytes_host,
                            int64_t T, int64_t row_bytes, const int64_t* ep_offsets_host, int32_t n_eps,
                            int32_t num_frames, float* reward_host, float* rtg_host, float* reward_stacked_host,
                            float* rtg_stacked_host);
ARP_API int arp_embed_zfile(ArpHandle* h, int32_t fd, const int64_t* chunk_offset_host, const int64_t* chunk_bytes_host,
                            int64_t T, int64_t row_bytes, float* emb_host);
ARP_API int arp_embed_tower_zfile(ArpHandle* h, int32_t fd, const int64_t* chunk_offset_host,
                                  const int64_t* chunk_bytes_host, int64_t T, int64_t row_bytes, float* rec_host);
ARP_API int arp_inflate_rows(ArpHandle* h, const uint8_t* src_dev, const int64_t* src_off_dev,
                             const int64_t* src_bytes_dev, int64_t n, int64_t row_bytes, uint8_t* out_dev,
                             int32_t* status_dev, void* stream);
ARP_API int arp_label_tower(ArpHandle* h, const float* rec_dev, int64_t T, const int64_t* ep_offsets_dev,
                            int32_t n_eps, int32_t num_frames, float* reward_dev, float* rtg_dev,
                            float* reward_stacked_dev, float* rtg_stacked_dev, void* stream);

ARP_API int arp_online_reward(ArpHandle* h, const uint8_t* ob_host, int32_t n, float* reward_host, float* logits_host,
                      float* feat_host);

ARP_API int arp_preprocess_rtgs(ArpHandle* h, const float* reward_dev, int64_t T, const int64_t* ep_offsets_dev,
                        int32_t n_eps, int32_t num_frames, int32_t use_normalize, float* shifted_dev, float* rtg_dev,
                        float* rtg_stacked_dev, float* stats_host, void* stream);
ARP_API int arp_quantile_f32(ArpHandle* h, const float* x_dev, int64_t n, int64_t k_lo, int64_t k_hi, float* lo_hi_host,
                     void* stream);

ARP_API int arp_compute_reward(ArpHandle* h, const uint8_t* ob_dev, int64_t T, int64_t row_stride_bytes, float* reward_dev,
                       float* logits_dev, void* stream);

ARP_API int arp_encode_image(ArpHandle* h, const uint8_t* ob_dev, int64_t T, int64_t row_stride_bytes, float* feat_dev,
                     void* stream);

ARP_API int arp_encode_taps_chw(ArpHandle* h, const float* chw_dev, int64_t T, float* taps_dev, float* feat_dev,
                        void* stream);

ARP_API int arp_decode_only(ArpHandle* h, const uint8_t* ob_dev, int64_t T, int64_t row_stride_bytes, float* chw_dev,
                    void* stream);
ARP_API int arp_scan_only(ArpHandle* h, const float* reward_dev, int64_t T, const int64_t* ep_offsets_dev, int32_t n_eps,
                  int32_t num_frames, float gamma, float* rtg_dev, float* reward_stacked_dev,
                  float* rtg_stacked_dev, void* stream);
ARP_API int arp_gemm_bf16(ArpHandle* h, const void* a_dev, const void* w_dev, void* out_dev, int32_t out_dtype, int64_t M,
                  int32_t N, int32_t K, const float* bias_dev, const void* resid_dev, int32_t act, void* stream);
ARP_API int arp_resid_gemm_stats(ArpHandle* h, const void* a_dev, const void* w_dev, const float* bias_dev, void* x_dev,
                         float* stats_dev, int64_t M, int32_t N, int32_t K, void* stream);
ARP_API int arp_ln_gemm(ArpHandle* h, const void* x_dev, const float* gamma_dev, const float* beta_dev, const float* w_f32_dev,
                const float* bias_dev, void* out_dev, int64_t M, int32_t N, int32_t act, void* stream);
ARP_API int arp_layernorm_bf16(ArpHandle* h, const float* x_dev, const float* gamma_dev, const float* beta_dev, void* y_dev,
                       int64_t M, void* stream);
ARP_API int arp_attention(ArpHandle* h, const void* qkv_dev, void* out_dev, int32_t B, int32_t tokens, void* stream);

ARP_API int64_t arp_launch_count(const ArpHandle* h);

typedef struct ArpProfileStats {
  int64_t launches;
  double total_ms;
  double flops;
  double bytes;
} ArpProfileStats;
#define ARP_PROFILE_CLASSES 7
ARP_API int arp_profile_begin(ArpHandle* h);
ARP_API int arp_profile_end(ArpHandle* h, ArpProfileStats* stats, int32_t n_classes);

#ifdef __cplusplus
}
#endif
#endif
```

Measured before the change: 30400.

## Fuse MLP fc and proj GEMMs into one persistent tcgen05 kernel

Replaces the separate LN-folded fc GEMM and residual proj GEMM in each transformer layer with a single clustered persistent kernel. Each cluster writes a band of hidden activations to a small per-cluster scratch region, then runs the proj GEMM on it using per-slice mbarriers, so the full 4W hidden tensor never makes a complete round trip through HBM. Leftover rows that do not fill a wave run through the old two-GEMM path on a side stream using the SMs the fused kernel leaves free. The cost is a more complex kernel with intra-CTA producer/consumer sync, a fixed 56-cluster grid, and extra tensor-map arguments on every GEMM launch.

```diff
diff --git a/arp_b200/build.py b/arp_b200/build.py
--- a/arp_b200/build.py
+++ b/arp_b200/build.py
@@ -86,7 +86,7 @@
     digest = _sources_digest()
     if JITTER_LIB.exists() and stamp.exists() and stamp.read_text().split() == [digest, _file_digest(JITTER_LIB)]:
         return JITTER_LIB
-    build_variant(JITTER_LIB, ["ARP_ATTN_JITTER"])
+    build_variant(JITTER_LIB, ["ARP_ATTN_JITTER", "ARP_MLP_JITTER"])
     stamp.write_text(f"{digest} {_file_digest(JITTER_LIB)}")
     return JITTER_LIB
 
diff --git a/arp_b200/capi.py b/arp_b200/capi.py
--- a/arp_b200/capi.py
+++ b/arp_b200/capi.py
@@ -31,7 +31,7 @@
     "arp_set_text", "arp_label", "arp_label_host", "arp_compute_reward", "arp_encode_image", "arp_decode_only",
     "arp_scan_only", "arp_gemm_bf16", "arp_layernorm_bf16", "arp_attention", "arp_launch_count",
     "arp_profile_begin", "arp_profile_end", "arp_online_reward", "arp_preprocess_rtgs",
-    "arp_quantile_f32", "arp_encode_taps_chw", "arp_operand_dtype", "arp_ln_gemm", "arp_resid_gemm_stats", "arp_label_file", "arp_wants_weight",
+    "arp_quantile_f32", "arp_encode_taps_chw", "arp_operand_dtype", "arp_ln_gemm", "arp_resid_gemm_stats", "arp_mlp_r16", "arp_label_file", "arp_wants_weight",
     "arp_set_text_groups", "arp_text_groups", "arp_embedding_dim", "arp_embed_host", "arp_embed_file",
     "arp_label_embeddings", "arp_tower_dim", "arp_embed_tower_host", "arp_embed_tower_file", "arp_label_tower",
     "arp_label_zfile", "arp_embed_zfile", "arp_embed_tower_zfile", "arp_inflate_rows",
@@ -117,6 +117,7 @@
     lib.arp_gemm_bf16.argtypes = [vp, vp, vp, vp, i32, i64, i32, i32, vp, vp, i32, vp]
     lib.arp_ln_gemm.argtypes = [vp, vp, vp, vp, vp, vp, vp, i64, i32, i32, vp]
     lib.arp_resid_gemm_stats.argtypes = [vp, vp, vp, vp, vp, vp, i64, i32, i32, vp]
+    lib.arp_mlp_r16.argtypes = [vp, vp, vp, vp, vp, vp, vp, vp, vp, i64, i32, vp]
     lib.arp_layernorm_bf16.argtypes = [vp, vp, vp, vp, vp, i64, vp]
     lib.arp_attention.argtypes = [vp, vp, vp, i32, i32, vp]
     lib.arp_launch_count.argtypes = [vp]
@@ -553,6 +554,20 @@
                                                    _stream_ptr(self.device)))
         return stats
 
+    def mlp_r16(self, x: torch.Tensor, stats_in: torch.Tensor, w_fc_fold: torch.Tensor, svec: torch.Tensor,
+                cvec: torch.Tensor, w_proj: torch.Tensor, b_proj: torch.Tensor, unfused: bool = False) -> torch.Tensor:
+        op = operand_dtype()
+        assert x.dtype == op and x.is_contiguous() and x.device == self.device and x.shape[1] == 768
+        M = x.shape[0]
+        f = lambda t: t.to(self.device, torch.float32).contiguous()
+        stats_in, svec, cvec, b_proj = f(stats_in), f(svec), f(cvec), f(b_proj)
+        w_fc_fold, w_proj = w_fc_fold.to(op).contiguous(), w_proj.to(op).contiguous()
+        stats_out = torch.empty(M, 6, 2, device=self.device, dtype=torch.float32)
+        self._check(self._lib.arp_mlp_r16(self._h, _ptr(x), _ptr(stats_in), _ptr(w_fc_fold), _ptr(svec), _ptr(cvec),
+                                          _ptr(w_proj), _ptr(b_proj), _ptr(stats_out), M, int(unfused),
+                                          _stream_ptr(self.device)))
+        return stats_out
+
     def ln_gemm(self, x: torch.Tensor, gamma, beta, w: torch.Tensor, bias: torch.Tensor, act: int = ACT_NONE) -> torch.Tensor:
         op = operand_dtype()
         x = x.to(op).contiguous()
diff --git a/arp_b200/csrc/attention_tc.cuh b/arp_b200/csrc/attention_tc.cuh
--- a/arp_b200/csrc/attention_tc.cuh
+++ b/arp_b200/csrc/attention_tc.cuh
@@ -137,12 +137,7 @@
 }
 
 #ifdef ARP_ATTN_JITTER
-__device__ __forceinline__ void atc_jitter(uint32_t salt) {
-  uint32_t h = (static_cast<uint32_t>(clock64()) ^ (salt * 2654435761u) ^ (threadIdx.x >> 5) * 40503u ^ blockIdx.x * 9176u);
-  h ^= h >> 13; h *= 0x5bd1e995u; h ^= h >> 15;
-  if (h & 1) __nanosleep((h >> 1) & 8191);
-}
-#define ATC_JITTER(salt) atc_jitter(salt)
+#define ATC_JITTER(salt) jitter_sleep(salt)
 #else
 #define ATC_JITTER(salt)
 #endif
diff --git a/arp_b200/csrc/capi.cu b/arp_b200/csrc/capi.cu
--- a/arp_b200/csrc/capi.cu
+++ b/arp_b200/csrc/capi.cu
@@ -158,6 +158,8 @@
   size_t pin_bytes = 0;
   cudaEvent_t ev_slot[8] = {nullptr, nullptr, nullptr, nullptr, nullptr, nullptr, nullptr, nullptr};
   cudaStream_t copy_stream = nullptr, own_stream = nullptr;
+  cudaStream_t mlp_stream = nullptr;
+  cudaEvent_t ev_mlp_fork = nullptr, ev_mlp_join = nullptr;
   cudaEvent_t ev_copied[2] = {nullptr, nullptr}, ev_consumed[2] = {nullptr, nullptr};
 
   std::map<TmapKey, CUtensorMap> tmaps;
@@ -480,6 +482,9 @@
   for (cudaEvent_t e : h->event_pool) cudaEventDestroy(e);
   if (h->copy_stream) cudaStreamDestroy(h->copy_stream);
   if (h->own_stream) cudaStreamDestroy(h->own_stream);
+  if (h->mlp_stream) cudaStreamDestroy(h->mlp_stream);
+  if (h->ev_mlp_fork) cudaEventDestroy(h->ev_mlp_fork);
+  if (h->ev_mlp_join) cudaEventDestroy(h->ev_mlp_join);
   delete h;
 }
 
@@ -598,6 +603,7 @@
   G2_ATTR(float, ACT_NONE, G2_STORE) G2_ATTR(float, ACT_QUICKGELU, G2_STORE) G2_ATTR(float, ACT_RELU, G2_STORE)
   G2_ATTR(float, ACT_NONE, G2_REDUCE) G2_ATTR(bf16, ACT_NONE, G2_REDUCE)
   G2_ATTR(bf16, ACT_NONE, G2_LNFOLD) G2_ATTR(bf16, ACT_QUICKGELU, G2_LNFOLD) G2_ATTR(bf16, ACT_NONE, G2_RESID_STATS)
+  G2_ATTR(bf16, ACT_QUICKGELU, G2_MLP)
 #undef G2_ATTR
   CREATE_TRY(set_smem(h, attention_tc_kernel<197>, AtcCfg<197>::SMEM_BYTES));
   CREATE_TRY(set_smem(h, attention_tc_kernel<50>, AtcCfg<50>::SMEM_BYTES));
@@ -605,7 +611,10 @@
   CREATE_TRY(set_smem(h, clip_head_kernel<768, 512>, HEAD_SMEM_BYTES));
   CREATE_TRY(set_smem(h, attention_f32_kernel, attn_f32_smem_bytes(197)));
   if (cudaStreamCreateWithFlags(&h->copy_stream, cudaStreamNonBlocking) != cudaSuccess ||
-      cudaStreamCreateWithFlags(&h->own_stream, cudaStreamNonBlocking) != cudaSuccess) {
+      cudaStreamCreateWithFlags(&h->own_stream, cudaStreamNonBlocking) != cudaSuccess ||
+      cudaStreamCreateWithFlags(&h->mlp_stream, cudaStreamNonBlocking) != cudaSuccess ||
+      cudaEventCreateWithFlags(&h->ev_mlp_fork, cudaEventDisableTiming) != cudaSuccess ||
+      cudaEventCreateWithFlags(&h->ev_mlp_join, cudaEventDisableTiming) != cudaSuccess) {
     h->err = "cudaStreamCreate failed";
     return bail(ARP_ERR_CUDA);
   }
@@ -830,7 +839,9 @@
 
 template <typename K>
 static cudaError_t launch_clustered(K kernel, int grid, int cg, int smem, cudaStream_t st, const CUtensorMap& ta,
-                                    const CUtensorMap& tb, const CUtensorMap& to, const GemmArgs& g) {
+                                    const CUtensorMap& tb, const CUtensorMap& to, const GemmArgs& g,
+                                    const CUtensorMap* ta2 = nullptr, const CUtensorMap* tb2 = nullptr,
+                                    const CUtensorMap* to2 = nullptr) {
   cudaLaunchConfig_t cfg{};
   cfg.gridDim = dim3(grid);
   cfg.blockDim = dim3(G2_THREADS);
@@ -843,7 +854,7 @@
   attr[0].val.clusterDim.z = 1;
   cfg.attrs = attr;
   cfg.numAttrs = 1;
-  return cudaLaunchKernelEx(&cfg, kernel, ta, tb, to, g);
+  return cudaLaunchKernelEx(&cfg, kernel, ta, tb, to, ta2 ? *ta2 : ta, tb2 ? *tb2 : tb, to2 ? *to2 : to, g);
 }
 
 struct LnFoldArgs { const float2* stats; const float* svec; const float* cvec; int nparts = 1; };
@@ -851,7 +862,7 @@
 static int launch_gemm(ArpHandle* h, const bf16* a, int64_t a_rows_alloc, const bf16* w, void* out, bool out_f32,
                        int act, int64_t M, int N, int K, int ldo, const float* bias, const void* resid, int ldr,
                        const float* rowtab, int period, cudaStream_t st, const LnFoldArgs* fold = nullptr,
-                       float2* stats_out = nullptr) {
+                       float2* stats_out = nullptr, int max_ctas = kNumSMs) {
   if (M <= 0) return ARP_OK;
   if (N % GEMM_BN || K % GEMM_BK) return fail(h, ARP_ERR_INVALID, "GEMM needs N %% 256 == 0 and K %% 64 == 0 (N=%d K=%d)", N, K);
   if (M > 0x7fffffff / 2) return fail(h, ARP_ERR_INVALID, "GEMM M too large");
@@ -886,7 +897,7 @@
   ARP_TRY(get_tmap(h, out, (uint64_t)M, (uint64_t)N, (uint64_t)ldo, 32, &to, out_f32 ? 32 : 64, out_f32 ? 4 : 2));
   const int row_blocks = (int)((M + GEMM_BM * cg - 1) / (GEMM_BM * cg));
   const int tiles = row_blocks * (N / GEMM_BN);
-  const int grid = std::min(tiles * cg, kNumSMs / cg * cg);
+  const int grid = std::min(tiles * cg, max_ctas / cg * cg);
   const int smem = G2Cfg<cg>::SMEM_BYTES;
   ProfScope prof(h, PC_GEMM, 2.0 * (double)M * N * K,
                  (double)M * K * 2 + (double)N * K * 2 + (double)M * N * osz * (reduce ? 2 : 1), st);
@@ -912,6 +923,70 @@
 #undef G2_LAUNCH
   h->launches++;
   if (e != cudaSuccess) return fail(h, ARP_ERR_CUDA, "GEMM launch failed: %s", cudaGetErrorString(e));
+  return ARP_OK;
+}
+
+constexpr int kMlpFusedClusters = 56;
+static int launch_mlp_r16(ArpHandle* h, bf16* x16, int64_t x_rows, const LnFoldArgs& f_fc, const bf16* w_fc_fold,
+                          const bf16* w_proj, const float* b_proj, bf16* hid, int64_t hid_rows, float2* stats_out,
+                          int64_t M, cudaStream_t st, bool unfused = false) {
+  if (M <= 0) return ARP_OK;
+  const int W = h->cfg.width, H = 4 * W;
+  constexpr int cg = 2, band = GEMM_BM * cg;
+  constexpr int clusters = kMlpFusedClusters, all_clusters = kNumSMs / cg;
+  constexpr int side_ctas = kNumSMs - clusters * cg;
+  if (W % GEMM_BN || H / GEMM_BN > G2_MAX_SLICES || f_fc.nparts != 2 * W / 256)
+    return fail(h, ARP_ERR_INVALID, "fused MLP: width %d not supported", W);
+  const int64_t bands = M / band;
+  const int64_t waves = unfused ? 0 : std::min((bands + all_clusters / 2) / all_clusters, bands / clusters);
+  const int64_t Mf = waves * clusters * band;
+  const int64_t scratch_rows = (int64_t)clusters * band;
+  cudaStream_t tail_st = st;
+  int tail_ctas = kNumSMs;
+  bf16* tail_hid = hid;
+  int64_t tail_hid_rows = hid_rows;
+  if (Mf > 0) {
+    if (Mf > 0x7fffffff / 2 || hid_rows < M + scratch_rows - Mf) return fail(h, ARP_ERR_INVALID, "fused MLP: bad M / hidden rows");
+    GemmArgs g;
+    memset(&g, 0, sizeof(g));
+    g.M = (int)Mf; g.N = H; g.K = W; g.out = hid; g.ldo = H; g.bias = b_proj; g.period = 1;
+    g.ln_stats = f_fc.stats; g.ln_nparts = f_fc.nparts; g.svec = f_fc.svec; g.cvec = f_fc.cvec; g.eps = 1e-5f;
+    g.resid = x16; g.ldr = W; g.stats_out = stats_out;
+    const CUtensorMap *ta, *tb, *to, *ta2, *tb2, *to2;
+    ARP_TRY(get_tmap(h, x16, (uint64_t)x_rows, (uint64_t)W, (uint64_t)W, GEMM_BM, &ta));
+    ARP_TRY(get_tmap(h, w_fc_fold, (uint64_t)H, (uint64_t)W, (uint64_t)W, GEMM_BN / cg, &tb));
+    ARP_TRY(get_tmap(h, hid, (uint64_t)scratch_rows, (uint64_t)H, (uint64_t)H, 32, &to, 64, 2));
+    ARP_TRY(get_tmap(h, hid, (uint64_t)scratch_rows, (uint64_t)H, (uint64_t)H, GEMM_BM, &ta2));
+    ARP_TRY(get_tmap(h, w_proj, (uint64_t)W, (uint64_t)H, (uint64_t)H, GEMM_BN / cg, &tb2));
+    ARP_TRY(get_tmap(h, x16, (uint64_t)Mf, (uint64_t)W, (uint64_t)W, 32, &to2, 64, 2));
+    if (Mf < M) {
+      ARP_CUDA(h, cudaEventRecord(h->ev_mlp_fork, st));
+      ARP_CUDA(h, cudaStreamWaitEvent(h->mlp_stream, h->ev_mlp_fork, 0));
+      tail_st = h->mlp_stream;
+      tail_ctas = side_ctas;
+      tail_hid = hid + scratch_rows * H;
+      tail_hid_rows = hid_rows - scratch_rows;
+    }
+    ProfScope prof(h, PC_GEMM, 2.0 * 2.0 * (double)Mf * H * W,
+                   (double)Mf * W * 2 * 3 + 2.0 * H * W * 2 + (double)Mf * f_fc.nparts * 8 * 2, st);
+    const cudaError_t e = launch_clustered(gemm_tcgen05_kernel<bf16, ACT_QUICKGELU, cg, G2_MLP>, clusters * cg, cg,
+                                           G2Cfg<cg>::SMEM_BYTES, st, *ta, *tb, *to, g, ta2, tb2, to2);
+    h->launches++;
+    if (e != cudaSuccess) return fail(h, ARP_ERR_CUDA, "fused MLP launch failed: %s", cudaGetErrorString(e));
+  }
+  const int64_t Mt = M - Mf;
+  if (Mt > 0) {
+    const LnFoldArgs f_t{f_fc.stats + Mf * f_fc.nparts, f_fc.svec, f_fc.cvec, f_fc.nparts};
+    bf16* xt = x16 + Mf * W;
+    ARP_TRY(launch_gemm(h, xt, x_rows - Mf, w_fc_fold, tail_hid, false, ACT_QUICKGELU, Mt, H, W, H, nullptr, nullptr, 0,
+                        nullptr, 0, tail_st, &f_t, nullptr, tail_ctas));
+    ARP_TRY(launch_gemm(h, tail_hid, tail_hid_rows, w_proj, xt, false, ACT_NONE, Mt, W, H, W, b_proj, xt, W, nullptr, 0,
+                        tail_st, nullptr, stats_out + Mf * (2 * W / 256), tail_ctas));
+    if (tail_st != st) {
+      ARP_CUDA(h, cudaEventRecord(h->ev_mlp_join, tail_st));
+      ARP_CUDA(h, cudaStreamWaitEvent(st, h->ev_mlp_join, 0));
+    }
+  }
   return ARP_OK;
 }
 
@@ -1081,10 +1156,7 @@
     ARP_TRY(launch_attention(h, ws.qkv, ws.attn, (int)n, h->tokens, st, Mcap));
     ARP_TRY(launch_gemm(h, ws.attn, Mcap, L.w_out, ws.x16, false, ACT_NONE, M, W, W, W, L.b_out, ws.x16, W, nullptr, 0, st,
                         nullptr, ws.stats));
-    ARP_TRY(launch_gemm(h, ws.x16, Mcap, L.w_fc_fold, ws.hid, false, ACT_QUICKGELU, M, 4 * W, W, 4 * W, nullptr, nullptr,
-                        0, nullptr, 0, st, &f_fc));
-    ARP_TRY(launch_gemm(h, ws.hid, Mcap, L.w_proj, ws.x16, false, ACT_NONE, M, W, 4 * W, W, L.b_proj, ws.x16, W, nullptr,
-                        0, st, nullptr, ws.stats));
+    ARP_TRY(launch_mlp_r16(h, ws.x16, Mcap, f_fc, L.w_fc_fold, L.w_proj, L.b_proj, ws.hid, Mcap, ws.stats, M, st));
     gather_taps(h, ws.x16, n, l, st, taps32);
   }
   return ARP_OK;
@@ -2178,6 +2250,23 @@
   return ARP_OK;
 }
 
+extern "C" int arp_mlp_r16(ArpHandle* h, void* x_dev, const float* stats_in_dev, const void* w_fc_fold_dev,
+                           const float* svec_dev, const float* cvec_dev, const void* w_proj_dev, const float* b_proj_dev,
+                           float* stats_out_dev, int64_t M, int32_t unfused, void* stream) {
+  if (!h || !x_dev || !stats_in_dev || !w_fc_fold_dev || !svec_dev || !cvec_dev || !w_proj_dev || !b_proj_dev || !stats_out_dev)
+    return fail(h, ARP_ERR_INVALID, "null argument");
+  if (M < 1 || M > 0x7fffffff / 2 || h->cfg.width != 768) return fail(h, ARP_ERR_INVALID, "bad M / width");
+  ARP_CUDA(h, cudaSetDevice(h->cfg.device));
+  cudaStream_t st = static_cast<cudaStream_t>(stream);
+  const int W = h->cfg.width;
+  const int64_t hid_rows = std::max<int64_t>(M, (int64_t)kNumSMs * GEMM_BM);
+  ARP_TRY(ensure_scratch(h, 1, (size_t)hid_rows * 4 * W * sizeof(bf16) + 256));
+  const LnFoldArgs f{reinterpret_cast<const float2*>(stats_in_dev), svec_dev, cvec_dev, 2 * W / 256};
+  return launch_mlp_r16(h, static_cast<bf16*>(x_dev), M, f, static_cast<const bf16*>(w_fc_fold_dev),
+                        static_cast<const bf16*>(w_proj_dev), b_proj_dev, reinterpret_cast<bf16*>(h->scratch[1]), hid_rows,
+                        reinterpret_cast<float2*>(stats_out_dev), M, st, unfused != 0);
+}
+
 extern "C" int arp_ln_gemm(ArpHandle* h, const void* x_dev, const float* gamma_dev, const float* beta_dev,
                            const float* w_f32_dev, const float* bias_dev, void* out_dev, int64_t M, int32_t N,
                            int32_t act, void* stream) {
diff --git a/arp_b200/csrc/common.cuh b/arp_b200/csrc/common.cuh
--- a/arp_b200/csrc/common.cuh
+++ b/arp_b200/csrc/common.cuh
@@ -92,6 +92,14 @@
   return d;
 }
 
+#if defined(ARP_ATTN_JITTER) || defined(ARP_MLP_JITTER)
+__device__ __forceinline__ void jitter_sleep(uint32_t salt) {
+  uint32_t h = (static_cast<uint32_t>(clock64()) ^ (salt * 2654435761u) ^ (threadIdx.x >> 5) * 40503u ^ blockIdx.x * 9176u);
+  h ^= h >> 13; h *= 0x5bd1e995u; h ^= h >> 15;
+  if (h & 1) __nanosleep((h >> 1) & 8191);
+}
+#endif
+
 __device__ __forceinline__ void mbar_init(uint64_t* bar, uint32_t count) {
   asm volatile("mbarrier.init.shared::cta.b64 [%0], %1;" ::"r"(smem_u32(bar)), "r"(count) : "memory");
 }
diff --git a/arp_b200/csrc/gemm_tcgen05.cuh b/arp_b200/csrc/gemm_tcgen05.cuh
--- a/arp_b200/csrc/gemm_tcgen05.cuh
+++ b/arp_b200/csrc/gemm_tcgen05.cuh
@@ -5,7 +5,7 @@
 namespace arp {
 
 enum GemmAct : int { ACT_NONE = 0, ACT_QUICKGELU = 1, ACT_RELU = 2 };
-enum G2Mode : int { G2_STORE = 0, G2_REDUCE = 1, G2_LNFOLD = 2, G2_RESID_STATS = 3 };
+enum G2Mode : int { G2_STORE = 0, G2_REDUCE = 1, G2_LNFOLD = 2, G2_RESID_STATS = 3, G2_MLP = 4 };
 
 struct GemmArgs {
   int M, N, K;
@@ -41,6 +41,7 @@
 constexpr int G2_EPI_WARPS = 8;
 constexpr int G2_STAGE_UNIT = 32 * 128;
 constexpr int G2_STAGING_BYTES = G2_EPI_WARPS * G2_STAGE_UNIT;
+constexpr int G2_MAX_SLICES = 12;
 
 template <int CG>
 struct G2Cfg {
@@ -50,12 +51,22 @@
   static constexpr int SMEM_BYTES = STAGES * STAGE_BYTES + G2_STAGING_BYTES + 1024 + 256;
 };
 
+#if defined(ARP_MLP_JITTER)
+#define G2_JITTER(salt) jitter_sleep(salt)
+#else
+#define G2_JITTER(salt)
+#endif
+
 template <typename OutT, int ACT, int CG, int MODE>
 __global__ void __launch_bounds__(G2_THREADS, 1)
 gemm_tcgen05_kernel(const __grid_constant__ CUtensorMap tmap_a, const __grid_constant__ CUtensorMap tmap_b,
-                    const __grid_constant__ CUtensorMap tmap_out, const GemmArgs args) {
+                    const __grid_constant__ CUtensorMap tmap_out, const __grid_constant__ CUtensorMap tmap_a2,
+                    const __grid_constant__ CUtensorMap tmap_b2, const __grid_constant__ CUtensorMap tmap_out2,
+                    const GemmArgs args) {
   using Cfg = G2Cfg<CG>;
   constexpr int STAGES = Cfg::STAGES;
+  constexpr bool MLP = MODE == G2_MLP;
+  static_assert(!MLP || (CG == 2 && sizeof(OutT) == 2 && ACT == ACT_QUICKGELU), "G2_MLP: the default path's 16-bit MLP");
   extern __shared__ uint8_t smem_raw[];
   uint8_t* smem = reinterpret_cast<uint8_t*>((reinterpret_cast<uintptr_t>(smem_raw) + 1023) & ~uintptr_t(1023));
   uint8_t* staging = smem + STAGES * Cfg::STAGE_BYTES;
@@ -65,6 +76,8 @@
   uint64_t* tfull_bar = bars + 2 * STAGES;
   uint64_t* tempty_bar = tfull_bar + 2;
   uint32_t* tmem_slot = reinterpret_cast<uint32_t*>(tempty_bar + 2);
+  uint64_t* slice_bar = tempty_bar + 3;
+  static_assert((2 * STAGES + 4 + 1 + G2_MAX_SLICES) * 8 <= 256, "barriers must fit the 256 reserved bytes");
   static_assert(MODE != G2_RESID_STATS || sizeof(OutT) == 2, "G2_RESID_STATS updates the 16-bit residual stream");
 
   const int warp = __shfl_sync(0xffffffffu, static_cast<int>(threadIdx.x >> 5), 0);
@@ -77,18 +90,34 @@
   const int num_n = args.N / GEMM_BN;
   const int num_tiles = num_m * num_n;
   const int num_kb = args.K / GEMM_BK;
-  const int my_tiles = cluster_id < num_tiles ? (num_tiles - cluster_id + num_clusters - 1) / num_clusters : 0;
-  auto tile_coords = [&](int it, int& m_blk, int& n_blk) {
+  const int proj_n = MLP ? args.K / GEMM_BN : 0;
+  const int band_tiles = num_n + proj_n;
+  const int my_tiles = MLP ? (cluster_id < num_m ? (num_m - cluster_id + num_clusters - 1) / num_clusters * band_tiles : 0)
+                           : (cluster_id < num_tiles ? (num_tiles - cluster_id + num_clusters - 1) / num_clusters : 0);
+  auto tile_coords = [&](int it, int& m_blk, int& n_blk) -> bool {
+    if (MLP) {
+      const int band = it / band_tiles, s = it - band * band_tiles;
+      m_blk = cluster_id + band * num_clusters;
+      n_blk = s < num_n ? s : s - num_n;
+      return s >= num_n;
+    }
     const int tile = cluster_id + it * num_clusters;
     const int tile_o = args.reverse ? num_tiles - 1 - tile : tile;
     m_blk = tile_o / num_n;
     n_blk = tile_o % num_n;
+    return MODE == G2_RESID_STATS;
   };
+  const int scratch_row = (cluster_id * CG + static_cast<int>(rank)) * GEMM_BM;
 
   if (warp == 0 && lane == 0) {
     tma_prefetch_desc(&tmap_a);
     tma_prefetch_desc(&tmap_b);
     tma_prefetch_desc(&tmap_out);
+    if (MLP) {
+      tma_prefetch_desc(&tmap_a2);
+      tma_prefetch_desc(&tmap_b2);
+      tma_prefetch_desc(&tmap_out2);
+    }
   }
   if (warp == 1 && lane == 0) {
     for (int i = 0; i < STAGES; ++i) {
@@ -99,6 +128,8 @@
       mbar_init(&tfull_bar[i], 1);
       mbar_init(&tempty_bar[i], G2_EPI_WARPS * CG);
     }
+    if (MLP)
+      for (int j = 0; j < G2_MAX_SLICES; ++j) mbar_init(&slice_bar[j], G2_EPI_WARPS);
     fence_mbar_init();
   }
   if (warp == 1) {
@@ -115,22 +146,33 @@
       uint32_t phase = 0;
       for (int it = 0; it < my_tiles; ++it) {
         int m_blk, n_blk;
-        tile_coords(it, m_blk, n_blk);
-        const int a_row = (m_blk * CG + rank) * GEMM_BM;
+        const bool proj = tile_coords(it, m_blk, n_blk) && MLP;
+        const CUtensorMap* ma = proj ? &tmap_a2 : &tmap_a;
+        const CUtensorMap* mb = proj ? &tmap_b2 : &tmap_b;
+        const int a_row = proj ? scratch_row : (m_blk * CG + rank) * GEMM_BM;
         const int b_row = n_blk * GEMM_BN + rank * Cfg::B_ROWS;
-        for (int kb = 0; kb < num_kb; ++kb) {
+        const int kbs = proj ? args.N / GEMM_BK : num_kb;
+        const bool wait_slices = proj && n_blk == 0;
+        const uint32_t band_parity = MLP ? static_cast<uint32_t>(it / band_tiles) & 1u : 0u;
+        for (int kb = 0; kb < kbs; ++kb) {
+          if (wait_slices && kb % (GEMM_BN / GEMM_BK) == 0) {
+            G2_JITTER(40 + kb);
+            mbar_wait(&slice_bar[kb / (GEMM_BN / GEMM_BK)], band_parity);
+            fence_proxy_async_all();
+            G2_JITTER(80 + kb);
+          }
           mbar_wait(&empty_bar[stage], phase ^ 1);
           uint8_t* sa = smem + stage * Cfg::STAGE_BYTES;
           uint8_t* sb = sa + GEMM_A_BYTES;
           if (CG == 1) {
             mbar_arrive_expect_tx(&full_bar[stage], Cfg::STAGE_BYTES);
-            tma_load_2d(sa, &tmap_a, &full_bar[stage], kb * GEMM_BK, a_row);
-            tma_load_2d(sb, &tmap_b, &full_bar[stage], kb * GEMM_BK, b_row);
+            tma_load_2d(sa, ma, &full_bar[stage], kb * GEMM_BK, a_row);
+            tma_load_2d(sb, mb, &full_bar[stage], kb * GEMM_BK, b_row);
           } else {
             if (rank == 0) mbar_arrive_expect_tx(&full_bar[stage], 2 * Cfg::STAGE_BYTES);
             const uint32_t leader_bar = mapa_u32(smem_u32(&full_bar[stage]), 0);
-            tma_load_2d_cg2(sa, &tmap_a, leader_bar, kb * GEMM_BK, a_row);
-            tma_load_2d_cg2(sb, &tmap_b, leader_bar, kb * GEMM_BK, b_row);
+            tma_load_2d_cg2(sa, ma, leader_bar, kb * GEMM_BK, a_row);
+            tma_load_2d_cg2(sb, mb, leader_bar, kb * GEMM_BK, b_row);
           }
           if (++stage == STAGES) { stage = 0; phase ^= 1; }
         }
@@ -147,7 +189,8 @@
         mbar_wait(&tempty_bar[acc], acc_phase ^ 1);
         tc_fence_after();
         const uint32_t d_tmem = tmem_base + acc * GEMM_BN;
-        for (int kb = 0; kb < num_kb; ++kb) {
+        const int kbs = MLP && it % band_tiles >= num_n ? args.N / GEMM_BK : num_kb;
+        for (int kb = 0; kb < kbs; ++kb) {
           mbar_wait(&full_bar[stage], phase);
           tc_fence_after();
           const uint32_t sa = smem_u32(smem + stage * Cfg::STAGE_BYTES);
@@ -160,10 +203,10 @@
           }
           if (CG == 1) {
             umma_commit(&empty_bar[stage]);
-            if (kb == num_kb - 1) umma_commit(&tfull_bar[acc]);
+            if (kb == kbs - 1) umma_commit(&tfull_bar[acc]);
           } else {
             umma_commit_cg2(&empty_bar[stage], 0b11);
-            if (kb == num_kb - 1) umma_commit_cg2(&tfull_bar[acc], 0b11);
+            if (kb == kbs - 1) umma_commit_cg2(&tfull_bar[acc], 0b11);
           }
           if (++stage == STAGES) { stage = 0; phase ^= 1; }
         }
@@ -184,12 +227,14 @@
     const int sw = lane & 7;
     for (int it = 0; it < my_tiles; ++it) {
       int m_blk, n_blk;
-      tile_coords(it, m_blk, n_blk);
+      const bool rs = tile_coords(it, m_blk, n_blk);
+      const bool lnf = MODE == G2_LNFOLD || (MLP && !rs);
       const int row0 = (m_blk * CG + rank) * GEMM_BM + quarter * 32;
       const int row = row0 + lane;
-      uint4 xo[MODE == G2_RESID_STATS ? 16 : 1];
+      const CUtensorMap* const rs_out = MLP ? &tmap_out2 : &tmap_out;
+      uint4 xo[MODE == G2_RESID_STATS || MLP ? 16 : 1];
       float st_n = 0.f, st_mean = 0.f, st_m2 = 0.f;
-      if (MODE == G2_RESID_STATS) {
+      if (rs) {
 #pragma unroll
         for (int c = 0; c < 16; ++c) {
           const int r = row0 + 4 * (c & 7) + (lane >> 3);
@@ -198,14 +243,15 @@
         }
         if (lane == 0 && it + 1 < my_tiles) {
           int m2, n2;
-          tile_coords(it + 1, m2, n2);
-          const int r2 = (m2 * CG + rank) * GEMM_BM + quarter * 32, c2 = n2 * GEMM_BN + half * 128;
-          tma_prefetch_l2_2d(&tmap_out, c2, r2);
-          tma_prefetch_l2_2d(&tmap_out, c2 + 64, r2);
+          if (tile_coords(it + 1, m2, n2)) {
+            const int r2 = (m2 * CG + rank) * GEMM_BM + quarter * 32, c2 = n2 * GEMM_BN + half * 128;
+            tma_prefetch_l2_2d(rs_out, c2, r2);
+            tma_prefetch_l2_2d(rs_out, c2 + 64, r2);
+          }
         }
       }
       float ln_rstd = 1.f, ln_rm = 0.f;
-      if (MODE == G2_LNFOLD && row < args.M) {
+      if (lnf && row < args.M) {
         if (args.ln_nparts == 1) {
           const float2 p = __ldg(args.ln_stats + row);
           ln_rstd = p.x;
@@ -239,10 +285,11 @@
       const uint32_t taddr = tmem_base + acc * GEMM_BN + half * 128 + (static_cast<uint32_t>(quarter * 32) << 16);
       const float* tab_row =
           args.rowtab ? args.rowtab + static_cast<size_t>(row % args.period) * args.N : nullptr;
-#pragma unroll(MODE == G2_RESID_STATS ? UNITS : 1)
+      if (rs) {
+#pragma unroll
       for (int u = 0; u < UNITS; ++u) {
         const int n0 = n_blk * GEMM_BN + half * 128 + u * UNIT_COLS;
-        if (MODE == G2_RESID_STATS) {
+        {
           if (lane == 0) tma_store_wait_read<0>();
           __syncwarp();
 #pragma unroll
@@ -303,11 +350,15 @@
           fence_proxy_async_smem();
           __syncwarp();
           if (lane == 0) {
-            tma_store_2d(&tmap_out, sbuf, n0, row0);
+            tma_store_2d(rs_out, sbuf, n0, row0);
             tma_store_commit();
           }
-          continue;
-        }
+        }
+      }
+      } else {
+#pragma unroll 1
+      for (int u = 0; u < UNITS; ++u) {
+        const int n0 = n_blk * GEMM_BN + half * 128 + u * UNIT_COLS;
         float v[UNIT_COLS];
         {
           uint32_t r[32];
@@ -332,7 +383,7 @@
             else mbar_arrive_cluster_relaxed(acc ? tempty_leader1 : tempty_leader0);
           }
         }
-        if (MODE == G2_LNFOLD) {
+        if (lnf) {
 #pragma unroll
           for (int j = 0; j < UNIT_COLS; j += 4) {
             const float4 sv = __ldg(reinterpret_cast<const float4*>(args.svec + n0 + j));
@@ -382,12 +433,23 @@
         __syncwarp();
         if (lane == 0) {
           if (MODE == G2_REDUCE) tma_reduce_add_2d(&tmap_out, sbuf, n0, row0);
-          else tma_store_2d(&tmap_out, sbuf, n0, row0);
+          else tma_store_2d(&tmap_out, sbuf, n0, MLP ? scratch_row + quarter * 32 : row0);
           tma_store_commit();
         }
       }
-      if (MODE == G2_RESID_STATS && row < args.M)
-        args.stats_out[static_cast<size_t>(row) * (2 * num_n) + n_blk * 2 + half] = make_float2(st_mean, st_m2);
+      if (MLP) {
+        if (lane == 0) {
+          tma_store_wait_all<0>();
+          fence_proxy_async_all();
+          G2_JITTER(n_blk);
+          mbar_arrive(&slice_bar[n_blk]);
+          G2_JITTER(20 + n_blk);
+        }
+        __syncwarp();
+      }
+      }
+      if (rs && row < args.M)
+        args.stats_out[static_cast<size_t>(row) * (2 * (MLP ? proj_n : num_n)) + n_blk * 2 + half] = make_float2(st_mean, st_m2);
       if (++acc == 2) { acc = 0; acc_phase ^= 1; }
     }
     if (lane == 0) tma_store_wait_all<0>();
diff --git a/include/arp_b200.h b/include/arp_b200.h
--- a/include/arp_b200.h
+++ b/include/arp_b200.h
@@ -7,7 +7,7 @@
 extern "C" {
 #endif
 
-#define ARP_B200_ABI_VERSION 9
+#define ARP_B200_ABI_VERSION 10
 
 #define ARP_MAX_TEXT 16
 #define ARP_MAX_TEXT_GROUPS 16
@@ -159,6 +159,9 @@
                          float* stats_dev, int64_t M, int32_t N, int32_t K, void* stream);
 ARP_API int arp_ln_gemm(ArpHandle* h, const void* x_dev, const float* gamma_dev, const float* beta_dev, const float* w_f32_dev,
                 const float* bias_dev, void* out_dev, int64_t M, int32_t N, int32_t act, void* stream);
+ARP_API int arp_mlp_r16(ArpHandle* h, void* x_dev, const float* stats_in_dev, const void* w_fc_fold_dev, const float* svec_dev,
+                const float* cvec_dev, const void* w_proj_dev, const float* b_proj_dev, float* stats_out_dev, int64_t M,
+                int32_t unfused, void* stream);
 ARP_API int arp_layernorm_bf16(ArpHandle* h, const float* x_dev, const float* gamma_dev, const float* beta_dev, void* y_dev,
                        int64_t M, void* stream);
 ARP_API int arp_attention(ArpHandle* h, const void* qkv_dev, void* out_dev, int32_t B, int32_t tokens, void* stream);
```

Result: slower. 27810 (median of 6 runs) (-8.5%).
